# minjiyoon/MMGL

Hardware: AMD Instinct MI355X
Metric: train samples/sec (OPT-1.3B flamingo, 16 neighbors) (higher is better)
Workload: dtype bf16; 1 GPU; opt-1.3b context=all neighbor_mode=embedding peft=flamingo, 11+5 neighbors x 4 tokens, T=512+128, roberta-base + clip-vit-base-patch16 frozen encoders, full train step (fwd+bwd+exchange+AdamW); per_gpu_batch=64, global_batch=64, seq_len=640, neighbor_keys=64, trainable_params=216736520, parallelism=dp1

## Files before the change

### include/mmgl_hip.h

```cpp
#ifndef MMGL_HIP_H
#define MMGL_HIP_H

#include <stddef.h>
#include <stdint.h>

#ifdef __cplusplus
extern "C" {
#endif

enum { MMGL_F32 = 0, MMGL_BF16 = 1 };
enum { MMGL_OK = 0, MMGL_ERR_INVALID = 1, MMGL_ERR_UNSUPPORTED = 2, MMGL_ERR_HIP = 3 };
enum { MMGL_ACT_NONE = 0, MMGL_ACT_RELU = 1 };

const char* mmgl_last_error(void);
int mmgl_version(void);

int mmgl_xattn_fwd(const void* q, const void* k, const void* v, const uint8_t* key_valid,
                   void* out, float* lse, int B, int H, int T, int S, int D, int dtype, void* stream);

size_t mmgl_xattn_bwd_workspace(int B, int H, int T, int S, int D);
int mmgl_xattn_bwd(const void* dout, const void* q, const void* k, const void* v, const float* lse,
                   const uint8_t* key_valid, void* dq, void* dk, void* dv,
                   void* workspace, size_t workspace_bytes,
                   int B, int H, int T, int S, int D, int dtype, void* stream);
// ... 28 lines not shown
                          void* probs, float* lse, int B, int H, int T, int S, int D, int causal, float p_drop,
                          uint64_t seed, int dtype, void* stream);
size_t mmgl_attn_general_bwd_workspace(int B, int H, int T);
int mmgl_attn_general_bwd(const void* dout, const void* q, const void* k, const void* v, const float* lse, const uint8_t* key_valid,
                          const float* head_mask, void* dq, void* dk, void* dv, void* workspace, size_t workspace_bytes, int B, int H,
                          int T, int S, int D, int causal, float p_drop, uint64_t seed, int dtype, void* stream);
int mmgl_attn_dropout_mask(uint8_t* mask, int B, int H, int T, int S, float p_drop, uint64_t seed, void* stream);

int mmgl_layernorm_fwd(const void* x, const void* gamma, const void* beta, void* y, float* mean, float* rstd,
                       int rows, int cols, float eps, int dtype, void* stream);
size_t mmgl_norm_bwd_workspace(int rows, int cols);
int mmgl_layernorm_bwd(const void* dy, const void* x, const void* gamma, const float* mean, const float* rstd,
                       void* dx, float* dgamma, float* dbeta, void* workspace, size_t workspace_bytes,
                       int rows, int cols, int dtype, void* stream);

int mmgl_rmsnorm_fwd(const void* x, const void* gamma, void* y, float* rstd,
                     int rows, int cols, float eps, int dtype, void* stream);
int mmgl_rmsnorm_bwd(const void* dy, const void* x, const void* gamma, const float* rstd,
                     void* dx, float* dgamma, void* workspace, size_t workspace_bytes,
                     int rows, int cols, int dtype, void* stream);

int mmgl_add_rmsnorm_fwd(const void* x, const void* res, const void* gamma, void* sum_out, void* y, float* rstd,
                         int rows, int cols, float eps, int dtype, void* stream);
int mmgl_add_rmsnorm_bwd(const void* dy, const void* dsum, const void* sum, const void* gamma, const float* rstd,
                         void* dres, float* dgamma, void* workspace, size_t workspace_bytes,
                         int rows, int cols, int dtype, void* stream);

int mmgl_gated_residual_fwd(const void* residual, const void* x, const float* gate, void* y,
                            size_t n, float p_drop, uint64_t seed, int dtype, void* stream);
size_t mmgl_gated_residual_bwd_workspace(size_t n);
int mmgl_gated_residual_bwd(const void* dy, const void* x, const float* gate, void* dx, float* dgate,
                            void* workspace, size_t workspace_bytes,
                            size_t n, float p_drop, uint64_t seed, int dtype, void* stream);

int mmgl_linear_fwd(const void* x, const void* W, const void* bias, void* y,
                    int M, int N, int K, int act, float out_scale, int dtype, void* stream);
size_t mmgl_linear_bwd_workspace(int M, int N, int K, int act, int dtype);
int mmgl_linear_bwd(const void* dy, const void* y, const void* x, const void* W, void* dx, void* dW, void* dbias,
                    void* workspace, size_t workspace_bytes, int M, int N, int K, int act, float out_scale,
                    int accumulate, int mask_dx, int dtype, void* stream);

int mmgl_lora_linear_fwd(const void* x, const void* W, const void* bias, const void* A, const void* Bm,
                         void* y, void* xa, int M, int N, int K, int r, float scale, int dtype, void* stream);
size_t mmgl_lora_linear_bwd_workspace(int M, int N, int K, int r, int dtype);
int mmgl_lora_linear_bwd(const void* dy, const void* x, const void* xa, const void* W, const void* A,
                         const void* Bm, void* dx, void* dA, void* dB, void* dyb, void* workspace,
                         size_t workspace_bytes, int M, int N, int K, int r, float scale, int accumulate,
                         int dtype, void* stream);

int mmgl_neighbor_interleave_fwd(const void* text_emb, const void* vis_emb, const int64_t* text_loc,
                                 const int64_t* img_loc, const int64_t* text_pos, const int64_t* img_pos,
                                 void* out_emb, uint8_t* out_valid, int B, int Nt, int Ni, int n_tok, int d,
                                 int dtype, void* stream);
int mmgl_neighbor_interleave_bwd(const void* d_out_emb, const int64_t* text_loc, const int64_t* img_loc,
                                 void* d_text_emb, void* d_vis_emb, int B, int Nt, int Ni, int n_tok, int d,
                                 int dtype, void* stream);

int mmgl_cross_entropy_fwd(const void* logits, const int64_t* labels, float* row_lse, float* row_loss,
                           float* loss_sum, float* count, int rows, int V, int64_t ignore_index, int dtype,
                           void* stream);
int mmgl_cross_entropy_bwd(const void* logits, const int64_t* labels, const float* row_lse,
                           const float* count, const float* dloss, void* dlogits,
                           int rows, int V, int64_t ignore_index, int dtype, void* stream);

int mmgl_position_ids(const int64_t* attention_mask, int64_t* pos, int B, int T, void* stream);

int mmgl_adamw_step(void* param, float* master, const void* grad, float* exp_avg, float* exp_avg_sq, size_t n,
                    float lr, float beta1, float beta2, float eps, float weight_decay, int step,
                    float grad_scale, int dtype, void* stream);

int mmgl_gemm_nt_fast(int M, int N, int K, int ldx, int ldw, int ldy, int dtype);
size_t mmgl_gemm_nt_workspace(int M, int N, int K, int ldx, int ldw, int ldy, int dtype);
int mmgl_gemm_nt(const void* x, int ldx, const void* W, int ldw, const void* bias, const void* residual, const void* zmask,
                 void* y, int ldy, int M, int N, int K, int act, float out_scale, void* workspace, size_t workspace_bytes,
                 int dtype, void* stream);
int mmgl_relu_bwd(const void* dy, const void* y, void* out, size_t n, int dtype, void* stream);
int mmgl_gemm_set_tile_counter(void* counter);
void* mmgl_gemm_get_tile_counter(void);
size_t mmgl_gemm_nt_relu_bits_bytes(int M, int N, int K, int ldx, int ldw, int ldy, int dtype);
int mmgl_gemm_nt_relu_bits(const void* x, int ldx, const void* W, int ldw, const void* bias, void* y, int ldy, void* bits_out,
                           int M, int N, int K, float out_scale, int dtype, void* stream);
int mmgl_gemm_nt_masked(const void* x, int ldx, const void* W, int ldw, const void* bits_in, void* y, int ldy, int M, int N, int K,
                        float out_scale, int dtype, void* stream);

int mmgl_rope_inplace(void* buf, const float* cos_sin, size_t rows, int T, int H, int D, int ld, int nblk, int backward,
                      int dtype, void* stream);
int mmgl_rope(const void* src, void* dst, const float* cos_sin, size_t rows, int T, int H, int D, int ld, int nblk, int nall,
              int backward, int dtype, void* stream);
int mmgl_swiglu_fwd(const void* gate_up, void* y, size_t M, int F, int dtype, void* stream);
int mmgl_swiglu_bwd(const void* dy, const void* gate_up, void* dgate_up, size_t M, int F, int dtype, void* stream);

int mmgl_encattn_fwd(const void* q, const void* k, const void* v, const int32_t* cu_seqlens, void* out, int nseq,
                     int H, int D, int ld_in, int ld_out, int max_len, int q_rows, int dtype, void* stream);
int mmgl_add_layernorm_fwd(const void* x, const void* res, const void* gamma, const void* beta, void* sum_out,
                           void* y, float* mean, float* rstd, int rows, int cols, float eps, float p_drop, uint64_t seed,
                           int dtype, void* stream);
int mmgl_add_layernorm_bwd(const void* dy, const void* dsum, const void* sum, const void* gamma, const float* mean,
                           const float* rstd, void* dres, void* dx, float* dgamma, float* dbeta, void* workspace,
                           size_t workspace_bytes, int rows, int cols, float p_drop, uint64_t seed, int dtype,
                           void* stream);
int mmgl_layernorm_tiles_fwd(const void* x, const void* gamma, const void* beta, void* y, void* yc, const int32_t* rowmap,
                             float* mean, float* rstd, int rows, int cols, int crows, float eps, int dtype, void* stream);
int mmgl_add_layernorm_tiles_fwd(const void* x, const void* res, const void* gamma, const void* beta, void* sum_out, void* y,
                                 void* yc, const int32_t* rowmap, float* mean, float* rstd, int rows, int cols, int crows,
                                 float eps, float p_drop, uint64_t seed, int dtype, void* stream);
int mmgl_activation_fwd(const void* x, void* y, size_t n, int act, int dtype, void* stream);
int mmgl_scale(const void* x, const float* scale, void* y, size_t n, int dtype, void* stream);

enum { MMGL_COMM_I64 = 2 };
int mmgl_comm_unique_id(void* out128);
int mmgl_comm_init(int rank, int world, const void* unique_id, void** comm);
int mmgl_allreduce_sum(void* comm, void* buf, size_t count, int dtype, void* stream);
int mmgl_allgather(void* comm, const void* in, void* out, size_t count_per_rank, int dtype, void* stream);
int mmgl_broadcast(void* comm, void* buf, size_t count, int dtype, int root, void* stream);
int mmgl_comm_destroy(void* comm);

int mmgl_gemm_skinny_lora(const void* x, int ldx, const void* W, int ldw, const void* bias, const void* residual, void* y, int ldy,
                          const void* lora_A, int lda, const void* lora_B, int ldb, int r, float lora_scale, void* workspace,
                          int M, int N, int K, int act, float scale, int dtype, void* stream);
int mmgl_gemm_skinny(const void* x, int ldx, const void* W, int ldw, const void* bias, const void* residual, void* y, int ldy,
                     int M, int N, int K, int act, float scale, int dtype, void* stream);
int mmgl_attn_decode_fwd(const void* q, int ldq, const void* k, const void* v, int ldkv, size_t batch_stride_kv,
                         const uint8_t* key_valid, int ld_valid, void* out, int B, int H, int S, int D, int dtype, void* stream);

int mmgl_attn_decode_gqa_fwd(const void* q, int ldq, const void* k, const void* v, int ldkv, size_t batch_stride_kv,
                             const uint8_t* key_valid, int ld_valid, void* out, int B, int H, int Hkv, int S, int D, int dtype,
                             void* stream);
int mmgl_rope_kv_append(void* qkv, int ldqkv, const float* cos_sin_row, void* kv_col, size_t batch_stride_kv, int B, int H, int Hkv,
                        int D, int dtype, void* stream);

size_t mmgl_beam_topk_workspace(int rows, int V, int W);
int mmgl_attn_decode_beam_fwd(const void* q, int ldq, const void* k_pre, const void* v_pre, int ld_pre, size_t batch_stride_pre,
                              const uint8_t* key_valid, int ld_valid, const void* k_tail, const void* v_tail, int ld_tail,
                              size_t row_stride_tail, const int* src, int ld_src, void* out, int B, int W, int H, int S_pre, int n_tail,
                              int D, int dtype, void* stream);
int mmgl_beam_topk(const void* logits, size_t ld_logits, const float* beam_score, float* cand_score, int* cand_index, void* workspace,
                   size_t workspace_bytes, int B, int rows_in, int W, int V, int dtype, void* stream);
int mmgl_beam_advance(const float* cand_score, const int* cand_index, int64_t* tokens, int* parents, float* beam_score,
                      const int* src_old, int* src_new, int ld_src, const float* pool_score_old, float* pool_score_new,
                      const int* pool_len_old, int* pool_len_new, const int* pool_anc_old, int* pool_anc_new,
                      const int64_t* pool_tok_old, int64_t* pool_tok_new, int* done, int B, int W, int V, int n_cols, int eos_token_id,
                      int last_step, int early_stopping, float length_divisor, void* stream);

int mmgl_sample_tokens(const void* logits, size_t ld_logits, const float* u, int64_t* tokens, int64_t token_stride, uint8_t* finished,
                       int* kept, int rows, int n_draws, int V, float temperature, int top_k, float top_p, int eos_token_id,
                       int64_t pad_token_id, int dtype, void* stream);

int mmgl_logits_process(void* logits, size_t ld_logits, const int64_t* history, size_t ld_history, const uint8_t* hist_valid,
                        size_t ld_valid, int n_masked, int hist_len, const int* ban, int n_ban, int rows, int V,
                        float repetition_penalty, int no_repeat_ngram_size, int dtype, void* stream);

int mmgl_guidance_logits(void* logits, size_t ld_logits, int batch, int V, float guidance_scale, int dtype, void* stream);

int mmgl_attn_decode_block_fwd(const void* q, int ldq, const void* k_new, const void* v_new, int ld_new, void* k, void* v, int ldkv,
                               size_t batch_stride_kv, int capacity, const uint8_t* key_valid, int ld_valid, const int* len, void* out,
                               int B, int m, int H, int D, int dtype, void* stream);
int mmgl_lookup_accept(const void* logits, size_t ld_logits, int m_in, int64_t* block, int* n_draft, int64_t* positions, int64_t* ids,
                       size_t ld_ids, const uint8_t* prompt_mask, size_t ld_mask, int* gen, int* len, uint8_t* finished, int* emitted,
                       int B, int T, int n_new, int V, int K, int N, int64_t eos_token_id, int64_t pad_token_id, int pos_offset,
                       int pos_max, int dtype, void* stream);

int mmgl_rope_kv_append_block(void* qkv, int ldqkv, const float* cos_sin, int n_pos, void* kv, int ldkv, size_t batch_stride_kv, int capacity,
                              const int* len, int B, int m, int H, int Hkv, int D, int dtype, void* stream);
int mmgl_attn_decode_gqa_block_fwd(const void* q, int ldq, const void* k, const void* v, int ldkv, size_t batch_stride_kv, int capacity,
                                   const uint8_t* key_valid, int ld_valid, const int* len, void* out, int B, int m, int H, int Hkv, int D,
                                   int dtype, void* stream);

int mmgl_contrastive_chunk(void);
size_t mmgl_contrastive_workspace(int B, int k, int n_cap);
int mmgl_contrastive_select(const void* cand_hidden, size_t ld_cand, void* ctx, size_t ld_ctx, size_t batch_stride_ctx, uint8_t* ctx_valid,
                            size_t ld_valid, int n_cap, const float* cand_score, const int* cand_index, size_t ld_pair, float alpha, int n_ctx,
                            int step, int* src, size_t ld_src, int64_t* ids, size_t ld_ids, uint8_t* finished, int64_t eos_token_id,
                            int64_t pad_token_id, void* hidden_out, int* selected, float* trace_p, float* trace_pen, float* trace_score,
                            void* workspace, size_t workspace_bytes, int B, int k, int d, int V, int dtype, void* stream);

int mmgl_kv_quantize(const void* k, const void* v, int ld_src, size_t batch_stride_src, void* codes, int ld_code, size_t batch_stride_code,
                     void* scale, int ld_scale, size_t batch_stride_scale, int B, int n, int H, int D, int dtype, void* stream);
int mmgl_attn_decode_q8_fwd(const void* q, int ldq, const void* k_new, const void* v_new, int ld_new, void* k_codes, void* v_codes,
                            int ld_code, size_t batch_stride_code, void* k_scale, void* v_scale, int ld_scale, size_t batch_stride_scale,
                            int capacity, const uint8_t* key_valid, int ld_valid, void* out, int B, int H, int S, int D, int dtype,
                            void* stream);

int mmgl_attn_decode_gqa_q8_fwd(const void* q, int ldq, const void* k_new, const void* v_new, int ld_new, void* k_codes, void* v_codes,
                                int ld_code, size_t batch_stride_code, void* k_scale, void* v_scale, int ld_scale,
                                size_t batch_stride_scale, int capacity, const uint8_t* key_valid, int ld_valid, void* out, int B, int H,
                                int Hkv, int S, int D, int dtype, void* stream);

int mmgl_weight_quantize(const void* w, int ldw, void* codes, int ld_codes, void* exps, int N, int K, int dtype, void* stream);
// ... 8 lines not shown
```

### mmgl_amd/_lib.py

```python
import ctypes
import os

import torch

_HERE = os.path.dirname(os.path.abspath(__file__))
LIB_PATH = os.environ.get("MMGL_LIB_PATH") or os.path.join(_HERE, "libmmgl_hip.so")

ABI_VERSION = 110
F32, BF16 = 0, 1
ACT_NONE, ACT_RELU = 0, 1
_ERR_INVALID, _ERR_UNSUPPORTED, _ERR_HIP = 1, 2, 3

c_void_p, c_int, c_float, c_size_t, c_u64, c_i64 = (ctypes.c_void_p, ctypes.c_int, ctypes.c_float, ctypes.c_size_t,
                                                    ctypes.c_uint64, ctypes.c_int64)
P, I, F, Z, U, L = c_void_p, c_int, c_float, c_size_t, c_u64, c_i64

SIGNATURES = {
    "mmgl_last_error": (ctypes.c_char_p, []),
    "mmgl_version": (I, []),
    "mmgl_xattn_fwd": (I, [P, P, P, P, P, P, I, I, I, I, I, I, P]),
    "mmgl_xattn_bwd_workspace": (Z, [I, I, I, I, I]),
    "mmgl_xattn_bwd": (I, [P, P, P, P, P, P, P, P, P, P, Z, I, I, I, I, I, I, P]),
    "mmgl_selfattn_fwd": (I, [P, P, P, P, P, P, I, I, I, I, I, I, P]),
    "mmgl_selfattn_bwd_workspace": (Z, [I, I, I]),
    "mmgl_selfattn_bwd": (I, [P, P, P, P, P, P, P, P, P, P, P, Z, I, I, I, I, I, I, I, P]),
    "mmgl_selfattn_prefix_fwd": (I, [P, P, P, P, P, P, I, I, I, I, I, I, I, I, P]),
    "mmgl_selfattn_prefix_bwd": (I, [P, P, P, P, P, P, P, P, P, P, P, Z, I, I, I, I, I, I, I, I, I, I, P]),
    "mmgl_selfattn_tiles_fwd": (I, [P, P, P, P, P, P, P, I, I, I, I, I, I, I, I, P]),
    "mmgl_selfattn_tiles_bwd": (I, [P, P, P, P, P, P, P, P, P, P, P, P, Z, I, I, I, I, I, I, I, I, I, I, P]),
    "mmgl_selfattn_gqa_fwd": (I, [P, P, P, P, P, P, I, I, I, I, I, I, I, I, P]),
    "mmgl_selfattn_gqa_bwd_workspace": (Z, [I, I, I, I, I, I]),
    "mmgl_selfattn_gqa_bwd": (I, [P, P, P, P, P, P, P, P, P, P, P, Z, I, I, I, I, I, I, I, I, I, I, P]),
    "mmgl_attn_general_fwd": (I, [P, P, P, P, P, P, P, P, I, I, I, I, I, I, F, U, I, P]),
    "mmgl_attn_general_bwd_workspace": (Z, [I, I, I]),
    "mmgl_attn_general_bwd": (I, [P, P, P, P, P, P, P, P, P, P, P, Z, I, I, I, I, I, I, F, U, I, P]),
    "mmgl_attn_dropout_mask": (I, [P, I, I, I, I, F, U, P]),
    "mmgl_layernorm_fwd": (I, [P, P, P, P, P, P, I, I, F, I, P]),
    "mmgl_norm_bwd_workspace": (Z, [I, I]),
    "mmgl_layernorm_bwd": (I, [P, P, P, P, P, P, P, P, P, Z, I, I, I, P]),
    "mmgl_rmsnorm_fwd": (I, [P, P, P, P, I, I, F, I, P]),
    "mmgl_rmsnorm_bwd": (I, [P, P, P, P, P, P, P, Z, I, I, I, P]),
    "mmgl_add_rmsnorm_fwd": (I, [P, P, P, P, P, P, I, I, F, I, P]),
    "mmgl_add_rmsnorm_bwd": (I, [P, P, P, P, P, P, P, P, Z, I, I, I, P]),
    "mmgl_gated_residual_fwd": (I, [P, P, P, P, Z, F, U, I, P]),
    "mmgl_gated_residual_bwd_workspace": (Z, [Z]),
    "mmgl_gated_residual_bwd": (I, [P, P, P, P, P, P, Z, Z, F, U, I, P]),
    "mmgl_linear_fwd": (I, [P, P, P, P, I, I, I, I, F, I, P]),
    "mmgl_linear_bwd_workspace": (Z, [I, I, I, I, I]),
    "mmgl_linear_bwd": (I, [P, P, P, P, P, P, P, P, Z, I, I, I, I, F, I, I, I, P]),
    "mmgl_lora_linear_fwd": (I, [P, P, P, P, P, P, P, I, I, I, I, F, I, P]),
    "mmgl_lora_linear_bwd_workspace": (Z, [I, I, I, I, I]),
    "mmgl_lora_linear_bwd": (I, [P, P, P, P, P, P, P, P, P, P, P, Z, I, I, I, I, F, I, I, P]),
    "mmgl_neighbor_interleave_fwd": (I, [P, P, P, P, P, P, P, P, I, I, I, I, I, I, P]),
    "mmgl_neighbor_interleave_bwd": (I, [P, P, P, P, P, I, I, I, I, I, I, P]),
    "mmgl_cross_entropy_fwd": (I, [P, P, P, P, P, P, I, I, L, I, P]),
    "mmgl_cross_entropy_bwd": (I, [P, P, P, P, P, P, I, I, L, I, P]),
    "mmgl_position_ids": (I, [P, P, I, I, P]),
    "mmgl_adamw_step": (I, [P, P, P, P, P, Z, F, F, F, F, F, I, F, I, P]),
    "mmgl_encattn_fwd": (I, [P, P, P, P, P, I, I, I, I, I, I, I, I, P]),
    "mmgl_add_layernorm_fwd": (I, [P, P, P, P, P, P, P, P, I, I, F, F, U, I, P]),
    "mmgl_add_layernorm_bwd": (I, [P, P, P, P, P, P, P, P, P, P, P, Z, I, I, F, U, I, P]),
    "mmgl_layernorm_tiles_fwd": (I, [P, P, P, P, P, P, P, P, I, I, I, F, I, P]),
    "mmgl_add_layernorm_tiles_fwd": (I, [P, P, P, P, P, P, P, P, P, P, I, I, I, F, F, U, I, P]),
    "mmgl_activation_fwd": (I, [P, P, Z, I, I, P]),
    "mmgl_scale": (I, [P, P, P, Z, I, P]),
    "mmgl_gemm_nt_fast": (I, [I, I, I, I, I, I, I]),
    "mmgl_gemm_nt_workspace": (Z, [I, I, I, I, I, I, I]),
    "mmgl_gemm_nt_relu_bits_bytes": (Z, [I, I, I, I, I, I, I]),
    "mmgl_gemm_nt_relu_bits": (I, [P, I, P, I, P, P, I, P, I, I, I, F, I, P]),
    "mmgl_gemm_nt_masked": (I, [P, I, P, I, P, P, I, I, I, I, F, I, P]),
    "mmgl_gemm_nt": (I, [P, I, P, I, P, P, P, P, I, I, I, I, I, F, P, Z, I, P]),
    "mmgl_relu_bwd": (I, [P, P, P, Z, I, P]),
    "mmgl_gemm_set_tile_counter": (I, [P]),
    "mmgl_gemm_get_tile_counter": (P, []),
    "mmgl_rope_inplace": (I, [P, P, Z, I, I, I, I, I, I, I, P]),
    "mmgl_rope": (I, [P, P, P, Z, I, I, I, I, I, I, I, I, P]),
    "mmgl_swiglu_fwd": (I, [P, P, Z, I, I, P]),
    "mmgl_swiglu_bwd": (I, [P, P, P, Z, I, I, P]),
    "mmgl_comm_unique_id": (I, [P]),
    "mmgl_comm_init": (I, [I, I, P, ctypes.POINTER(ctypes.c_void_p)]),
    "mmgl_allreduce_sum": (I, [P, P, Z, I, P]),
    "mmgl_allgather": (I, [P, P, P, Z, I, P]),
    "mmgl_broadcast": (I, [P, P, Z, I, I, P]),
    "mmgl_comm_destroy": (I, [P]),
    "mmgl_gemm_skinny": (I, [P, I, P, I, P, P, P, I, I, I, I, I, F, I, P]),
    "mmgl_attn_decode_fwd": (I, [P, I, P, P, I, Z, P, I, P, I, I, I, I, I, P]),
    "mmgl_gemm_skinny_lora": (I, [P, I, P, I, P, P, P, I, P, I, P, I, I, F, P, I, I, I, I, F, I, P]),
    "mmgl_attn_decode_gqa_fwd": (I, [P, I, P, P, I, Z, P, I, P, I, I, I, I, I, I, P]),
    "mmgl_rope_kv_append": (I, [P, I, P, P, Z, I, I, I, I, I, P]),
    "mmgl_attn_decode_beam_fwd": (I, [P, I, P, P, I, Z, P, I, P, P, I, Z, P, I, P, I, I, I, I, I, I, I, P]),
    "mmgl_beam_topk_workspace": (Z, [I, I, I]),
    "mmgl_beam_topk": (I, [P, Z, P, P, P, P, Z, I, I, I, I, I, P]),
    "mmgl_beam_advance": (I, [P, P, P, P, P, P, P, I, P, P, P, P, P, P, P, P, P, I, I, I, I, I, I, I, F, P]),
    "mmgl_sample_tokens": (I, [P, Z, P, P, L, P, P, I, I, I, F, I, F, I, L, I, P]),
    "mmgl_logits_process": (I, [P, Z, P, Z, P, Z, I, I, P, I, I, I, F, I, I, P]),
    "mmgl_guidance_logits": (I, [P, Z, I, I, F, I, P]),
    "mmgl_attn_decode_block_fwd": (I, [P, I, P, P, I, P, P, I, Z, I, P, I, P, P, I, I, I, I, I, P]),
    "mmgl_lookup_accept": (I, [P, Z, I, P, P, P, P, Z, P, Z, P, P, P, P, I, I, I, I, I, I, L, L, I, I, I, P]),
    "mmgl_rope_kv_append_block": (I, [P, I, P, I, P, I, Z, I, P, I, I, I, I, I, I, P]),
    "mmgl_attn_decode_gqa_block_fwd": (I, [P, I, P, P, I, Z, I, P, I, P, P, I, I, I, I, I, I, P]),
    "mmgl_contrastive_chunk": (I, []),
    "mmgl_contrastive_workspace": (Z, [I, I, I]),
    "mmgl_contrastive_select": (I, [P, Z, P, Z, Z, P, Z, I, P, P, Z, F, I, I, P, Z, P, Z, P, L, L, P, P, P, P, P, P, Z, I, I, I, I, I, P]),
    "mmgl_kv_quantize": (I, [P, P, I, Z, P, I, Z, P, I, Z, I, I, I, I, I, P]),
    "mmgl_attn_decode_q8_fwd": (I, [P, I, P, P, I, P, P, I, Z, P, P, I, Z, I, P, I, P, I, I, I, I, I, P]),
    "mmgl_attn_decode_gqa_q8_fwd": (I, [P, I, P, P, I, P, P, I, Z, P, P, I, Z, I, P, I, P, I, I, I, I, I, I, P]),
    "mmgl_weight_quantize": (I, [P, I, P, I, P, I, I, I, P]),
    "mmgl_gemm_skinny_w8": (I, [P, I, P, I, P, P, P, P, I, I, I, I, I, F, I, P]),
}

_lib = None


def lib():
    global _lib
    if _lib is None:
        if not os.path.exists(LIB_PATH):
            raise RuntimeError(
                f"{LIB_PATH} not found: the HIP extension is not built. Run `python -m mmgl_amd._build` "
                "(or __graft_entry__.build()). mmgl_amd has no CPU fallback.")
        h = ctypes.CDLL(LIB_PATH)
        h.mmgl_version.restype = ctypes.c_int
        if h.mmgl_version() != ABI_VERSION:
            raise RuntimeError(f"{LIB_PATH} reports ABI version {h.mmgl_version()}, this binding expects {ABI_VERSION}: a stale build -- "
                               "run `python -m mmgl_amd._build --force`")
        for name, (res, args) in SIGNATURES.items():
            fn = getattr(h, name)
            fn.restype = res
            fn.argtypes = args
        _lib = h
    return _lib


def check(rc: int, what: str = ""):
    if rc == 0:
        return
    msg = lib().mmgl_last_error().decode("utf-8", "replace")
    if rc in (_ERR_INVALID, _ERR_UNSUPPORTED):
        raise ValueError(msg or what)
    raise RuntimeError(msg or what)


def dtype_code(t: torch.Tensor) -> int:
    if t.dtype == torch.float32:
        return F32
    if t.dtype == torch.bfloat16:
        return BF16
    raise ValueError(f"mmgl_amd kernels take float32 or bfloat16 activations, got {t.dtype}")


def ptr(t):
    return None if t is None else ctypes.c_void_p(t.data_ptr())


# ... 60 lines not shown
```

### mmgl_amd/csrc/gemm.hip

```cpp
#include "common.h"
#include "gemm8p.h"
#include <stdlib.h>

namespace {

constexpr int BM = 128, BN = 128, ROWB = 128;
constexpr int TILE_BYTES = BM * ROWB;

template <typename T> struct GT {
    static constexpr int VN = 16 / sizeof(T);
    static constexpr int BK = ROWB / sizeof(T);
    static constexpr int KSTEPS = BK / 32;
    typedef T chunk_t __attribute__((ext_vector_type(16 / sizeof(T))));
};

__device__ __forceinline__ int swz(int row, int c) { return row * ROWB + ((c ^ ((row >> 1) & 7)) << 4); }

template <typename T> __device__ __forceinline__ typename Elem<T>::v8 lds_frag(const char* tile, int row, int ks, int g);
template <> __device__ __forceinline__ bf16x8 lds_frag<bf16>(const char* tile, int row, int ks, int g) {
    return *(const bf16x8*)(tile + swz(row, ks * 4 + g));
}
template <> __device__ __forceinline__ f32x8 lds_frag<float>(const char* tile, int row, int ks, int g) {
    const f32x4 a = *(const f32x4*)(tile + swz(row, 2 * g));
    const f32x4 b = *(const f32x4*)(tile + swz(row, 2 * g + 1));
// ... 796 lines not shown
    MMGL_CHECK_ARG(dy && x && W && workspace && (act == MMGL_ACT_NONE || y), "mmgl_linear_bwd: null pointer");
    MMGL_CHECK_ARG(workspace_bytes >= mmgl_linear_bwd_workspace(M, N, K, act, dtype), "mmgl_linear_bwd: workspace too small");
    hipStream_t st = (hipStream_t)stream;
    char* ws = (char*)workspace;
    DT_SWITCH("mmgl_linear_bwd",
              linear_bwd<bf16>((const bf16*)dy, (const bf16*)y, (const bf16*)x, (const bf16*)W, (bf16*)dx, (bf16*)dW, (bf16*)dbias, ws, M, N, K, act, out_scale, accumulate, st, mask_dx != 0),
              linear_bwd<float>((const float*)dy, (const float*)y, (const float*)x, (const float*)W, (float*)dx, (float*)dW, (float*)dbias, ws, M, N, K, act, out_scale, accumulate, st, mask_dx != 0));
}

extern "C" int mmgl_lora_linear_fwd(const void* x, const void* W, const void* bias, const void* A, const void* Bm, void* y,
                                    void* xa, int M, int N, int K, int r, float scale, int dtype, void* stream) {
    MMGL_CHECK_ARG(x && W && A && Bm && y && xa && r > 0, "mmgl_lora_linear_fwd: bad arguments");
    hipStream_t st = (hipStream_t)stream;
    DT_SWITCH("mmgl_lora_linear_fwd",
              lora_fwd<bf16>((const bf16*)x, (const bf16*)W, (const bf16*)bias, (const bf16*)A, (const bf16*)Bm, (bf16*)y, (bf16*)xa, M, N, K, r, scale, st),
              lora_fwd<float>((const float*)x, (const float*)W, (const float*)bias, (const float*)A, (const float*)Bm, (float*)y, (float*)xa, M, N, K, r, scale, st));
}

extern "C" size_t mmgl_lora_linear_bwd_workspace(int M, int N, int K, int r, int dtype) {
    return lora_ws(M, N, K, r, dtype == MMGL_BF16 ? 2 : 4);
}

extern "C" int mmgl_lora_linear_bwd(const void* dy, const void* x, const void* xa, const void* W, const void* A,
                                    const void* Bm, void* dx, void* dA, void* dB, void* dyb, void* workspace,
                                    size_t workspace_bytes, int M, int N, int K, int r, float scale, int accumulate,
                                    int dtype, void* stream) {
    MMGL_CHECK_ARG(dy && x && xa && W && A && Bm && dx && dA && dB && dyb && workspace && r > 0, "mmgl_lora_linear_bwd: bad arguments");
    MMGL_CHECK_ARG(workspace_bytes >= mmgl_lora_linear_bwd_workspace(M, N, K, r, dtype), "mmgl_lora_linear_bwd: workspace too small");
    hipStream_t st = (hipStream_t)stream;
    char* ws = (char*)workspace;
    DT_SWITCH("mmgl_lora_linear_bwd",
              lora_bwd<bf16>((const bf16*)dy, (const bf16*)x, (const bf16*)xa, (const bf16*)W, (const bf16*)A, (const bf16*)Bm, (bf16*)dx, (bf16*)dA, (bf16*)dB, (bf16*)dyb, ws, M, N, K, r, scale, accumulate, st),
              lora_bwd<float>((const float*)dy, (const float*)x, (const float*)xa, (const float*)W, (const float*)A, (const float*)Bm, (float*)dx, (float*)dA, (float*)dB, (float*)dyb, ws, M, N, K, r, scale, accumulate, st));
}

extern "C" int mmgl_gemm_nt_fast(int M, int N, int K, int ldx, int ldw, int ldy, int dtype) {
    const NtRoute r = nt_route(M, N, K, ldx, ldw, ldy, dtype, true);
    return r == NtRoute::P8 ? 1 : r == NtRoute::MID ? 2 : 0;
}

extern "C" size_t mmgl_gemm_nt_workspace(int M, int N, int K, int ldx, int ldw, int ldy, int dtype) {
    if (nt_route(M, N, K, ldx, ldw, ldy, dtype, true) != NtRoute::P8 || !gemm8p_use_splits(M, N, K)) return 0;
    return align_up(gemm8p_split_bytes(M, N, K), 256);
}

extern "C" int mmgl_gemm_nt(const void* x, int ldx, const void* W, int ldw, const void* bias, const void* residual, const void* zmask,
                            void* y, int ldy, int M, int N, int K, int act, float out_scale, void* workspace, size_t workspace_bytes,
                            int dtype, void* stream) {
    MMGL_CHECK_ARG(x && W && y, "mmgl_gemm_nt: null pointer");
    MMGL_CHECK_ARG(act >= 0 && act <= 4, "mmgl_gemm_nt: unknown activation %d", act);
    MMGL_CHECK_ARG(ldx + 127 >= K && ldw >= K && ldy >= N, "mmgl_gemm_nt: leading dimensions (%d, %d, %d) smaller than the rows (K=%d, N=%d)", ldx, ldw, ldy, K, N);
    hipStream_t st = (hipStream_t)stream;
    const NtRoute r = nt_route(M, N, K, ldx, ldw, ldy, dtype, true);
    DT_SWITCH("mmgl_gemm_nt",
              launch_nt<bf16>(r, (const bf16*)x, ldx, (const bf16*)W, ldw, (bf16*)y, ldy, (const bf16*)bias, (const bf16*)residual,
                              (const bf16*)zmask, M, N, K, act, out_scale, (float*)workspace, workspace_bytes, st),
              launch_nt<float>(r, (const float*)x, ldx, (const float*)W, ldw, (float*)y, ldy, (const float*)bias, (const float*)residual,
                               (const float*)zmask, M, N, K, act, out_scale, (float*)workspace, workspace_bytes, st));
}

extern "C" size_t mmgl_gemm_nt_relu_bits_bytes(int M, int N, int K, int ldx, int ldw, int ldy, int dtype) {
    return nt_route(M, N, K, ldx, ldw, ldy, dtype, false) == NtRoute::P8 ? gemm8p_bits_bytes(M, N) : 0;
}

extern "C" int mmgl_gemm_nt_relu_bits(const void* x, int ldx, const void* W, int ldw, const void* bias, void* y, int ldy, void* bits_out,
                                      int M, int N, int K, float out_scale, int dtype, void* stream) {
    MMGL_CHECK_ARG(x && W && y && bits_out, "mmgl_gemm_nt_relu_bits: null pointer");
    MMGL_CHECK_ARG(mmgl_gemm_nt_relu_bits_bytes(M, N, K, ldx, ldw, ldy, dtype) > 0,
                   "mmgl_gemm_nt_relu_bits: shape M=%d N=%d K=%d (ld %d %d %d, dtype %d) does not run as whole tiles of the persistent kernel", M, N, K, ldx, ldw, ldy, dtype);
    return launch_gemm8p((const bf16*)x, ldx, (const bf16*)W, ldw, (bf16*)y, ldy, (const bf16*)bias, nullptr, nullptr, M, N, K, MMGL_ACT_RELU,
                         out_scale, (hipStream_t)stream, nullptr, 0, (unsigned*)bits_out, nullptr);
}

extern "C" int mmgl_gemm_nt_masked(const void* x, int ldx, const void* W, int ldw, const void* bits_in, void* y, int ldy, int M, int N, int K,
                                   float out_scale, int dtype, void* stream) {
    MMGL_CHECK_ARG(x && W && y && bits_in, "mmgl_gemm_nt_masked: null pointer");
    MMGL_CHECK_ARG(ldx + 127 >= K && ldw >= K && ldy >= N, "mmgl_gemm_nt_masked: leading dimensions (%d, %d, %d) smaller than the rows (K=%d, N=%d)", ldx, ldw, ldy, K, N);
    MMGL_CHECK_ARG(mmgl_gemm_nt_relu_bits_bytes(M, N, K, ldx, ldw, ldy, dtype) > 0,
                   "mmgl_gemm_nt_masked: shape M=%d N=%d K=%d (ld %d %d %d, dtype %d) does not run as whole tiles of the persistent kernel", M, N, K, ldx, ldw, ldy, dtype);
    return launch_gemm8p((const bf16*)x, ldx, (const bf16*)W, ldw, (bf16*)y, ldy, nullptr, nullptr, nullptr, M, N, K, MMGL_ACT_NONE, out_scale,
                         (hipStream_t)stream, nullptr, 0, nullptr, (const unsigned*)bits_in);
}

extern "C" int mmgl_relu_bwd(const void* dy, const void* y, void* out, size_t n, int dtype, void* stream) {
    MMGL_CHECK_ARG(dy && y && out, "mmgl_relu_bwd: null pointer");
    hipStream_t st = (hipStream_t)stream;
    DT_SWITCH("mmgl_relu_bwd", launch_relu_mask<bf16>((const bf16*)dy, (const bf16*)y, (bf16*)out, n, 1.f, st),
              launch_relu_mask<float>((const float*)dy, (const float*)y, (float*)out, n, 1.f, st));
}
```

### mmgl_amd/csrc/gemm8p.h

```cpp
#pragma once
#include "common.h"

bool gemm8p_supported(int M, int N, int K, int ldx, int ldw, int ldy);
constexpr int GEMM8P_MIN_TILES = 160;
int gemm8p_splits(int M, int N, int K);
size_t gemm8p_split_bytes(int M, int N, int K);
int launch_gemm8p(const bf16* X, int ldx, const bf16* W, int ldw, bf16* Y, int ldy, const bf16* bias, const bf16* resid,
                  const bf16* zmask, int M, int N, int K, int act, float scale, hipStream_t st, float* part = nullptr,
                  size_t part_bytes = 0, unsigned* bits_out = nullptr, const unsigned* bits_in = nullptr);
inline size_t gemm8p_bits_bytes(int M, int N) { return (size_t)cdiv(M, 256) * cdiv(N, 256) * 8192; }

int gemm8p_tt_splits(int RA, int RB, int M);
int launch_gemm8p_tt(const bf16* A, int lda, const bf16* B, int ldb, bf16* Out, float* part, int RA, int RB, int M, int nsplit, float scale,
                     int accumulate, hipStream_t st);

bool gemm_mid_supported(int M, int N, int K, int ldx, int ldw, int ldy);
int launch_gemm_mid(const bf16* X, int ldx, const bf16* W, int ldw, bf16* Y, int ldy, const bf16* bias, const bf16* resid, const bf16* zmask,
                    int M, int N, int K, int act, float scale, hipStream_t st);
```

### mmgl_amd/csrc/gemm8p.hip

```cpp
#include "common.h"
#include "gemm8p.h"
#include <atomic>
#include <stdlib.h>
#include <type_traits>

namespace {

typedef __attribute__((address_space(3))) void lds_void;
typedef unsigned p8_u32x4 __attribute__((ext_vector_type(4)));

constexpr int P8_UNIT = 16384;
constexpr int P8_LDS = 8 * P8_UNIT;
constexpr int P8_LDS_TOTAL = P8_LDS + 16 * 1024;
constexpr int P8_LDS_ALLOC = P8_LDS_TOTAL + 64;

struct P8Args {
    const bf16* X;
    const bf16* W;
    bf16* Y;
    const bf16* bias;
    const bf16* resid;
    const bf16* zmask;
    int M, N, K;
    int ldx, ldw, ldy;
    float scale;
    int act;
    int tiles_m, tiles_n, total;
    int nsplit;
    float* part;
    unsigned* bits_out;
    const unsigned* bits_in;
    int tile0;
    long long* trace;
    int trace_wg;
    unsigned* sched;
};

__device__ __forceinline__ int p8_fetch_item(unsigned* sched, int xcd, int nlists, int G, int Gx, int nitems) {
    for (int t = 0; t < nlists; ++t) {
        const int j = xcd + t < nlists ? xcd + t : xcd + t - nlists;
        const unsigned k = atomicAdd(&sched[j], 1u);
        const long long v = (long long)(k / (unsigned)Gx) * G + j * Gx + (int)(k % (unsigned)Gx);
        if (v < nitems) return (int)v;
    }
    return -1;
}

template <int ACT> __device__ __forceinline__ float p8_act(float v) {
    if constexpr (ACT == 2) {
        const float z = fabsf(v) * 0.70710678118654752f;
        const float t = __builtin_amdgcn_rcpf(1.f + 0.3275911f * z);
        const float poly = t * (0.254829592f + t * (-0.284496736f + t * (1.421413741f + t * (-1.453152027f + t * 1.061405429f))));
        const float er = 1.f - poly * __expf(-z * z);
        return 0.5f * v * (1.f + copysignf(er, v));
    }
    else if constexpr (ACT == 3) return v * __builtin_amdgcn_rcpf(1.f + __expf(-1.702f * v));
    else if constexpr (ACT == 4) {
        const float u = 0.7978845608028654f * (v + 0.044715f * v * v * v);
        return 0.5f * v * (1.f + tanhf(u));
    } else if constexpr (ACT == 1) return fmaxf(v, 0.f);
    else return v;
}

__device__ __forceinline__ int p8_lane() {
    int l;
    asm volatile("v_mbcnt_lo_u32_b32 %0, -1, 0\n\tv_mbcnt_hi_u32_b32 %0, -1, %0" : "=v"(l));
    return l;
}

#ifndef P8_STORE_AUX
#define P8_STORE_AUX 18
#endif
#ifndef P8_ZMASK_AUX
#define P8_ZMASK_AUX 2
#endif
#ifndef P8_PART_AUX
#define P8_PART_AUX 0
#endif
#ifndef P8_LOADX_AUX
#define P8_LOADX_AUX 0
#endif
#ifndef P8_LOADW_AUX
#define P8_LOADW_AUX 0
#endif
#ifndef P8_TRACE
#define P8_TRACE 0
#endif
#define P8_BARRIER() asm volatile("s_barrier" ::: "memory")
#define P8_VMCNT(n) asm volatile("s_waitcnt vmcnt(" #n ")" ::: "memory")
#define P8_LGKM0() asm volatile("s_waitcnt lgkmcnt(0)" ::: "memory")

template <int ACT, bool ZR> __global__ __launch_bounds__(512) void gemm8p_kernel(P8Args a) {
    extern __shared__ __attribute__((aligned(16))) char smem[];
    const int tid = threadIdx.x, lane = tid & 63;
    const int wave = __builtin_amdgcn_readfirstlane(tid >> 6);
    const int wr = wave >> 2, wc = wave & 3;
    const int x = lane & 15, g = lane >> 4;
    int nk = a.K >> 6;

    const int G = gridDim.x;
    const int wg = (G & 7) == 0 ? (int)(blockIdx.x & 7) * (G >> 3) + (int)(blockIdx.x >> 3) : (int)blockIdx.x;
    const bool dyn = a.sched != nullptr;
    const int nlists = (G & 7) == 0 ? 8 : 1, Gx = G / nlists, xcd = nlists == 8 ? (int)(blockIdx.x & 7) : 0;
    int* mailbox = (int*)(smem + P8_LDS_TOTAL);
    auto item_origin = [&](int v, int& m0, int& n0, int& k0, int& nki, int& sp) -> bool {
        if (v < 0 || v >= a.total * a.nsplit) return false;
        int tm, tn;
        sp = v % a.nsplit;
        grouped_tile(a.tile0 + v / a.nsplit, a.tiles_m, a.tiles_n, tm, tn);
        m0 = tm * 256;
        n0 = tn * 256;
        const int units = a.K >> 7, base = units / a.nsplit, rem = units % a.nsplit;
        k0 = (sp * base + (sp < rem ? sp : rem)) * 128;
        nki = (base + (sp < rem ? 1 : 0)) * 2;
        return true;
    };
    auto tile_origin = [&](int it, int& m0, int& n0, int& k0, int& nki, int& sp) -> bool { return item_origin(it * G + wg, m0, n0, k0, nki, sp); };
    auto mk_desc = [&](const bf16* base, int row0, int rows, int ld, int k0, bool valid) {
// ... 54 lines not shown
#if P8_TRACE
    int tr_n = 0;
    auto stamp = [&](int it_) __attribute__((always_inline)) {
        if (a.trace && (int)blockIdx.x == a.trace_wg && it_ >= 2 && tr_n < 64) {
            const long long t = __builtin_readcyclecounter();
            if (lane == 0) a.trace[wave * 64 + tr_n] = t;
            ++tr_n;
        }
    };
#define P8_STAMP(it_) stamp(it_)
#else
#define P8_STAMP(it_) (void)0
#endif

#define P8_MM(FX, FW, J0, T0, I0, I1)                                                          \
    do {                                                                                       \
        _Pragma("unroll") for (int i_ = (I0); i_ < (I1); ++i_) {                               \
            const int ks_ = i_ >> 3, j_ = (i_ >> 1) & 3, t_ = i_ & 1;                          \
            mma16(acc[(T0) + t_][(J0) + j_], FW[ks_][t_], FX[ks_][j_]);                        \
        }                                                                                      \
    } while (0)

    int m0 = 0, n0 = 0, m1 = 0, n1 = 0, k0 = 0, k1 = 0, nk1 = 0, sp0 = 0, sp1 = 0;
    int it = 0;
    int vcur = wg, vnext = G + wg;
    if (dyn) {
        if (tid == 0) mailbox[2] = p8_fetch_item(a.sched, xcd, nlists, G, Gx, a.total * a.nsplit);
        __syncthreads();
        vcur = mailbox[2];
        if (vcur < 0) {
            if (tid == 0 && atomicAdd(&a.sched[8], 1u) == (unsigned)G - 1u)
                for (int i = 0; i < 9; ++i) atomicExch(&a.sched[i], 0u);
            return;
        }
    }
    if (!item_origin(vcur, m0, n0, k0, nk, sp0)) return;
    bool have_next = dyn ? false : tile_origin(1, m1, n1, k1, nk1, sp1);
    __amdgpu_buffer_rsrc_t dXc = mk_desc(a.X, m0, a.M, a.ldx, k0, true), dWc = mk_desc(a.W, n0, a.N, a.ldw, k0, true);
    __amdgpu_buffer_rsrc_t dXn = mk_desc(a.X, m1, a.M, a.ldx, k1, have_next), dWn = mk_desc(a.W, n1, a.N, a.ldw, k1, have_next);

    const __amdgpu_buffer_rsrc_t dBias = __builtin_amdgcn_make_buffer_rsrc((void*)a.bias, 0, a.bias ? a.N * 2 : 0, 0x00020000);
    auto fetch_bias = [&](int nt0, int par) __attribute__((always_inline)) {
        const int ln = p8_lane();
        const unsigned off = ln < 8 ? (unsigned)((nt0 + wc * 64 + ln * 8) * 2) : 0xffffffffu;
        __builtin_amdgcn_raw_ptr_buffer_load_lds(dBias, (lds_void*)(smem + P8_LDS + (par & 1) * 8192 + wave * 1024), 16, off, 0, 0, 0);
    };
    auto y_desc = [&](const bf16* base, int mt0) {
        long long rem = (long long)(a.M - mt0) * a.ldy * 2;
        if (rem > 0xffffffffLL) rem = 0xffffffffLL;
        return __builtin_amdgcn_make_buffer_rsrc((void*)(base + (size_t)mt0 * a.ldy), 0, (int)(unsigned)rem, 0x00020000);
    };
    const bool has_bias = a.bias != nullptr, has_scale = a.scale != 1.f;
    auto epilogue_q = [&](int m0, int n0, int par, int q_lo, int q_hi) __attribute__((always_inline)) {
        if constexpr (ACT == 5) {
            const int ln = p8_lane();
            const int ncol_l = wc * 64 + 8 * (ln >> 4);
            const unsigned base = (unsigned)(((wr * 128 + (ln & 15)) * 256 + ncol_l) * 4);
            const unsigned rstep = (unsigned)(16 * 256 * 4);
            const int vitem = vcur;
            const __amdgpu_buffer_rsrc_t dP = __builtin_amdgcn_make_buffer_rsrc((void*)(a.part + ((size_t)vitem << 16)), 0, 256 * 256 * 4, 0x00020000);
#pragma unroll
            for (int T0 = 0; T0 < 4; T0 += 2)
#pragma unroll
                for (int J = 0; J < 8; ++J) {
                    const unsigned off = base + (unsigned)J * rstep + (unsigned)(64 * T0);
                    __builtin_amdgcn_raw_buffer_store_b128(__builtin_bit_cast(p8_u32x4, acc[T0][J]), dP, off, 0, P8_PART_AUX);
                    __builtin_amdgcn_raw_buffer_store_b128(__builtin_bit_cast(p8_u32x4, acc[T0 + 1][J]), dP, off + 16, 0, P8_PART_AUX);
                    acc[T0][J] = vzero<f32x4>();
                    acc[T0 + 1][J] = vzero<f32x4>();
                }
            return;
        }
        const int ln = p8_lane();
        const int ncol_l = wc * 64 + 8 * (ln >> 4);
        const bool col_ok0 = n0 + ncol_l < a.N, col_ok1 = n0 + ncol_l + 32 < a.N;
        const unsigned base = (unsigned)(((wr * 128 + (ln & 15)) * a.ldy + n0 + ncol_l) * 2);
        const unsigned rstep = (unsigned)(16 * a.ldy * 2);
        auto y_off = [&](int J, int T0) __attribute__((always_inline)) -> unsigned {
            return (T0 ? col_ok1 : col_ok0) ? base + (unsigned)J * rstep + (unsigned)(32 * T0) : 0xffffffffu;
        };
        const __amdgpu_buffer_rsrc_t dY = y_desc(a.Y, m0);
        bf16x8 pre[16];
        p8_u32x4 mbits = {0u, 0u, 0u, 0u};
        if constexpr (ZR) {
            const __amdgpu_buffer_rsrc_t dZ = y_desc(a.zmask ? a.zmask : a.resid, m0);
            if (a.bits_in) {
                mbits = *(const p8_u32x4*)(a.bits_in + ((size_t)((a.tile0 + vcur) * 8 + wave) * 64 + ln) * 4);
            } else if (a.zmask) {
#pragma unroll
                for (int q = 0; q < 4; ++q)
#pragma unroll
                    for (int j = 0; j < 4; ++j) {
                        const int J0 = (q == 0 || q == 1) ? 0 : 4, T0 = (q == 0 || q == 3) ? 0 : 2;
                        pre[q * 4 + j] = __builtin_bit_cast(bf16x8, __builtin_amdgcn_raw_buffer_load_b128(dZ, y_off(J0 + j, T0), 0, P8_ZMASK_AUX));
                    }
            } else {
#pragma unroll
                for (int q = 0; q < 4; ++q)
#pragma unroll
                    for (int j = 0; j < 4; ++j) {
                        const int J0 = (q == 0 || q == 1) ? 0 : 4, T0 = (q == 0 || q == 3) ? 0 : 2;
                        pre[q * 4 + j] = __builtin_bit_cast(bf16x8, __builtin_amdgcn_raw_buffer_load_b128(dZ, y_off(J0 + j, T0), 0, 0));
                    }
            }
        }
#pragma unroll
        for (int q = 0; q < 4; ++q) {
            if (q < q_lo || q >= q_hi) continue;
            const int J0 = (q == 0 || q == 1) ? 0 : 4, T0 = (q == 0 || q == 3) ? 0 : 2;
            if (has_bias) {
                const bf16x8 br = *(const bf16x8*)(smem + P8_LDS + (par & 1) * 8192 + wave * 1024 + ((ln >> 4) + 2 * T0) * 16);
                const f32x4 b0 = {(float)br[0], (float)br[1], (float)br[2], (float)br[3]}, b1 = {(float)br[4], (float)br[5], (float)br[6], (float)br[7]};
#pragma unroll
                for (int j = 0; j < 4; ++j) { acc[T0][J0 + j] += b0; acc[T0 + 1][J0 + j] += b1; }
            }
            if (has_scale) {
#pragma unroll
                for (int j = 0; j < 4; ++j) { acc[T0][J0 + j] *= a.scale; acc[T0 + 1][J0 + j] *= a.scale; }
            }
            unsigned qbits = 0;
            auto rows = [&](auto mode_tag) __attribute__((always_inline)) {
                constexpr int MODE = decltype(mode_tag)::value;
#pragma unroll
                for (int j = 0; j < 4; ++j) {
                    const unsigned off = y_off(J0 + j, T0);
                    const f32x4 lo = acc[T0][J0 + j], hi = acc[T0 + 1][J0 + j];
                    f32x8 v = {lo[0], lo[1], lo[2], lo[3], hi[0], hi[1], hi[2], hi[3]};
                    if constexpr (ACT >= 2 || (ACT == 1 && ZR)) {
#pragma unroll
                        for (int e = 0; e < 8; ++e) v[e] = p8_act<ACT>(v[e]);
                    }
                    if constexpr (MODE == 2) {
                        const bf16x8 z = pre[q * 4 + j];
#pragma unroll
                        for (int e = 0; e < 8; ++e) v[e] += (float)z[e];
                    }
                    if constexpr (MODE == 3) {
                        const bf16x8 z = pre[q * 4 + j];
                        const __amdgpu_buffer_rsrc_t dR = y_desc(a.resid, m0);
                        const bf16x8 rr = __builtin_bit_cast(bf16x8, __builtin_amdgcn_raw_buffer_load_b128(dR, off, 0, 0));
#pragma unroll
                        for (int e = 0; e < 8; ++e) v[e] = (((float)z[e] > 0.f) ? v[e] : 0.f) + (float)rr[e];
                    }
                    p8_u32x4 ob = __builtin_bit_cast(p8_u32x4, __builtin_convertvector(v, bf16x8));
                    if constexpr (ACT == 1 && !ZR) {
#pragma unroll
                        for (int e = 0; e < 4; ++e) {
                            unsigned w = ob[e];
                            asm("v_pk_max_i16 %0, %1, 0" : "=v"(w) : "v"(w));
                            ob[e] = w;
                        }
                        if (a.bits_out) {
                            unsigned by = 0;
#pragma unroll
                            for (int e = 0; e < 4; ++e) {
                                unsigned t = ob[e];
                                asm("v_pk_min_u16 %0, %1, 1 op_sel_hi:[1,0]" : "=v"(t) : "v"(t));
                                t |= t >> 15;
                                by |= t << (2 * e);
                            }
                            qbits |= (by & 0xffu) << (8 * j);
                        }
                    }
                    if constexpr (MODE == 1) {
                        const p8_u32x4 zz = __builtin_bit_cast(p8_u32x4, pre[q * 4 + j]);
#pragma unroll
                        for (int e = 0; e < 4; ++e) {
                            unsigned m = zz[e];
                            asm("v_pk_max_i16 %0, %1, 0\n\tv_pk_min_u16 %0, %0, 1 op_sel_hi:[1,0]\n\tv_pk_sub_u16 %0, 0, %0" : "=v"(m) : "v"(m));
                            ob[e] &= m;
                        }
                    }
                    if constexpr (MODE == 4) {
                        const unsigned by = mbits[q] >> (8 * j);
#pragma unroll
                        for (int e = 0; e < 4; ++e) {
                            unsigned t = (by >> (2 * e)) & 3u;
                            t = (t | (t << 15)) & 0x00010001u;
                            unsigned mk;
                            asm("v_mul_u32_u24 %0, %1, %2" : "=v"(mk) : "v"(t), "v"(0xffffu));
                            ob[e] &= mk;
                        }
                    }
                    __builtin_amdgcn_raw_buffer_store_b128(ob, dY, off, 0, P8_STORE_AUX);
                }
            };
            if constexpr (!ZR) rows(std::integral_constant<int, 0>());
            else if (a.bits_in) rows(std::integral_constant<int, 4>());
            else if (a.zmask && a.resid) rows(std::integral_constant<int, 3>());
            else if (a.zmask) rows(std::integral_constant<int, 1>());
            else rows(std::integral_constant<int, 2>());
            if constexpr (ACT == 1 && !ZR) {
                if (a.bits_out) a.bits_out[((size_t)((a.tile0 + vcur) * 8 + wave) * 64 + ln) * 4 + q] = qbits;
            }
#pragma unroll
            for (int j = 0; j < 4; ++j) { acc[T0][J0 + j] = vzero<f32x4>(); acc[T0 + 1][J0 + j] = vzero<f32x4>(); }
        }
    };
    auto epilogue = [&]() __attribute__((always_inline)) { epilogue_q(m0, n0, it, 0, 4); };


    stage(3, 7, dWc, 0);
    stage(0, 0, dXc, 0);
    stage(1, 1, dWc, 0);
    stage(2, 2, dXc, 0);
    stage(3, 3, dWc, 128);
    stage(0, 4, dXc, 128);
    stage(1, 5, dWc, 128);
#pragma unroll
    for (int t = 0; t < 4; ++t)
#pragma unroll
        for (int j = 0; j < 8; ++j) acc[t][j] = vzero<f32x4>();
    bf16x8 fx[2][4], fwA[2][2], fwB[2][2];
    fetch_bias(n0, 0);
    if (dyn && tid == 0) {
        const int nit = a.total * a.nsplit, cap = (nit + G - 1) / G;
        const int i1 = cap >= 2 ? p8_fetch_item(a.sched, xcd, nlists, G, Gx, nit) : -1;
        mailbox[0] = i1;
        mailbox[1] = (cap >= 3 && i1 >= 0) ? p8_fetch_item(a.sched, xcd, nlists, G, Gx, nit) : -1;
        asm volatile("s_waitcnt lgkmcnt(0)" ::: "memory");
    }
    P8_VMCNT(11);
    P8_BARRIER();
    rdW(fwA, 7);
    P8_LGKM0();
    if (wr) P8_BARRIER();
    if (dyn) {
        vnext = mailbox[0];
        have_next = item_origin(vnext, m1, n1, k1, nk1, sp1);
        dXn = mk_desc(a.X, m1, a.M, a.ldx, k1, have_next);
        dWn = mk_desc(a.W, n1, a.N, a.ldw, k1, have_next);
    }

#define P8_PHASE_M(READ, TY, SLOT, DK, FX, FW, J0, T0, MM, WAITN)                                \
    do {                                                                                         \
        READ;                                                                                    \
        {                                                                                        \
            const int kk_ = kt + (DK);                                                           \
            const bool nx_ = kk_ >= nk;                                                          \
            const int kb_ = (nx_ ? kk_ - nk : kk_) * 128;                                        \
            if ((TY) & 1) stage((TY), (SLOT), nx_ ? dWn : dWc, kb_);                             \
            else stage((TY), (SLOT), nx_ ? dXn : dXc, kb_);                                      \
        }                                                                                        \
        P8_VMCNT(WAITN);                                                                         \
        P8_BARRIER();                                                                            \
        __builtin_amdgcn_sched_barrier(0);                                                       \
        __builtin_amdgcn_s_setprio(1);                                                           \
         \
         \
        MM(FX, FW, J0, T0, 0, 15);                                                               \
        P8_LGKM0();                                                                              \
        __builtin_amdgcn_sched_barrier(0);                                                       \
        P8_BARRIER();                                                                            \
        MM(FX, FW, J0, T0, 15, 16);                                                              \
        __builtin_amdgcn_s_setprio(0);                                                           \
        __builtin_amdgcn_sched_barrier(0);                                                       \
    } while (0)

#define P8_PHASE(READ, TY, SLOT, DK, FX, FW, J0, T0) P8_PHASE_M(READ, TY, SLOT, DK, FX, FW, J0, T0, P8_MM, 10)
    for (;;) {
        P8_STAMP(it);
        for (int kt = 0; kt < nk; kt += 2) {
            P8_PHASE(rdX(fx, 0), 2, 6, 1, fx, fwA, 0, 0);
            if (kt < 4) P8_STAMP(it);
            P8_PHASE(rdW(fwB, 1), 3, 7, 2, fx, fwB, 0, 2);
            if (kt < 4) P8_STAMP(it);
            P8_PHASE(rdX(fx, 2), 0, 0, 2, fx, fwB, 4, 2);
            if (kt < 4) P8_STAMP(it);
            P8_PHASE(rdW(fwB, 3), 1, 1, 2, fx, fwA, 4, 0);
            if (kt < 4) P8_STAMP(it);
// ... 78 lines not shown
        }
        const size_t yo = m * (size_t)ldy + n;
        if (zmask) {
            const bf16x8 z = *(const bf16x8*)(zmask + yo);
#pragma unroll
            for (int e = 0; e < 8; ++e) v[e] = ((float)z[e] > 0.f) ? v[e] : 0.f;
        }
        if (resid) {
            const bf16x8 r = *(const bf16x8*)(resid + yo);
#pragma unroll
            for (int e = 0; e < 8; ++e) v[e] += (float)r[e];
        }
        f32x8 o8 = {v[0], v[1], v[2], v[3], v[4], v[5], v[6], v[7]};
        *(bf16x8*)(Y + yo) = __builtin_convertvector(o8, bf16x8);
    }
}

}

void gemm8p_plan(int M, int N, int K, int* direct, int* nsplit) {
    const int tiles = cdiv(M, 256) * cdiv(N, 256), units = K / 128;
    *direct = tiles;
    *nsplit = 0;
    if (tiles < GEMM8P_MIN_TILES) {
        constexpr int min_units = 24;
        if (units < min_units) return;
        if (units < 32 && tiles >= 64) return;
        int s = (224 + tiles - 1) / tiles;
        if (s > 8) s = 8;
        if (s > units / 2) s = units / 2;
        if (s >= 2) { *direct = 0; *nsplit = s; }
        return;
    }
    constexpr int hybrid = 3;
    const int G = mmgl_num_cu(), rounds = tiles / G, r = tiles % G;
    if (!hybrid || rounds < 1 || rounds > 12 || r == 0) return;
    int s = G / r;
    if (s > 8) s = 8;
    if (s > units / 4) s = units / 4;
    if (s >= hybrid && s >= 2) { *direct = tiles - r; *nsplit = s; }
}
int gemm8p_splits(int M, int N, int K) {
    int d, s;
    gemm8p_plan(M, N, K, &d, &s);
    return s;
}

bool gemm8p_supported(int M, int N, int K, int ldx, int ldw, int ldy) {
    return M > 0 && N > 0 && K >= 256 && K % 128 == 0 && N % 16 == 0 && ldx % 8 == 0 && ldw % 8 == 0 && ldy % 8 == 0 &&
           (long long)M * ldx * 2 < 0xffffffffLL && (long long)N * ldw * 2 < 0xffffffffLL;
}

size_t gemm8p_split_bytes(int M, int N, int K) {
    int d, sp;
    gemm8p_plan(M, N, K, &d, &sp);
    return sp ? (size_t)(cdiv(M, 256) * cdiv(N, 256) - d) * sp * (256 * 256 * sizeof(float)) : 0;
}

static std::atomic<unsigned*> g_tile_counter[64];
static std::atomic<int> g_tile_counters_set{0};
static hipStream_t const P8_STREAM_UNBOUND = (hipStream_t)(intptr_t)-1;
static std::atomic<hipStream_t> g_tile_stream[64];
static unsigned* p8_tile_counter() {
    if (!g_tile_counters_set.load(std::memory_order_relaxed)) return nullptr;
    int dev = 0;
    if (hipGetDevice(&dev) != hipSuccess) return nullptr;
    return g_tile_counter[dev & 63].load(std::memory_order_acquire);
}
static bool p8_tile_counter_for(hipStream_t st, unsigned** out) {
    *out = nullptr;
    if (!g_tile_counters_set.load(std::memory_order_relaxed)) return true;
    int dev = 0;
    if (hipGetDevice(&dev) != hipSuccess) return true;
    unsigned* c = g_tile_counter[dev & 63].load(std::memory_order_acquire);
    if (!c) return true;
    hipStream_t bound = P8_STREAM_UNBOUND;
    if (!g_tile_stream[dev & 63].compare_exchange_strong(bound, st, std::memory_order_acq_rel) && bound != st) return false;
    *out = c;
    return true;
}

int launch_gemm8p(const bf16* X, int ldx, const bf16* W, int ldw, bf16* Y, int ldy, const bf16* bias, const bf16* resid,
                  const bf16* zmask, int M, int N, int K, int act, float scale, hipStream_t st, float* part, size_t part_bytes,
                  unsigned* bits_out, const unsigned* bits_in) {
    if (!gemm8p_supported(M, N, K, ldx, ldw, ldy))
        MMGL_FAIL(MMGL_ERR_UNSUPPORTED, "gemm8p: shape M=%d N=%d K=%d (ld %d %d %d) not supported", M, N, K, ldx, ldw, ldy);
    P8Args a;
    a.X = X; a.W = W; a.Y = Y; a.bias = bias; a.resid = resid; a.zmask = zmask;
    a.M = M; a.N = N; a.K = K; a.ldx = ldx; a.ldw = ldw; a.ldy = ldy; a.scale = scale; a.act = act;
    a.tiles_m = cdiv(M, 256); a.tiles_n = cdiv(N, 256); a.total = a.tiles_m * a.tiles_n;
    a.nsplit = 1;
    a.part = nullptr;
    a.bits_out = bits_out;
    a.bits_in = bits_in;
    if (bits_out && (act != 1 || resid || zmask)) MMGL_FAIL(MMGL_ERR_INVALID, "gemm8p: mask bits are written by the plain ReLU epilogue only");
    if (bits_in && (zmask || resid || act != 0)) MMGL_FAIL(MMGL_ERR_INVALID, "gemm8p: mask bits are applied by the plain epilogue only");
    if (bits_out || bits_in) part = nullptr;
    const int n_cu = mmgl_num_cu();
    const int tiles = a.total;
    int direct = tiles, nsplit = 0;
    if (part && part_bytes >= gemm8p_split_bytes(M, N, K)) gemm8p_plan(M, N, K, &direct, &nsplit);
    a.trace = nullptr;
    a.trace_wg = 0;
    a.tile0 = 0;
    if (!p8_tile_counter_for(st, &a.sched)) {
        static const bool strict = getenv("MMGL_GEMM_STRICT_STREAM") && atoi(getenv("MMGL_GEMM_STRICT_STREAM"));
        if (strict)
            MMGL_FAIL(MMGL_ERR_INVALID, "gemm8p: the dynamic tile schedule of this device is bound to another stream (one stream per device "
                                        "while mmgl_gemm_set_tile_counter is in effect)");
        a.sched = nullptr;
    }
    if (direct > 0) {
        a.total = direct;
        const int grid = direct < n_cu ? direct : n_cu;
#if P8_TRACE
        if (const char* e = getenv("MMGL_P8_TRACE")) a.trace = (long long*)strtoull(e, nullptr, 0);
        if (const char* e = getenv("MMGL_P8_TRACE_WG")) a.trace_wg = atoi(e);
#endif
        const bool zr = resid || zmask || bits_in;
#define P8_LAUNCH(A, Z)                                                                                     \
    do {                                                                                                    \
        if (int rc = mmgl_set_lds(gemm8p_kernel<A, Z>, P8_LDS_ALLOC, "gemm8p")) return rc;                  \
        hipLaunchKernelGGL((gemm8p_kernel<A, Z>), dim3(grid), dim3(512), P8_LDS_ALLOC, st, a);              \
    } while (0)
        switch (act) {
            case 0: if (zr) P8_LAUNCH(0, true); else P8_LAUNCH(0, false); break;
            case 1: if (zr) P8_LAUNCH(1, true); else P8_LAUNCH(1, false); break;
            case 2: if (zr) MMGL_FAIL(MMGL_ERR_UNSUPPORTED, "gemm8p: gelu(erf) with residual / zmask is not instantiated"); P8_LAUNCH(2, false); break;
            case 3: if (zr) P8_LAUNCH(3, true); else P8_LAUNCH(3, false); break;
            case 4: if (zr) P8_LAUNCH(4, true); else P8_LAUNCH(4, false); break;
            default: MMGL_FAIL(MMGL_ERR_INVALID, "gemm8p: unknown activation %d", act);
        }
#undef P8_LAUNCH
        MMGL_CHECK_LAUNCH("gemm8p");
    }
    if (nsplit) {
        MMGL_CHECK_ARG(act >= 0 && act <= 4, "gemm8p: unknown activation %d", act);
        const int rest = tiles - direct;
        a.tile0 = direct;
        a.total = rest;
        a.nsplit = nsplit;
        a.part = part;
        a.trace = nullptr;
        const int items = rest * nsplit, g = items < n_cu ? items : n_cu;
        if (int rc = mmgl_set_lds(gemm8p_kernel<5, false>, P8_LDS_ALLOC, "gemm8p (K split)")) return rc;
        hipLaunchKernelGGL((gemm8p_kernel<5, false>), dim3(g), dim3(512), P8_LDS_ALLOC, st, a);
        MMGL_CHECK_LAUNCH("gemm8p (K split)");
        int blocks = rest * 32;
        if (blocks > 2048) blocks = 2048;
        hipLaunchKernelGGL(p8_splitk_finish_kernel, dim3(blocks), dim3(256), 0, st, part, Y, bias, resid, zmask, M, N, ldy, nsplit, act, scale,
                           direct, rest, a.tiles_m, a.tiles_n);
        MMGL_CHECK_LAUNCH("gemm8p split-K finish");
    }
    return MMGL_OK;
}

extern "C" int mmgl_gemm_set_tile_counter(void* counter) {
    int dev = 0;
    hipError_t e = hipGetDevice(&dev);
    if (e != hipSuccess) MMGL_FAIL(MMGL_ERR_HIP, "mmgl_gemm_set_tile_counter: hipGetDevice: %s", hipGetErrorString(e));
    g_tile_stream[dev & 63].store(P8_STREAM_UNBOUND, std::memory_order_release);
    unsigned* old = g_tile_counter[dev & 63].exchange((unsigned*)counter, std::memory_order_acq_rel);
    g_tile_counters_set.fetch_add((counter != nullptr) - (old != nullptr), std::memory_order_relaxed);
    return MMGL_OK;
}

extern "C" void* mmgl_gemm_get_tile_counter(void) { return p8_tile_counter(); }
```

### mmgl_amd/csrc/rownorm.hip

```cpp
#include "common.h"

namespace {

constexpr int NVMAX = 4;
constexpr int MAXBLK = 512;

template <typename T> struct Vec {
    static constexpr int N = 16 / sizeof(T);
    typedef T type __attribute__((ext_vector_type(16 / sizeof(T))));
};

template <int TPR> __device__ __forceinline__ float row_sum(float v, float* red, int row_in_blk) {
    v = wave_sum(v);
    if constexpr (TPR == 64) return v;
    else {
        const int w = threadIdx.x >> 6;
        __syncthreads();
        if ((threadIdx.x & 63) == 0) red[w] = v;
        __syncthreads();
        return red[0] + red[1] + red[2] + red[3];
    }
}

template <typename T, int TPR, int NV, int MODE>
__global__ __launch_bounds__(256) void norm_fwd_kernel(const T* __restrict__ x, const T* __restrict__ res,
                                                       const T* __restrict__ gamma, const T* __restrict__ beta,
                                                       T* __restrict__ sum_out, T* __restrict__ y,
                                                       float* __restrict__ mean, float* __restrict__ rstd, int rows,
                                                       int cols, float eps, float p, uint64_t seed,
                                                       const int* __restrict__ rowmap, T* __restrict__ yc, int crows) {
    constexpr bool RMS = (MODE & 1) != 0, COMPACT = (MODE & 4) != 0;
    typedef typename Vec<T>::type V;
    constexpr int VN = Vec<T>::N;
    __shared__ float red[4];
    const int rpb = 256 / TPR;
    const int tr = threadIdx.x % TPR, rib = threadIdx.x / TPR;
    const int nchunks = cols / VN;
    const float keep_scale = p > 0.f ? 1.f / (1.f - p) : 1.f;
    const uint32_t thr = (uint32_t)fminf(p * 4294967296.f, 4294967295.f);
    for (int row0 = blockIdx.x * rpb; row0 < rows; row0 += gridDim.x * rpb) {
        const int row = row0 + rib;
        const bool live = row < rows;
        int crow = -1;
        if constexpr (COMPACT) crow = live ? rowmap[row] : -1;
        float xv[NV][VN];
        float s = 0.f;
#pragma unroll
        for (int i = 0; i < NV; ++i) {
            const int c = tr + i * TPR;
            if (live && c < nchunks) {
                V v = *(const V*)(x + (size_t)row * cols + c * VN);
                if (res) {
                    const V r = *(const V*)(res + (size_t)row * cols + c * VN);
                    if (p > 0.f) {
                        const uint64_t e0 = (uint64_t)row * cols + (uint64_t)c * VN;
#pragma unroll
                        for (int j = 0; j < VN; ++j) {
                            const float a = (mmgl_hash32(seed, e0 + j) < thr) ? 0.f : (float)v[j];
                            v[j] = (T)fmaf(keep_scale, a, (float)r[j]);
                        }
                    } else {
#pragma unroll
                        for (int j = 0; j < VN; ++j) v[j] = (T)((float)v[j] + (float)r[j]);
                    }
                    if (sum_out) *(V*)(sum_out + (size_t)row * cols + c * VN) = v;
                }
#pragma unroll
                for (int j = 0; j < VN; ++j) { xv[i][j] = (float)v[j]; s += xv[i][j]; }
            } else {
#pragma unroll
                for (int j = 0; j < VN; ++j) xv[i][j] = 0.f;
            }
        }
        float mu = 0.f;
        if constexpr (!RMS) mu = row_sum<TPR>(s, red, rib) / cols;
        float ss = 0.f;
#pragma unroll
        for (int i = 0; i < NV; ++i) {
            const int c = tr + i * TPR;
            if (c < nchunks) {
#pragma unroll
                for (int j = 0; j < VN; ++j) { const float d = xv[i][j] - mu; ss += d * d; }
            }
        }
        const float var = row_sum<TPR>(ss, red, rib) / cols;
        const float rs = rsqrtf(var + eps);
        if (live && tr == 0) {
            if (mean) mean[row] = mu;
            if (rstd) rstd[row] = rs;
        }
#pragma unroll
        for (int i = 0; i < NV; ++i) {
            const int c = tr + i * TPR;
            if (live && c < nchunks) {
                V o;
                V gv, bv;
                if (gamma) gv = *(const V*)(gamma + c * VN);
                if (beta) bv = *(const V*)(beta + c * VN);
#pragma unroll
                for (int j = 0; j < VN; ++j) {
                    float t = (xv[i][j] - mu) * rs;
                    if (gamma) t *= (float)gv[j];
                    if (beta) t += (float)bv[j];
                    o[j] = (T)t;
                }
                *(V*)(y + (size_t)row * cols + c * VN) = o;
                if constexpr (COMPACT) {
                    if ((unsigned)crow < (unsigned)crows) *(V*)(yc + (size_t)crow * cols + c * VN) = o;
                }
            }
        }
    }
}

template <typename T, int TPR, int NV, int MODE>
__global__ __launch_bounds__(256) void norm_bwd_kernel(const T* __restrict__ dy, const T* __restrict__ x,
                                                       const T* __restrict__ gamma, const float* __restrict__ mean,
                                                       const float* __restrict__ rstd, const T* __restrict__ dres,
                                                       T* __restrict__ dx, T* __restrict__ dx_drop, float* __restrict__ part,
                                                       int rows, int cols, float p, uint64_t seed) {
    constexpr bool RMS = (MODE & 1) != 0, PARAMS = (MODE & 2) != 0;
    typedef typename Vec<T>::type V;
    constexpr int VN = Vec<T>::N;
    __shared__ float red[4];
    const int rpb = 256 / TPR;
    const int tr = threadIdx.x % TPR, rib = threadIdx.x / TPR;
    const int nchunks = cols / VN;
    float dg[NV][VN], dbt[NV][VN], gm[NV][VN];
#pragma unroll
    for (int i = 0; i < NV; ++i) {
        const int c = tr + i * TPR;
        V gv;
        const bool hg = gamma && c < nchunks;
        if (hg) gv = *(const V*)(gamma + c * VN);
// ... 54 lines not shown
                    for (int j = 0; j < VN; ++j) od[j] = (mmgl_hash32(seed, e0 + j) < thr) ? (T)0.f : (T)((float)o[j] * ks);
                    *(V*)(dx_drop + (size_t)row * cols + c * VN) = od;
                }
            }
        }
    }
    if (PARAMS && part) {
        float* pg = part + ((size_t)(blockIdx.x * rpb + rib)) * cols * 2;
#pragma unroll
        for (int i = 0; i < NV; ++i) {
            const int c = tr + i * TPR;
            if (c < nchunks) {
#pragma unroll
                for (int j = 0; j < VN; ++j) {
                    pg[c * VN + j] = dg[i][j];
                    pg[cols + c * VN + j] = dbt[i][j];
                }
            }
        }
    }
}

__global__ __launch_bounds__(256) void norm_param_reduce_kernel(const float* __restrict__ part, float* __restrict__ dgamma,
                                                                float* __restrict__ dbeta, int nparts, int cols) {
    __shared__ float red[8][33];
    const int cx = threadIdx.x & 31, py = threadIdx.x >> 5;
    const int c = blockIdx.x * 32 + cx;
    float a = 0.f;
    if (c < 2 * cols) {
        int p = py;
        for (; p + 24 < nparts; p += 32) {
            const float v0 = part[(size_t)p * cols * 2 + c], v1 = part[(size_t)(p + 8) * cols * 2 + c];
            const float v2 = part[(size_t)(p + 16) * cols * 2 + c], v3 = part[(size_t)(p + 24) * cols * 2 + c];
            a += (v0 + v1) + (v2 + v3);
        }
        for (; p < nparts; p += 8) a += part[(size_t)p * cols * 2 + c];
    }
    red[py][cx] = a;
    __syncthreads();
    if (py == 0 && c < 2 * cols) {
        float s = 0.f;
#pragma unroll
        for (int i = 0; i < 8; ++i) s += red[i][cx];
        if (c < cols) { if (dgamma) dgamma[c] = s; }
        else if (dbeta) dbeta[c - cols] = s;
    }
}

struct Geo { int tpr, nv, rpb; };
template <typename T> int geometry(const char* who, int rows, int cols, Geo& g) {
    constexpr int VN = Vec<T>::N;
    MMGL_CHECK_ARG(rows > 0 && cols > 0, "%s: rows/cols must be positive", who);
    if (cols % VN) MMGL_FAIL(MMGL_ERR_UNSUPPORTED, "%s: cols=%d must be a multiple of %d", who, cols, VN);
    const int nchunks = cols / VN;
    g.tpr = (nchunks <= 64 * 4) ? 64 : 256;
    g.nv = (nchunks + g.tpr - 1) / g.tpr;
    if (g.nv > NVMAX) MMGL_FAIL(MMGL_ERR_UNSUPPORTED, "%s: cols=%d exceeds the register-resident row limit %d", who, cols,
                                256 * NVMAX * VN);
    g.rpb = 256 / g.tpr;
    return MMGL_OK;
}

int bwd_blocks(int rows, int rpb) {
    int b = (rows + rpb - 1) / rpb;
    return b > MAXBLK ? MAXBLK : b;
}

#define NORM_DISPATCH(KERN, T, RMS, g, ...)                                                        \
    do {                                                                                           \
        if (g.tpr == 64) {                                                                         \
            if (g.nv == 1) hipLaunchKernelGGL((KERN<T, 64, 1, RMS>), __VA_ARGS__);                 \
            else if (g.nv == 2) hipLaunchKernelGGL((KERN<T, 64, 2, RMS>), __VA_ARGS__);            \
            else hipLaunchKernelGGL((KERN<T, 64, 4, RMS>), __VA_ARGS__);                           \
        } else {                                                                                   \
            if (g.nv == 1) hipLaunchKernelGGL((KERN<T, 256, 1, RMS>), __VA_ARGS__);                \
            else if (g.nv == 2) hipLaunchKernelGGL((KERN<T, 256, 2, RMS>), __VA_ARGS__);           \
            else hipLaunchKernelGGL((KERN<T, 256, 4, RMS>), __VA_ARGS__);                          \
        }                                                                                          \
    } while (0)

template <typename T, bool RMS>
int norm_fwd(const char* who, const void* x, const void* res, const void* gamma, const void* beta, void* sum_out, void* y,
             float* mean, float* rstd, int rows, int cols, float eps, hipStream_t st, float p = 0.f, uint64_t seed = 0,
             const int* rowmap = nullptr, void* yc = nullptr, int crows = 0) {
    Geo g;
    int rc = geometry<T>(who, rows, cols, g);
    if (rc) return rc;
    int blocks = (rows + g.rpb - 1) / g.rpb;
    if (blocks > 8192) blocks = 8192;
    if (!RMS && rowmap)
        NORM_DISPATCH(norm_fwd_kernel, T, (RMS ? 1 : 4), g, dim3(blocks), dim3(256), 0, st, (const T*)x, (const T*)res, (const T*)gamma,
                      (const T*)beta, (T*)sum_out, (T*)y, mean, rstd, rows, cols, eps, p, seed, rowmap, (T*)yc, crows);
    else
        NORM_DISPATCH(norm_fwd_kernel, T, (RMS ? 1 : 0), g, dim3(blocks), dim3(256), 0, st, (const T*)x, (const T*)res, (const T*)gamma,
                      (const T*)beta, (T*)sum_out, (T*)y, mean, rstd, rows, cols, eps, p, seed, (const int*)nullptr, (T*)nullptr, 0);
    MMGL_CHECK_LAUNCH(who);
    return MMGL_OK;
}

template <typename T, bool RMS>
int norm_bwd(const char* who, const void* dy, const void* x, const void* gamma, const float* mean, const float* rstd,
             const void* dres, void* dx, float* dgamma, float* dbeta, void* ws, size_t ws_bytes, int rows, int cols, hipStream_t st,
             void* dx_drop = nullptr, float p = 0.f, uint64_t seed = 0) {
    Geo g;
    int rc = geometry<T>(who, rows, cols, g);
    if (rc) return rc;
    const bool want = dgamma || dbeta;
    int blocks = bwd_blocks(rows, g.rpb);
    if (!want) { blocks = (rows + g.rpb - 1) / g.rpb; if (blocks > 8192) blocks = 8192; }
    float* part = nullptr;
    if (want) {
        MMGL_CHECK_ARG(ws && ws_bytes >= (size_t)blocks * g.rpb * cols * 2 * sizeof(float),
                       "%s: workspace too small (%zu B)", who, ws_bytes);
        part = (float*)ws;
    }
    if (want)
        NORM_DISPATCH(norm_bwd_kernel, T, (RMS ? 3 : 2), g, dim3(blocks), dim3(256), 0, st, (const T*)dy, (const T*)x,
                      (const T*)gamma, mean, rstd, (const T*)dres, (T*)dx, (T*)dx_drop, part, rows, cols, p, seed);
    else
        NORM_DISPATCH(norm_bwd_kernel, T, (RMS ? 1 : 0), g, dim3(blocks), dim3(256), 0, st, (const T*)dy, (const T*)x,
                      (const T*)gamma, mean, rstd, (const T*)dres, (T*)dx, (T*)dx_drop, part, rows, cols, p, seed);
    MMGL_CHECK_LAUNCH(who);
    if (want) {
        hipLaunchKernelGGL(norm_param_reduce_kernel, dim3((2 * cols + 31) / 32), dim3(256), 0, st, part, dgamma, dbeta,
                           blocks * g.rpb, cols);
        MMGL_CHECK_LAUNCH(who);
    }
    return MMGL_OK;
}

}

extern "C" size_t mmgl_norm_bwd_workspace(int rows, int cols) {
    if (rows <= 0 || cols <= 0) return 0;
    size_t parts = (size_t)((rows + 3) / 4) * 4;
    if (parts > (size_t)MAXBLK * 4) parts = (size_t)MAXBLK * 4;
    return parts * cols * 2 * sizeof(float);
}

#define NORM_BY_DTYPE(FN, RMS, ...)                                                    \
    do {                                                                               \
        if (dtype == MMGL_BF16) return FN<bf16, RMS>(__func__, __VA_ARGS__);           \
        if (dtype == MMGL_F32) return FN<float, RMS>(__func__, __VA_ARGS__);           \
        MMGL_FAIL(MMGL_ERR_INVALID, "%s: bad dtype %d", __func__, dtype);              \
    } while (0)

extern "C" int mmgl_layernorm_fwd(const void* x, const void* gamma, const void* beta, void* y, float* mean, float* rstd,
                                  int rows, int cols, float eps, int dtype, void* stream) {
    MMGL_CHECK_ARG(x && y && mean && rstd, "mmgl_layernorm_fwd: null pointer");
    NORM_BY_DTYPE(norm_fwd, false, x, nullptr, gamma, beta, nullptr, y, mean, rstd, rows, cols, eps, (hipStream_t)stream);
}

extern "C" int mmgl_add_layernorm_fwd(const void* x, const void* res, const void* gamma, const void* beta, void* sum_out,
                                      void* y, float* mean, float* rstd, int rows, int cols, float eps, float p_drop,
                                      uint64_t seed, int dtype, void* stream) {
    MMGL_CHECK_ARG(x && res && y, "mmgl_add_layernorm_fwd: null pointer");
    MMGL_CHECK_ARG(p_drop >= 0.f && p_drop < 1.f, "mmgl_add_layernorm_fwd: dropout p=%g outside [0,1)", p_drop);
    NORM_BY_DTYPE(norm_fwd, false, x, res, gamma, beta, sum_out, y, mean, rstd, rows, cols, eps, (hipStream_t)stream, p_drop, seed);
}

static int compact_check(const char* who, const int32_t* rowmap, const void* yc, int rows, int crows) {
    MMGL_CHECK_ARG(rowmap && yc && crows > 0 && crows <= rows, "%s: rowmap / compact buffer missing or crows = %d outside (0, rows]", who, crows);
    return MMGL_OK;
}

extern "C" int mmgl_layernorm_tiles_fwd(const void* x, const void* gamma, const void* beta, void* y, void* yc, const int32_t* rowmap,
                                        float* mean, float* rstd, int rows, int cols, int crows, float eps, int dtype, void* stream) {
    MMGL_CHECK_ARG(x && y && mean && rstd, "mmgl_layernorm_tiles_fwd: null pointer");
    if (int rc = compact_check("mmgl_layernorm_tiles_fwd", rowmap, yc, rows, crows)) return rc;
    NORM_BY_DTYPE(norm_fwd, false, x, nullptr, gamma, beta, nullptr, y, mean, rstd, rows, cols, eps, (hipStream_t)stream, 0.f, 0, rowmap, yc,
                  crows);
}

extern "C" int mmgl_add_layernorm_tiles_fwd(const void* x, const void* res, const void* gamma, const void* beta, void* sum_out, void* y,
                                            void* yc, const int32_t* rowmap, float* mean, float* rstd, int rows, int cols, int crows,
                                            float eps, float p_drop, uint64_t seed, int dtype, void* stream) {
    MMGL_CHECK_ARG(x && res && y, "mmgl_add_layernorm_tiles_fwd: null pointer");
    MMGL_CHECK_ARG(p_drop >= 0.f && p_drop < 1.f, "mmgl_add_layernorm_tiles_fwd: dropout p=%g outside [0,1)", p_drop);
    if (int rc = compact_check("mmgl_add_layernorm_tiles_fwd", rowmap, yc, rows, crows)) return rc;
    NORM_BY_DTYPE(norm_fwd, false, x, res, gamma, beta, sum_out, y, mean, rstd, rows, cols, eps, (hipStream_t)stream, p_drop, seed, rowmap,
                  yc, crows);
}

extern "C" int mmgl_add_layernorm_bwd(const void* dy, const void* dsum, const void* sum, const void* gamma, const float* mean,
                                      const float* rstd, void* dres, void* dx, float* dgamma, float* dbeta, void* workspace,
                                      size_t workspace_bytes, int rows, int cols, float p_drop, uint64_t seed, int dtype,
                                      void* stream) {
    MMGL_CHECK_ARG(dy && sum && mean && rstd && dres, "mmgl_add_layernorm_bwd: null pointer");
    MMGL_CHECK_ARG(p_drop >= 0.f && p_drop < 1.f, "mmgl_add_layernorm_bwd: dropout p=%g outside [0,1)", p_drop);
    MMGL_CHECK_ARG(p_drop == 0.f || dx, "mmgl_add_layernorm_bwd: dx is required when p_drop > 0");
    NORM_BY_DTYPE(norm_bwd, false, dy, sum, gamma, mean, rstd, dsum, dres, dgamma, dbeta, workspace, workspace_bytes, rows, cols,
                  (hipStream_t)stream, p_drop > 0.f ? dx : nullptr, p_drop, seed);
}

extern "C" int mmgl_layernorm_bwd(const void* dy, const void* x, const void* gamma, const float* mean, const float* rstd,
                                  void* dx, float* dgamma, float* dbeta, void* workspace, size_t workspace_bytes, int rows,
                                  int cols, int dtype, void* stream) {
    MMGL_CHECK_ARG(dy && x && mean && rstd && dx, "mmgl_layernorm_bwd: null pointer");
    NORM_BY_DTYPE(norm_bwd, false, dy, x, gamma, mean, rstd, nullptr, dx, dgamma, dbeta, workspace, workspace_bytes, rows, cols,
                  (hipStream_t)stream);
}

extern "C" int mmgl_rmsnorm_fwd(const void* x, const void* gamma, void* y, float* rstd, int rows, int cols, float eps,
                                int dtype, void* stream) {
    MMGL_CHECK_ARG(x && y && rstd, "mmgl_rmsnorm_fwd: null pointer");
    NORM_BY_DTYPE(norm_fwd, true, x, nullptr, gamma, nullptr, nullptr, y, nullptr, rstd, rows, cols, eps, (hipStream_t)stream);
}

extern "C" int mmgl_add_rmsnorm_fwd(const void* x, const void* res, const void* gamma, void* sum_out, void* y, float* rstd, int rows,
                                    int cols, float eps, int dtype, void* stream) {
    MMGL_CHECK_ARG(x && res && sum_out && y && rstd, "mmgl_add_rmsnorm_fwd: null pointer");
    NORM_BY_DTYPE(norm_fwd, true, x, res, gamma, nullptr, sum_out, y, nullptr, rstd, rows, cols, eps, (hipStream_t)stream);
}

extern "C" int mmgl_add_rmsnorm_bwd(const void* dy, const void* dsum, const void* sum, const void* gamma, const float* rstd, void* dres,
                                    float* dgamma, void* workspace, size_t workspace_bytes, int rows, int cols, int dtype, void* stream) {
    MMGL_CHECK_ARG(dy && sum && rstd && dres, "mmgl_add_rmsnorm_bwd: null pointer");
    NORM_BY_DTYPE(norm_bwd, true, dy, sum, gamma, nullptr, rstd, dsum, dres, dgamma, nullptr, workspace, workspace_bytes, rows, cols,
                  (hipStream_t)stream);
}

extern "C" int mmgl_rmsnorm_bwd(const void* dy, const void* x, const void* gamma, const float* rstd, void* dx,
                                float* dgamma, void* workspace, size_t workspace_bytes, int rows, int cols, int dtype,
                                void* stream) {
    MMGL_CHECK_ARG(dy && x && rstd && dx, "mmgl_rmsnorm_bwd: null pointer");
    NORM_BY_DTYPE(norm_bwd, true, dy, x, gamma, nullptr, rstd, nullptr, dx, dgamma, nullptr, workspace, workspace_bytes, rows, cols,
                  (hipStream_t)stream);
}
```

### mmgl_amd/model/modelling_cross_attention.py

```python
import math
import os
from typing import List, Optional, Tuple, Union

import torch
import torch.nn as nn
import torch.nn.functional as F
from transformers import (AutoConfig, AutoModelForCausalLM, CLIPTextModel, CLIPVisionModel, PretrainedConfig,
                          RobertaModel)
from transformers.activations import ACT2FN
from transformers.modeling_outputs import BaseModelOutputWithPast, CausalLMOutputWithPast

from .. import ops
from .decode_cache import BeamState, DecodeCache, LookupState, StepCodes
from .encoders import ClipTextEncoder, PackedTextEncoder, PackedVisionEncoder
from .generation import beam_loop, check_prompt, contrastive_loop, decode_loop, lookup_loop, make_select
from .sampling import (check_contrastive, check_guidance, check_kv_cache, check_lookup, check_processors, check_sampling,
                       check_weight_dtype)

CROSS_MODES = ("cross_attention", "embedding")


def uses_cross_attention(neighbor_mode: str, peft_type: str = "flamingo") -> bool:
    return neighbor_mode == "cross_attention" or (neighbor_mode == "embedding" and peft_type == "flamingo")

# ... 84 lines not shown
class MPTAttention(nn.Module):

    def __init__(self, config, cross_attention):
        super().__init__()
        self.embed_dim = config.hidden_size
        self.num_heads = config.num_attention_heads
        self.dropout = config.attention_dropout
        self.head_dim = self.embed_dim // self.num_heads
        bias = config.enable_bias
        if self.head_dim * self.num_heads != self.embed_dim:
            raise ValueError(f"embed_dim must be divisible by num_heads (got `embed_dim`: {self.embed_dim}"
                             f" and `num_heads`: {self.num_heads}).")
        self.scaling = self.head_dim ** -0.5
        self.is_decoder = False
        self.k_proj = nn.Linear(self.embed_dim, self.embed_dim, bias=bias)
        self.q_proj = nn.Linear(self.embed_dim, self.embed_dim, bias=bias)
        self.out_proj = nn.Linear(self.embed_dim, self.embed_dim, bias=bias)
        self.cross_attention = cross_attention
        self.peft_type = config.peft_type
        self.v_proj = nn.Linear(self.embed_dim, self.embed_dim, bias=bias)

    def _forward_cross(self, hidden_states, neighbor_embeds, neighbor_attention_mask, layer_head_mask, output_attentions, kv_out=None):
        if neighbor_embeds is None:
            raise ValueError("cross-attention layer called without neighbor_embeds")
        general = layer_head_mask is not None or output_attentions or (self.training and self.dropout > 0)
        bsz, tgt_len, _ = hidden_states.shape
        src_len = neighbor_embeds.shape[1]
        if neighbor_attention_mask is None:
            key_valid = torch.ones(bsz, src_len, dtype=torch.uint8, device=hidden_states.device)
        else:
            key_valid = _key_valid_from(neighbor_attention_mask)
            if key_valid.shape != (bsz, src_len):
                raise ValueError(f"Attention mask should be of size {(bsz, 1, tgt_len, src_len)}, but is"
                                 f" {tuple(neighbor_attention_mask.shape)}")
        q = ops.linear(hidden_states, self.q_proj.weight, self.q_proj.bias, out_scale=self.scaling)
        k = ops.linear(neighbor_embeds, self.k_proj.weight, self.k_proj.bias)
        v = ops.linear(neighbor_embeds, self.v_proj.weight, self.v_proj.bias)
        if kv_out is not None:
            kv_out.append((k, v))
        attn_w = None
        if general:
            o, attn_w = ops.attn_general(q, k, v, key_valid, self.num_heads, causal=False, head_mask=layer_head_mask, p_drop=self.dropout,
                                         training=self.training, output_attentions=output_attentions)
        else:
            o = ops.xattn_core(q, k, v, key_valid, self.num_heads)
        return ops.linear(o, self.out_proj.weight, self.out_proj.bias), attn_w, None

    def _fused_qkv(self, ps, slot):
        if any(p is None or p.requires_grad for p in ps):
            return None
        key = tuple((p.data_ptr(), p._version, p.dtype) for p in ps)
        cache = self.__dict__.get(slot)
        if cache is None or cache[0] != key:
            with torch.no_grad():
                w = torch.cat([ps[0].float() * self.scaling, ps[1].float(), ps[2].float()], 0).to(ps[0].dtype).contiguous()
                b = torch.cat([ps[3].float() * self.scaling, ps[4].float(), ps[5].float()], 0).to(ps[0].dtype).contiguous()
            cache = (key, (w, b))
            self.__dict__[slot] = cache
        return cache[1]

    def key_tiles_route(self, x, key_tiles, layer_head_mask, output_attentions, past_key_value, kv_out):
        if key_tiles is None or self.cross_attention or past_key_value is not None or kv_out is not None:
            return False
        if layer_head_mask is not None or output_attentions or (self.training and self.dropout > 0):
            return False
        return ops.selfattn_tiles_supported(x, self.num_heads, key_tiles) and self._frozen_qkv() is not None

    def _frozen_qkv(self):
        q, k, v = self.q_proj, self.k_proj, self.v_proj
        if any(type(m) is not nn.Linear for m in (q, k, v)):
            return None
        return self._fused_qkv((q.weight, k.weight, v.weight, q.bias, k.bias, v.bias), "_qkv_cache")

    def _lora_qkv(self):
        q, k, v = self.q_proj, self.k_proj, self.v_proj
        if not (hasattr(q, "lora_A") and hasattr(v, "lora_A") and type(k) is nn.Linear) or q.r != v.r or q.scaling != v.scaling:
            return None
        if self.training and (getattr(q, "lora_dropout", 0.0) > 0.0 or getattr(v, "lora_dropout", 0.0) > 0.0):
            return None
        return self._fused_qkv((q.base_layer.weight, k.weight, v.base_layer.weight, q.base_layer.bias, k.bias, v.base_layer.bias),
                               "_lora_qkv_cache")

    def _forward_self(self, hidden_states, attention_mask, layer_head_mask, output_attentions, past_key_value=None, kv_out=None,
                      live=None):
        H, d = self.num_heads, self.embed_dim
        if attention_mask is None or attention_mask.dim() != 2:
            raise ValueError("self-attention takes the [bsz, seq_len] key mask (causality is implied); additive 4-D masks are "
                             f"not materialised on this path (got {None if attention_mask is None else tuple(attention_mask.shape)})")
        general = layer_head_mask is not None or output_attentions or (self.training and self.dropout > 0)
        if general and past_key_value is not None:
            raise ValueError("layer_head_mask / output_attentions / attention dropout together with a key / value prefix (prefix tuning) "
                             "are not implemented")
        fused = self._frozen_qkv()
        if live is not None:
            yc, key_tiles = live
            o = ops.frozen_selfattn_tiles(hidden_states, yc, *fused, attention_mask, key_tiles, H)
            return _lin(self.out_proj, o), None, None
        if general:
            if fused is not None:
                qkv = ops.frozen_linear(hidden_states, *fused)
                q, k, v = qkv[..., :d], qkv[..., d:2 * d], qkv[..., 2 * d:]
            else:
                q = _lin(self.q_proj, hidden_states) * self.scaling
                k, v = _lin(self.k_proj, hidden_states), _lin(self.v_proj, hidden_states)
            o, attn_w = ops.attn_general(q, k, v, attention_mask, H, causal=True, head_mask=layer_head_mask, p_drop=self.dropout,
                                         training=self.training, output_attentions=output_attentions)
            return _lin(self.out_proj, o), attn_w, None
        if past_key_value is not None:
            kp, vp = past_key_value
            B, T, _ = hidden_states.shape
            P = kp.shape[-2]
            if fused is not None:
                qkv = ops.frozen_linear(hidden_states, *fused)
                q, k, v = qkv[..., :d], qkv[..., d:2 * d], qkv[..., 2 * d:]
            else:
                q = _lin(self.q_proj, hidden_states) * self.scaling
                k, v = _lin(self.k_proj, hidden_states), _lin(self.v_proj, hidden_states)
            k = torch.cat([kp.to(k.dtype).expand(B, P, d), k], dim=1)
            v = torch.cat([vp.to(v.dtype).expand(B, P, d), v], dim=1)
            o = ops.selfattn_core_prefix(q, k, v, attention_mask, H, P)
        elif fused is not None:
            qkv = ops.frozen_linear(hidden_states, *fused)
            if kv_out is not None:
                self._file_kv(kv_out, qkv[..., d:2 * d], qkv[..., 2 * d:], qkv[..., d:])
            o = ops.selfattn_core_fused(qkv, attention_mask, H)
        elif (lq := self._lora_qkv()) is not None and ops.lora_qkv_supported(hidden_states, lq[0], self.q_proj.r):
            qkv = ops.lora_qkv(hidden_states, lq[0], lq[1], self.q_proj.lora_A, self.q_proj.lora_B, self.v_proj.lora_A, self.v_proj.lora_B,
                               self.q_proj.scaling, self.scaling)
            if kv_out is not None:
                self._file_kv(kv_out, qkv[..., d:2 * d], qkv[..., 2 * d:], qkv[..., d:])
            o = ops.selfattn_core_fused(qkv, attention_mask, H)
        else:
            if type(self.q_proj) is nn.Linear and self.q_proj.weight.requires_grad:
                q = ops.linear(hidden_states, self.q_proj.weight, self.q_proj.bias, out_scale=self.scaling)
            elif type(self.q_proj) is not nn.Linear and hasattr(self.q_proj, "lora_A"):
                q = self.q_proj(hidden_states, out_scale=self.scaling)
            else:
                q = _lin(self.q_proj, hidden_states) * self.scaling
            k, v = _lin(self.k_proj, hidden_states), _lin(self.v_proj, hidden_states)
            if kv_out is not None:
                self._file_kv(kv_out, k, v)
            o = ops.selfattn_core(q, k, v, attention_mask, H)
        return _lin(self.out_proj, o), None, None

    def _file_kv(self, kv_out, k, v, kv=None):
        if isinstance(kv_out, tuple):
            ops.kv_quantize(k, v, kv_out[0], kv_out[1], self.num_heads)
        elif kv is not None:
            kv_out[:, :kv.shape[1]].copy_(kv)
        else:
            kv_out[:, :k.shape[1], :k.shape[2]].copy_(k)
            kv_out[:, :k.shape[1], k.shape[2]:].copy_(v)

    def forward(self, hidden_states, attention_mask=None, neighbor_embeds=None, neighbor_attention_mask=None,
                past_key_value=None, layer_head_mask=None, output_attentions=False, kv_out=None, live=None):
        if self.cross_attention:
            return self._forward_cross(hidden_states, neighbor_embeds, neighbor_attention_mask, layer_head_mask, output_attentions, kv_out)
        return self._forward_self(hidden_states, attention_mask, layer_head_mask, output_attentions, past_key_value, kv_out, live)

    @staticmethod
    def _decode_proj(mod, x, out_scale=1.0, out=None):
        if type(mod) is not nn.Linear and hasattr(mod, "lora_A") and hasattr(mod, "decode"):
            return mod.decode(x, out_scale=out_scale, out=out)
        _plain(mod)
        return ops.decode_linear(x, mod.weight, mod.bias, out_scale=out_scale, out=out)

    def _decode_qkv(self, x, dst, w8=None):
        d = self.embed_dim
        fused = self._frozen_qkv()
        if w8 is not None:
            if fused is not None:
                w, b = fused
                key = self.__dict__["_qkv_cache"][0]
                q = ops.decode_linear_w8(x, *w8.get(self, "q", w[:d], key), b[:d])
                ops.decode_linear_w8(x, *w8.get(self, "kv", w[d:], key), b[d:], out=dst)
            else:
                q = ops.decode_linear_w8(x, *w8.get(self, "q", self.q_proj.weight), self.q_proj.bias, out_scale=self.scaling)
                ops.decode_linear_w8(x, *w8.get(self, "k", self.k_proj.weight), self.k_proj.bias, out=dst[:, :d])
                ops.decode_linear_w8(x, *w8.get(self, "v", self.v_proj.weight), self.v_proj.bias, out=dst[:, d:])
            return q
        if fused is not None:
            w, b = fused
            q = ops.decode_linear(x, w[:d], b[:d])
            ops.decode_linear(x, w[d:], b[d:], out=dst)
        else:
            q = self._decode_proj(self.q_proj, x, out_scale=self.scaling)
            ops.decode_linear(x, self.k_proj.weight, self.k_proj.bias, out=dst[:, :d])
            self._decode_proj(self.v_proj, x, out=dst[:, d:])
        return q

    def decode_self(self, x, cache, idx):
        _plain(self.k_proj, self.out_proj)
        dst = cache.new_kv(idx)
        if not cache.plain or cache.w8 is not None:
            _plain(self.q_proj, self.v_proj)
        return cache.attend_self(idx, self._decode_qkv(x, dst, cache.w8), dst, self.num_heads)

    def decode_cross(self, x, cache, idx):
        _plain(self.q_proj, self.out_proj)
        q = ops.decode_linear(x, self.q_proj.weight, self.q_proj.bias, out_scale=self.scaling)
        return cache.attend_cross(idx, q, self.num_heads)


class _Deferred:
    __slots__ = ("residual", "branch", "p_drop", "training")

    def __init__(self, residual, branch, p_drop=0.0, training=False):
        self.residual, self.branch, self.p_drop, self.training = residual, branch, p_drop, training


def _materialize(h, *_):
    return ops.gated_residual(h.residual, h.branch, None, h.p_drop, h.training) if isinstance(h, _Deferred) else h


class MPTDecoderLayer(nn.Module):

    def __init__(self, config, cross_attention=False):
        super().__init__()
        self.embed_dim = config.hidden_size
        self.self_attn = MPTAttention(config, cross_attention)
        self.do_layer_norm_before = config.do_layer_norm_before
        self.dropout = config.dropout
        self.activation_name = config.activation_function
        self.activation_fn = ACT2FN[config.activation_function]
        affine = config.layer_norm_elementwise_affine
        self.self_attn_layer_norm = nn.LayerNorm(self.embed_dim, elementwise_affine=affine)
        self.fc1 = nn.Linear(self.embed_dim, config.ffn_dim, bias=config.enable_bias)
        self.fc2 = nn.Linear(config.ffn_dim, self.embed_dim, bias=config.enable_bias)
        self.final_layer_norm = nn.LayerNorm(self.embed_dim, elementwise_affine=affine)
        self.cross_attention = cross_attention
        self.peft_type = config.peft_type
        if self.cross_attention and self.peft_type == "flamingo":
            self.tanh_layer1 = nn.Tanh()
            self.tanh_layer2 = nn.Tanh()
            self.gating1 = nn.Parameter(torch.tensor(0.0))
            self.gating2 = nn.Parameter(torch.tensor(0.0))

    def _ln(self, ln, x):
        return ops.layer_norm(x, ln.weight, ln.bias, ln.eps)

    def _ln_fanout(self, ln, x):
        if torch.is_grad_enabled() and x.requires_grad:
            return ops.layer_norm_fanout(x, ln.weight, ln.bias, ln.eps)
        return x, ops.layer_norm(x, ln.weight, ln.bias, ln.eps)

    def _ffn(self, x, frozen):
        if self.activation_name == "relu":
            return ops.relu_ffn(x, self.fc1.weight, self.fc1.bias, self.fc2.weight, self.fc2.bias, frozen=frozen)
        lin = _lin if frozen is None else lambda m, t: ops.linear(t, m.weight, m.bias)
        return lin(self.fc2, self.activation_fn(lin(self.fc1, x)))

    def _forward_cross(self, h, neighbor_embeds, neighbor_attention_mask, layer_head_mask, output_attentions, kv_out=None):
        gated = self.peft_type == "flamingo"
        residual, x = self._ln_fanout(self.self_attn_layer_norm, h) if self.do_layer_norm_before else (h, h)
        a, attn_w, _ = self.self_attn(x, neighbor_embeds=neighbor_embeds, neighbor_attention_mask=neighbor_attention_mask,
                                      layer_head_mask=layer_head_mask, output_attentions=output_attentions, kv_out=kv_out)
        h = ops.gated_residual(residual, a, self.gating1 if gated else None, self.dropout, self.training)
        if not self.do_layer_norm_before:
            h = self._ln(self.self_attn_layer_norm, h)
        residual, x = self._ln_fanout(self.final_layer_norm, h) if self.do_layer_norm_before else (h, h)
        x = self._ffn(x, frozen=False)
        h = ops.gated_residual(residual, x, self.gating2 if gated else None, self.dropout, self.training)
        if not self.do_layer_norm_before:
            h = self._ln(self.final_layer_norm, h)
        return h, attn_w

    def _forward_self(self, h, attention_mask, layer_head_mask, output_attentions, defer_residual=False, past_key_value=None, kv_out=None,
                      key_tiles=None):
        pre = self.do_layer_norm_before
        ln1, ln2 = self.self_attn_layer_norm, self.final_layer_norm
        pair = lambda x, r, ln: ops.add_layer_norm_pair(x, r, ln.weight, ln.bias, ln.eps, self.dropout, self.training)
        like = h.residual if isinstance(h, _Deferred) else h
        live = None
        if pre and self.self_attn.key_tiles_route(like, key_tiles, layer_head_mask, output_attentions, past_key_value, kv_out):
            if isinstance(h, _Deferred):
                h, x, yc = ops.add_layer_norm_tiles(h.branch, h.residual, ln1.weight, ln1.bias, ln1.eps, key_tiles, h.p_drop, h.training)
            else:
                h, x, yc = ops.layer_norm_tiles(h, ln1.weight, ln1.bias, ln1.eps, key_tiles)
            live = (yc, key_tiles)
        elif isinstance(h, _Deferred):
            if pre:
                h, x = ops.add_layer_norm_pair(h.branch, h.residual, ln1.weight, ln1.bias, ln1.eps, h.p_drop, h.training)
            else:
                h = x = _materialize(h)
        elif pre:
            h, x = self._ln_fanout(ln1, h)
        else:
            x = h
        residual = h
        a, attn_w, _ = self.self_attn(x, attention_mask=attention_mask, layer_head_mask=layer_head_mask,
                                      output_attentions=output_attentions, past_key_value=past_key_value, kv_out=kv_out, live=live)
        if pre:
            h, x = pair(a, residual, ln2)
        else:
            _, h = pair(a, residual, ln1)
            x = h
        residual = h
        x = self._ffn(x, frozen=None)
        if pre and defer_residual:
            return _Deferred(residual, x, self.dropout, self.training), attn_w
        if not pre:
            _, h = pair(x, residual, ln2)
            return h, attn_w
        return ops.gated_residual(residual, x, None, self.dropout, self.training), attn_w

    def forward(self, hidden_states, attention_mask=None, neighbor_embeds=None, neighbor_attention_mask=None,
                layer_head_mask=None, past_key_value=None, output_attentions=False, use_cache=False, defer_residual=False, kv_out=None,
                key_tiles=None):
        if self.cross_attention:
            h, attn_w = self._forward_cross(_materialize(hidden_states), neighbor_embeds, neighbor_attention_mask, layer_head_mask,
                                            output_attentions, kv_out)
        else:
            h, attn_w = self._forward_self(hidden_states, attention_mask, layer_head_mask, output_attentions, defer_residual, past_key_value,
                                           kv_out, key_tiles)
        outputs = (h,)
        if output_attentions:
            outputs += (attn_w,)
        if use_cache:
            outputs += (None,)
        return outputs


    def _decode_ffn(self, x, w8=None):
        if self.activation_name == "relu":
            return _decode_linear(self, "fc1", x, w8, act="relu")
        return ops.activation_(_decode_linear(self, "fc1", x, w8), self.activation_name)

    def decode_step(self, h, cache, idx):
        pre = self.do_layer_norm_before
        attn = self.self_attn
        ln1, ln2 = self.self_attn_layer_norm, self.final_layer_norm
        _plain(self.fc1, self.fc2, attn.out_proj)
        x = self._ln(ln1, h) if pre else h
        gated = self.cross_attention
        w8 = None if gated else cache.w8
        if gated:
            g1, g2 = (self.gating1, self.gating2) if self.peft_type == "flamingo" else (None, None)
            a = attn.decode_cross(x, cache, idx)
            h = ops.gated_residual(h, ops.decode_linear(a, attn.out_proj.weight, attn.out_proj.bias), g1, 0.0, False)
        else:
            h = _decode_linear(self, "out_proj", attn.decode_self(x, cache, idx), w8, residual=h)
        if not pre:
            h = self._ln(ln1, h)
        x = self._decode_ffn(self._ln(ln2, h) if pre else h, w8)
        if gated:
            h = ops.gated_residual(h, ops.decode_linear(x, self.fc2.weight, self.fc2.bias), g2, 0.0, False)
        else:
            h = _decode_linear(self, "fc2", x, w8, residual=h)
        return h if pre else self._ln(ln2, h)


class MPTPreTrainedModel(nn.Module):
    config_class = MPTConfig
    base_model_prefix = "model"

    def __init__(self, config):
        super().__init__()
        self.config = config

    def _init_weights(self, module):
        std = self.config.init_std
        if isinstance(module, nn.Linear):
            module.weight.data.normal_(mean=0.0, std=std)
            if module.bias is not None:
                module.bias.data.zero_()
        elif isinstance(module, nn.Embedding):
            module.weight.data.normal_(mean=0.0, std=std)
            if module.padding_idx is not None:
                module.weight.data[module.padding_idx].zero_()

    def post_init(self):
        self.apply(self._init_weights)


class MPTDecoder(MPTPreTrainedModel):

    def __init__(self, config: MPTConfig):
        super().__init__(config)
        self.dropout = config.dropout
        self.layerdrop = config.layerdrop
# ... 76 lines not shown
            prefix_len = past_key_values[0][0].shape[-2]
            if self.cross_attention:
                raise ValueError("a key/value prefix is only defined for the plain (self-attention) decoder")
        if input_ids is not None and inputs_embeds is not None:
            raise ValueError("You cannot specify both decoder_input_ids and decoder_inputs_embeds at the same time")
        elif input_ids is not None:
            input_shape = input_ids.size()
            input_ids = input_ids.view(-1, input_shape[-1])
        elif inputs_embeds is not None:
            input_shape = inputs_embeds.size()[:-1]
        else:
            raise ValueError("You have to specify either decoder_input_ids or decoder_inputs_embeds")
        if inputs_embeds is None:
            inputs_embeds = self.embed_tokens(input_ids)
        batch_size, seq_length = input_shape
        rows = slice(None)
        if use_cache and cache_rows is not None:
            cache, r0 = cache_rows
            rows = slice(r0, r0 + batch_size)
            if kv_dtype is not None or cache.kv_scale is not None or seq_length > cache.capacity or rows.stop > cache.mask.shape[0]:
                raise ValueError(f"decode cache: rows [{r0}, {rows.stop}) x {seq_length} columns do not fit a cache of "
                                 f"{cache.mask.shape[0]} rows x {cache.capacity} columns in the model's dtype")
        elif use_cache:
            capacity = self.max_target_positions if cache_capacity is None else int(cache_capacity)
            if seq_length > capacity or capacity > self.max_target_positions:
                raise ValueError(f"decode cache: a prompt of {seq_length} columns, capacity {capacity}, max_position_embeddings "
                                 f"{self.max_target_positions}")
            cache = DecodeCache(len(self.layers), batch_size, capacity, self.config.hidden_size, inputs_embeds.dtype, inputs_embeds.device,
                                kv_dtype, self.config.num_attention_heads)
        if attention_mask is None:
            attention_mask = torch.ones(batch_size, seq_length + prefix_len, device=inputs_embeds.device)
        elif attention_mask.shape[1] == seq_length and prefix_len:
            attention_mask = torch.cat([attention_mask.new_ones(batch_size, prefix_len), attention_mask], dim=1)
        elif attention_mask.shape[1] != seq_length + prefix_len:
            raise ValueError(f"The provided attention mask has length {attention_mask.shape[1]}, but its length should be "
                             f"{seq_length + prefix_len} (sum of the lengths of current and past inputs)")
        if not first_key_valid:
            torch._assert_async((attention_mask[:, 0] != 0).all(),
                                "MPTDecoder: attention_mask[:, 0] must be 1 for every sample (right-padded sequences)")
        causal_attention_mask = (attention_mask != 0).to(torch.uint8).contiguous()
        key_valid = None
        if neighbor_attention_mask is not None:
            key_valid = _key_valid_from(neighbor_attention_mask).to(torch.uint8).contiguous()
        if neighbor_embeds is not None and neighbor_embeds.dtype != inputs_embeds.dtype:
            neighbor_embeds = neighbor_embeds.to(inputs_embeds.dtype)

        pos_embeds = self.embed_positions(attention_mask, prefix_len)
        if self.project_in is not None:
            inputs_embeds = _lin(self.project_in, inputs_embeds)
        hidden_states = inputs_embeds + pos_embeds

        all_hidden_states = () if output_hidden_states else None
        all_self_attns = () if output_attentions else None
        if head_mask is not None and head_mask.size()[0] != len(self.layers):
            raise ValueError(f"The `head_mask` should be specified for {len(self.layers)} layers, but it is for"
                             f" {head_mask.size()[0]}.")

        defer = not output_hidden_states
        for idx, decoder_layer in enumerate(self.layers):
            if output_hidden_states:
                all_hidden_states += (hidden_states,)
            if self.training and self.layerdrop > 0:
                if torch.rand([]) < self.layerdrop:
                    continue
            lhm = head_mask[idx] if head_mask is not None else None
            layer_outputs = decoder_layer(hidden_states, attention_mask=causal_attention_mask, layer_head_mask=lhm,
                                          output_attentions=output_attentions, defer_residual=defer,
                                          past_key_value=None if past_key_values is None else past_key_values[idx],
                                          kv_out=None if cache is None else cache.kv_out(idx) if cache_rows is None else cache.kv[idx][rows],
                                          key_tiles=key_tiles)
            if self.cross_attention and neighbor_embeds is not None and (idx + 1) % self.neighbor_layer_wise == 0:
                hidden_states = _materialize(layer_outputs[0])
                neighbor_idx = (idx + 1) // self.neighbor_layer_wise - 1
                layer_outputs = self.neighbor_layers[neighbor_idx](
                    hidden_states, attention_mask=causal_attention_mask, neighbor_embeds=neighbor_embeds,
                    neighbor_attention_mask=key_valid, layer_head_mask=lhm, output_attentions=output_attentions,
                    kv_out=None if cache is None else cache.cross)
            hidden_states = layer_outputs[0]
            if output_attentions:
                all_self_attns += (layer_outputs[1],)

        if self.final_layer_norm is not None:
            fln = self.final_layer_norm
            if isinstance(hidden_states, _Deferred):
                _, hidden_states = ops.add_layer_norm_pair(hidden_states.branch, hidden_states.residual, fln.weight, fln.bias, fln.eps,
                                                           hidden_states.p_drop, hidden_states.training)
            else:
                hidden_states = ops.layer_norm(hidden_states, fln.weight, fln.bias, fln.eps)
        hidden_states = _materialize(hidden_states)
        if self.project_out is not None:
            hidden_states = _lin(self.project_out, hidden_states)
        if output_hidden_states:
            all_hidden_states += (hidden_states,)
        if cache is not None:
            cache.mask[rows, :seq_length] = causal_attention_mask
            cache.col = seq_length
            next_pos = causal_attention_mask.sum(dim=1, dtype=torch.int64) + self.embed_positions.offset
            if cache_rows is None:
                cache.next_pos = next_pos
            else:
                cache.next_pos[rows] = next_pos
            if cache.cross and (cache_rows is None or neighbor_embeds is not None):
                cache.cross_valid = key_valid if key_valid is not None else torch.ones(cache.cross[0][0].shape[:2], dtype=torch.uint8,
                                                                                       device=hidden_states.device)
        if not return_dict:
            return tuple(v for v in [hidden_states, cache, all_hidden_states, all_self_attns] if v is not None)
        return BaseModelOutputWithPast(last_hidden_state=hidden_states, past_key_values=cache,
                                       hidden_states=all_hidden_states, attentions=all_self_attns)

    def prefill_guided(self, input_ids, attention_mask, neighbor_embeds, neighbor_attention_mask, first_key_valid=False,
                       cache_capacity=None):
        B, T = input_ids.shape
        capacity = self.max_target_positions if cache_capacity is None else int(cache_capacity)
        if T > capacity or capacity > self.max_target_positions:
            raise ValueError(f"decode cache: a prompt of {T} columns, capacity {capacity}, max_position_embeddings {self.max_target_positions}")
        w = self.embed_tokens.weight
        cache = DecodeCache(len(self.layers), 2 * B, capacity, self.config.hidden_size, w.dtype, w.device)
        cache.pairs = B
        cache.next_pos = torch.empty(2 * B, dtype=torch.int64, device=w.device)
        last = []
        for r0, ne, nm in ((0, neighbor_embeds, neighbor_attention_mask), (B, None, None)):
            out = self(input_ids=input_ids, attention_mask=attention_mask, neighbor_embeds=ne, neighbor_attention_mask=nm, use_cache=True,
                       first_key_valid=first_key_valid, cache_rows=(cache, r0))
            last.append(out.last_hidden_state[:, -1])
        if len(cache.cross) != len(self.neighbor_layers) or not cache.cross:
            raise ValueError("guidance_scale: the decoder ran no gated layer on the neighbors: there is nothing to contrast")
        return torch.cat(last, dim=0), cache

    def _decode_step(self, input_ids, inputs_embeds, cache, output_hidden_states, return_dict):
        if (input_ids is None) == (inputs_embeds is None):
            raise ValueError("You have to specify either decoder_input_ids or decoder_inputs_embeds")
        shape = input_ids.shape if input_ids is not None else inputs_embeds.shape[:2]
        beam = cache.beam
        rows = cache.mask.shape[0] * (1 if beam is None else beam.W)
        if len(shape) != 2 or shape[1] != 1 or shape[0] != rows:
            raise ValueError(f"a decode step takes one new token per cached " + ("sample" if beam is None else "beam")
                             + f" ([{rows}, 1]), got {tuple(shape)}")
        if cache.next_pos is None:
            raise ValueError("the DecodeCache has not been filled: run the prompt with use_cache=True first")
        if beam is not None:
            if beam.n_tail >= beam.n_cap or cache.col + beam.n_tail >= self.max_target_positions:
                raise ValueError(f"beam tail is full: column {beam.n_tail} of capacity {beam.n_cap} behind {cache.col} prompt columns "
                                 f"(max_position_embeddings {self.max_target_positions})")
        elif cache.col >= cache.capacity or cache.col >= self.max_target_positions:
            raise ValueError(f"decode cache is full: column {cache.col} of capacity {cache.capacity} "
                             f"(max_position_embeddings {self.max_target_positions})")
        ops.require_cuda(cache.mask, input_ids, inputs_embeds)
        with torch.no_grad():
            emb = self.embed_tokens(input_ids[:, 0]) if inputs_embeds is None else inputs_embeds[:, 0]
            pos = cache.next_pos if beam is None else cache.next_pos.repeat_interleave(beam.W)
            if beam is None:
                cache.mask[:, cache.col] = 1
            layer_inputs = [] if output_hidden_states else None
            h = self._decode_rows(emb, pos, cache, layer_inputs)
            if beam is None:
                cache.col += 1
            else:
                beam.n_tail += 1
            cache.next_pos = cache.next_pos + 1
        h = h[:, None]
        all_hidden_states = tuple(x[:, None] for x in layer_inputs) + (h,) if output_hidden_states else None
        if not return_dict:
            return tuple(v for v in [h, cache, all_hidden_states] if v is not None)
        return BaseModelOutputWithPast(last_hidden_state=h, past_key_values=cache, hidden_states=all_hidden_states, attentions=None)

    def _decode_rows(self, emb, positions, cache, layer_inputs=None):
        if self.project_in is not None:
# ... 583 lines not shown
```

### mmgl_amd/ops.py

```python
import math
import os
import weakref

import torch
import torch.nn.functional as F

from . import _lib
from ._lib import dtype_code, lib, ptr, ptr_off, require_cuda, stream_ptr


def _dropout(p_drop, training, seed):
    p = float(p_drop) if training else 0.0
    if p > 0.0 and seed is None:
        seed = int(torch.randint(0, 2 ** 62, (1,)).item())
    return p, int(seed or 0)


def _check_mask(key_valid, shape):
    if key_valid.shape != shape:
        raise ValueError(f"Attention mask should be of size {tuple(shape)}, but is {tuple(key_valid.shape)}")


def _key_valid(key_valid):
    if key_valid.dtype != torch.uint8:
# ... 233 lines not shown
        qkv, key_valid, out, lse = ctx.saved_tensors
        H, Hkv = ctx.heads
        B, T, ld = qkv.shape
        D = ld // (H + 2 * Hkv)
        es = qkv.element_size()
        dqkv = torch.empty_like(qkv)
        _gqa_bwd(qkv, dout, ptr(qkv), ptr_off(qkv, H * D * es), ptr_off(qkv, (H + Hkv) * D * es), out, lse, key_valid,
                 ptr(dqkv), ptr_off(dqkv, H * D * es), ptr_off(dqkv, (H + Hkv) * D * es), B, T, H, Hkv, D, ld, ld, ld, ld)
        return dqkv, None, None, None


def _kv_heads(op, num_heads, num_kv_heads):
    if num_kv_heads is None or num_kv_heads == num_heads:
        return None
    if num_kv_heads < 1 or num_heads % num_kv_heads:
        raise ValueError(f"{op}: num_heads = {num_heads} must be a multiple of num_kv_heads = {num_kv_heads}")
    return int(num_kv_heads)


def selfattn_core_fused(qkv, key_valid, num_heads, num_kv_heads=None):
    Hkv = _kv_heads("selfattn_core_fused", num_heads, num_kv_heads)
    if Hkv is not None:
        if qkv.dim() != 3 or qkv.shape[2] % (num_heads + 2 * Hkv):
            raise ValueError(f"selfattn_core_fused: qkv{tuple(qkv.shape)} is not [B, T, (H+2*Hkv)*D] for H={num_heads}, Hkv={Hkv}")
        _check_mask(key_valid, qkv.shape[:2])
        return _SelfAttnFusedGQA.apply(qkv, _key_valid(key_valid), num_heads, Hkv)
    if qkv.dim() != 3 or qkv.shape[2] % (3 * num_heads):
        raise ValueError(f"selfattn_core_fused: qkv{tuple(qkv.shape)} is not [B, T, 3*H*D] for H={num_heads}")
    _check_mask(key_valid, qkv.shape[:2])
    return _SelfAttnFusedQKV.apply(qkv, _key_valid(key_valid), num_heads)


def selfattn_core(q, k, v, key_valid, num_heads, num_kv_heads=None):
    Hkv = _kv_heads("selfattn_core", num_heads, num_kv_heads)
    if Hkv is not None:
        if (q.dim() != 3 or k.dim() != 3 or k.shape != v.shape or q.shape[:2] != k.shape[:2] or q.shape[2] % num_heads
                or k.shape[2] != q.shape[2] // num_heads * Hkv):
            raise ValueError(f"selfattn_core: incompatible shapes q{tuple(q.shape)} k{tuple(k.shape)} v{tuple(v.shape)} for H={num_heads}, Hkv={Hkv}")
        _check_mask(key_valid, k.shape[:2])
        return _SelfAttnGQA.apply(q, k, v, _key_valid(key_valid), num_heads, Hkv)
    _attn_args("selfattn_core", q, k, v, key_valid, num_heads, 0)
    return _SelfAttn.apply(q, k, v, _key_valid(key_valid), num_heads, None)


def selfattn_core_prefix(q, k, v, key_valid, num_heads, prefix_len):
    _attn_args("selfattn_core_prefix", q, k, v, key_valid, num_heads, prefix_len, f" for a prefix of {prefix_len}")
    return _SelfAttn.apply(q, k, v, _key_valid(key_valid), num_heads, int(prefix_len))


KEY_TILE = 64


def key_tile_table(attention_mask):
    am = attention_mask.cpu() != 0
    B, T = am.shape
    if T == 0 or T % KEY_TILE:
        return None, 0
    live = am.view(B, T // KEY_TILE, KEY_TILE).any(dim=-1).reshape(-1)
    index = torch.cumsum(live.to(torch.int32), 0, dtype=torch.int32) - 1
    table = torch.where(live, index, torch.full_like(index, -1)).view(B, T // KEY_TILE).contiguous()
    return table, KEY_TILE * int(live.sum())


class KeyTiles:
    __slots__ = ("table", "rowmap", "m_live")

    def __init__(self, table, m_live, device):
        self.table = table.to(device=device, dtype=torch.int32, non_blocking=True).contiguous()
        self.m_live = int(m_live)
        t = self.table.view(-1, 1)
        rows = t * KEY_TILE + torch.arange(KEY_TILE, dtype=torch.int32, device=self.table.device)
        self.rowmap = torch.where(t >= 0, rows, torch.full_like(rows, -1)).reshape(-1).contiguous()

    def fits(self, B, T):
        return self.m_live > 0 and tuple(self.table.shape) == (B, T // KEY_TILE) and T % KEY_TILE == 0


def selfattn_tiles_supported(like, num_heads, tiles):
    B, T, d = like.shape
    return (tiles is not None and like.is_cuda and like.dtype == torch.bfloat16 and d == 64 * num_heads and T <= 4096
            and tiles.fits(B, T))


def layer_norm_tiles(x, gamma, beta, eps, tiles):
    if torch.is_grad_enabled() and x.requires_grad:
        return _NormPair.apply(x, None, gamma, beta, float(eps), False, 0.0, 0, tiles)
    yc = x.new_empty(tiles.m_live, x.shape[-1])
    with torch.no_grad():
        _, y, _, _, _ = _norm_fwd(False, x, None, gamma, beta, float(eps), compact=(tiles.rowmap, yc))
    return x, y.view(x.shape), yc


def add_layer_norm_tiles(x, res, gamma, beta, eps, tiles, p_drop=0.0, training=False, seed=None):
    if x.shape != res.shape:
        raise ValueError(f"add_layer_norm_tiles: shapes differ {tuple(x.shape)} vs {tuple(res.shape)}")
    return _NormPair.apply(x, res, gamma, beta, float(eps), False, *_dropout(p_drop, training, seed), tiles)


class _FrozenSelfAttnTiles(torch.autograd.Function):

    @staticmethod
    def forward(ctx, y, yc, w, b, key_valid, tiles, num_heads):
        require_cuda(y, yc, key_valid)
        B, T, d = y.shape
        m = tiles.m_live
        y2 = y.contiguous().view(-1, d)
        q = gemm_nt(y2, w[:d], None if b is None else b[:d], k_splits=False)
        kv = gemm_nt(yc, w[d:], None if b is None else b[d:], k_splits=False)
        out = torch.empty(B, T, d, dtype=y.dtype, device=y.device)
        lse = torch.empty(B, num_heads, T, dtype=torch.float32, device=y.device)
        es = y.element_size()
        work = dict(flops=2.0 * B * T * T * d, bytes=(2.0 * B * T * d + 2.0 * m * d) * es)
        _lib.call("mmgl_selfattn_tiles_fwd", work, ptr(q), ptr(kv), ptr_off(kv, d * es), ptr(key_valid), ptr(tiles.table), ptr(out), ptr(lse),
                  B, num_heads, T, d // num_heads, m, d, 2 * d, dtype_code(y), stream_ptr())
        ctx.save_for_backward(q, kv, key_valid, out, lse, w)
        ctx.tiles, ctx.num_heads = tiles, num_heads
        return out

    @staticmethod
    def backward(ctx, dout):
        q, kv, key_valid, out, lse, w = ctx.saved_tensors
        tiles, H = ctx.tiles, ctx.num_heads
        B, T, d = out.shape
        m, es = tiles.m_live, out.element_size()
        dout = dout.contiguous()
        dqkv = torch.empty(B, T, 3 * d, dtype=out.dtype, device=out.device)
        nbytes = lib().mmgl_selfattn_bwd_workspace(B, H, T)
        ws = torch.empty(nbytes, dtype=torch.uint8, device=out.device)
        work = dict(flops=5.0 * B * T * T * d, bytes=(6.0 * B * T * d + 2.0 * m * d) * es)
        _lib.call("mmgl_selfattn_tiles_bwd", work, ptr(dout), ptr(q), ptr(kv), ptr_off(kv, d * es), ptr(out), ptr(lse), ptr(key_valid),
                  ptr(tiles.table), ptr(dqkv), ptr_off(dqkv, d * es), ptr_off(dqkv, 2 * d * es), ptr(ws), nbytes, B, H, T, d // H, m, d, 2 * d,
                  3 * d, 3 * d, dtype_code(out), stream_ptr())
        return frozen_dgrad(dqkv.view(-1, 3 * d), w).view(B, T, d), None, None, None, None, None, None


def frozen_selfattn_tiles(y, yc, w, b, key_valid, tiles, num_heads):
    if not selfattn_tiles_supported(y, num_heads, tiles):
        raise ValueError(f"frozen_selfattn_tiles: y{tuple(y.shape)} {y.dtype} with {num_heads} heads is not a bf16 head_dim-64 batch "
                         f"whose [B, T // 64] table and m_live > 0 are given")
    if w.requires_grad or (b is not None and b.requires_grad) or w.shape != (3 * y.shape[2], y.shape[2]):
        raise ValueError("frozen_selfattn_tiles: w must be the frozen fused [3d, d] projection")
    if yc.shape != (tiles.m_live, y.shape[2]):
        raise ValueError(f"frozen_selfattn_tiles: yc{tuple(yc.shape)} is not [m_live = {tiles.m_live}, d]")
    _check_mask(key_valid, y.shape[:2])
    return _FrozenSelfAttnTiles.apply(y, yc, w, b, _key_valid(key_valid), tiles, num_heads)


def _ws(nbytes, device):
    return torch.empty(max(int(nbytes), 16), dtype=torch.uint8, device=device)


def _norm_fwd(rms, x, res, gamma, beta, eps, p=0.0, seed=0, keep_sum=True, keep_stats=True, compact=None):
    require_cuda(x, res)
    cols = x.shape[-1]
    x2 = x.contiguous().view(-1, cols)
    rows = x2.shape[0]
    y = torch.empty_like(x2)
    mean = torch.empty(rows, dtype=torch.float32, device=x.device) if keep_stats and not rms else None
    rstd = torch.empty(rows, dtype=torch.float32, device=x.device) if keep_stats else None
    g = None if gamma is None else gamma.to(x.dtype).contiguous()
    b = None if beta is None else beta.to(x.dtype).contiguous()
    if compact is not None:
        rowmap, yc = compact
        if rms or rowmap.numel() != rows:
            raise ValueError(f"_norm_fwd: the compact copy is LayerNorm's, with one map entry per row ({rowmap.numel()} for {rows} rows)")
        work = dict(bytes=((2.0 if res is None else 3.0 + keep_sum) * rows * cols + yc.numel()) * x.element_size())
        if res is None:
            s = x2
            _lib.call("mmgl_layernorm_tiles_fwd", work, ptr(x2), ptr(g), ptr(b), ptr(y), ptr(yc), ptr(rowmap), ptr(mean), ptr(rstd), rows,
                      cols, yc.shape[0], eps, dtype_code(x), stream_ptr())
        else:
            r2 = res.contiguous().view(-1, cols)
            s = torch.empty_like(x2) if keep_sum else None
            _lib.call("mmgl_add_layernorm_tiles_fwd", work, ptr(x2), ptr(r2), ptr(g), ptr(b), ptr(s), ptr(y), ptr(yc), ptr(rowmap), ptr(mean),
                      ptr(rstd), rows, cols, yc.shape[0], eps, p, seed, dtype_code(x), stream_ptr())
    elif res is None:
        s = x2
        work = dict(bytes=2.0 * rows * cols * x.element_size())
        if rms:
            _lib.call("mmgl_rmsnorm_fwd", work, ptr(x2), ptr(g), ptr(y), ptr(rstd), rows, cols, eps, dtype_code(x), stream_ptr())
        else:
            _lib.call("mmgl_layernorm_fwd", work, ptr(x2), ptr(g), ptr(b), ptr(y), ptr(mean), ptr(rstd), rows, cols, eps, dtype_code(x),
                      stream_ptr())
    else:
        r2 = res.contiguous().view(-1, cols)
        s = torch.empty_like(x2) if keep_sum else None
        work = dict(bytes=(3.0 + keep_sum) * rows * cols * x.element_size())
        if rms:
            _lib.call("mmgl_add_rmsnorm_fwd", work, ptr(x2), ptr(r2), ptr(g), ptr(s), ptr(y), ptr(rstd), rows, cols, eps, dtype_code(x),
                      stream_ptr())
        else:
            _lib.call("mmgl_add_layernorm_fwd", work, ptr(x2), ptr(r2), ptr(g), ptr(b), ptr(s), ptr(y), ptr(mean), ptr(rstd), rows, cols,
                      eps, p, seed, dtype_code(x), stream_ptr())
    return s, y, g, mean, rstd


def _norm_bwd(rms, fused, dy, dsum, s, g, mean, rstd, pgrad, pdtype, p=0.0, seed=0):
    rows, cols = s.shape
    dy = dy.contiguous().view(rows, cols)
    dsum = None if dsum is None else dsum.contiguous().view(rows, cols)
    ds = torch.empty_like(s)
    dx = torch.empty_like(s) if p > 0.0 else None
    want = any(pgrad)
    dgamma = torch.empty(cols, dtype=torch.float32, device=s.device) if want else None
    dbeta = torch.empty(cols, dtype=torch.float32, device=s.device) if want and not rms else None
    nbytes = lib().mmgl_norm_bwd_workspace(rows, cols) if want else 0
    ws = torch.empty(nbytes, dtype=torch.uint8, device=s.device) if want else None
    work = dict(bytes=(3.0 + (dsum is not None) + (dx is not None)) * rows * cols * s.element_size())
    if not fused:
        if rms:
            _lib.call("mmgl_rmsnorm_bwd", work, ptr(dy), ptr(s), ptr(g), ptr(rstd), ptr(ds), ptr(dgamma), ptr(ws), nbytes, rows, cols,
                      dtype_code(s), stream_ptr())
        else:
            _lib.call("mmgl_layernorm_bwd", work, ptr(dy), ptr(s), ptr(g), ptr(mean), ptr(rstd), ptr(ds), ptr(dgamma), ptr(dbeta), ptr(ws),
                      nbytes, rows, cols, dtype_code(s), stream_ptr())
    elif rms:
        _lib.call("mmgl_add_rmsnorm_bwd", work, ptr(dy), ptr(dsum), ptr(s), ptr(g), ptr(rstd), ptr(ds), ptr(dgamma), ptr(ws), nbytes, rows,
                  cols, dtype_code(s), stream_ptr())
    else:
        _lib.call("mmgl_add_layernorm_bwd", work, ptr(dy), ptr(dsum), ptr(s), ptr(g), ptr(mean), ptr(rstd), ptr(ds), ptr(dx), ptr(dgamma),
                  ptr(dbeta), ptr(ws), nbytes, rows, cols, p, seed, dtype_code(s), stream_ptr())
    return ds, dx, (dgamma.to(pdtype) if pgrad[0] else None), (dbeta.to(pdtype) if pgrad[1] else None)


def _norm_ctx(ctx, rms, shape, gamma, beta, p=0.0, seed=0):
    pgrad = (gamma is not None and gamma.requires_grad, beta is not None and beta.requires_grad)
    ctx.cfg = (rms, shape, pgrad, None if gamma is None else gamma.dtype, p, seed)


class _Norm(torch.autograd.Function):

    @staticmethod
    def forward(ctx, x, gamma, beta, eps, rms):
        x2, y, g, mean, rstd = _norm_fwd(rms, x, None, gamma, beta, eps)
        ctx.save_for_backward(x2, g, mean, rstd)
        _norm_ctx(ctx, rms, x.shape, gamma, beta)
        return y.view(x.shape)

    @staticmethod
    def backward(ctx, dy):
        x2, g, mean, rstd = ctx.saved_tensors
        rms, shape, pgrad, pdtype, _, _ = ctx.cfg
        dx, _, dg, db = _norm_bwd(rms, False, dy, None, x2, g, mean, rstd, pgrad, pdtype)
        return dx.view(shape), dg, db, None, None


class _NormPair(torch.autograd.Function):

    @staticmethod
    def forward(ctx, x, res, gamma, beta, eps, rms, p, seed, tiles):
        yc = None if tiles is None else x.new_empty(tiles.m_live, x.shape[-1])
        s, y, g, mean, rstd = _norm_fwd(rms, x, res, gamma, beta, eps, p, seed, compact=None if tiles is None else (tiles.rowmap, yc))
        ctx.save_for_backward(s, g, mean, rstd)
        ctx.set_materialize_grads(False)
        _norm_ctx(ctx, rms, x.shape, gamma, beta, p, seed)
        ctx.fanout = res is None
        outs = (x if res is None else s.view(x.shape)), y.view(x.shape)
        if tiles is None:
            return outs
        ctx.mark_non_differentiable(yc)
        return outs + (yc,)

    @staticmethod
    def backward(ctx, ds, dy, _dyc=None):
        s, g, mean, rstd = ctx.saved_tensors
        rms, shape, pgrad, pdtype, p, seed = ctx.cfg
        if dy is None:
            if ds is None or p == 0.0:
                return ds, (None if ctx.fanout else ds), None, None, None, None, None, None, None
            dy = torch.zeros_like(ds)
        dres, dx, dg, db = _norm_bwd(rms, True, dy, ds, s, g, mean, rstd, pgrad, pdtype, p, seed)
        dres = dres.view(shape)
        if ctx.fanout:
            return dres, None, dg, db, None, None, None, None, None
        return (dres if dx is None else dx.view(shape)), dres, dg, db, None, None, None, None, None


def layer_norm(x, gamma, beta, eps=1e-5):
    return _Norm.apply(x, gamma, beta, float(eps), False)


def layer_norm_fanout(x, gamma, beta, eps=1e-5):
    return _NormPair.apply(x, None, gamma, beta, float(eps), False, 0.0, 0, None)


def add_layer_norm_pair(x, res, gamma, beta, eps=1e-5, p_drop=0.0, training=False, seed=None):
    if x.shape != res.shape:
        raise ValueError(f"add_layer_norm_pair: shapes differ {tuple(x.shape)} vs {tuple(res.shape)}")
    return _NormPair.apply(x, res, gamma, beta, float(eps), False, *_dropout(p_drop, training, seed), None)


def rms_norm(x, gamma, eps=1e-6):
    return _Norm.apply(x, gamma, None, float(eps), True)


def add_rms_norm_pair(x, res, gamma, eps=1e-6):
    if x.shape != res.shape:
        raise ValueError(f"add_rms_norm_pair: shapes differ {tuple(x.shape)} vs {tuple(res.shape)}")
    return _NormPair.apply(x, res, gamma, None, float(eps), True, 0.0, 0, None)


class _GatedResidual(torch.autograd.Function):
    @staticmethod
    def forward(ctx, residual, x, gate, p_drop, seed):
        require_cuda(residual, x)
        residual, x = residual.contiguous(), x.contiguous()
        y = torch.empty_like(x)
        g32 = None if gate is None else gate.detach().to(torch.float32).reshape(1).contiguous()
        _lib.call("mmgl_gated_residual_fwd", dict(bytes=3.0 * x.numel() * x.element_size()), ptr(residual), ptr(x), ptr(g32), ptr(y), x.numel(), p_drop, seed,
                                            dtype_code(x), stream_ptr())
        ctx.save_for_backward(x, g32)
        ctx.p, ctx.seed = p_drop, seed
        ctx.gate_meta = None if gate is None else (gate.dtype, gate.shape, gate.requires_grad)
        return y

    @staticmethod
    def backward(ctx, dy):
        x, g32 = ctx.saved_tensors
        dy = dy.contiguous()
        dx = torch.empty_like(x)
        dgate = torch.zeros(1, dtype=torch.float32, device=x.device) if g32 is not None else None
        ws = _ws(lib().mmgl_gated_residual_bwd_workspace(x.numel()), x.device)
        _lib.call("mmgl_gated_residual_bwd", dict(bytes=3.0 * x.numel() * x.element_size()), ptr(dy), ptr(x), ptr(g32), ptr(dx), ptr(dgate), ptr(ws), ws.numel(), x.numel(),
                                            ctx.p, ctx.seed, dtype_code(x), stream_ptr())
        dg = None
        if ctx.gate_meta is not None and ctx.gate_meta[2]:
            dg = dgate.to(ctx.gate_meta[0]).reshape(ctx.gate_meta[1])
        return dy, dx, dg, None, None


def gated_residual(residual, x, gate=None, p_drop=0.0, training=False, seed=None):
    return _GatedResidual.apply(residual, x, gate, *_dropout(p_drop, training, seed))


_ACTS = {"none": _lib.ACT_NONE, "relu": _lib.ACT_RELU}


def _act_code(op, act):
    code = _ACTS.get(act)
    if code is None:
        raise ValueError(f"{op}: activation {act!r} is not fused (supported: none, relu)")
    return code


def _mfma_aligned(gemm, x, w, bias=None, residual=None, zmask=None, act=0, out_scale=1.0, out=None):
    N, K = w.shape
    kq = 8 if x.dtype == torch.bfloat16 else 4
    if K % kq == 0 and N % 8 == 0:
        return gemm(x, w, bias, residual, zmask, act, out_scale, K, out)
    pk, pn = (-K) % kq, (-N) % 8
    x = F.pad(x, (0, pk)) if pk else x
    w = F.pad(w, (0, pk, 0, pn))
    bias, residual, zmask = (F.pad(c, (0, pn)) if (pn and c is not None) else c for c in (bias, residual, zmask))
    y = gemm(x, w, bias, residual, zmask, act, out_scale, K + pk, None)
    y = y[..., :N] if pn else y
    return y if out is None else out.copy_(y)


class _Linear(torch.autograd.Function):
    @staticmethod
    def forward(ctx, x, weight, bias, act, out_scale, mask_dx=False, premasked=False):
        require_cuda(x, weight)
        shape = x.shape
        K = shape[-1]
        N = weight.shape[0]
        x2 = x.contiguous().view(-1, K)
# ... 352 lines not shown
            return wt.contiguous()
        full = wt.new_zeros(wt.shape[0], npad)
        full[:, :n] = wt
        return full


def _transposed(weight, pad_to=1):
    key = (id(weight), pad_to)
    tag = (weight.data_ptr(), weight._version, weight.dtype, tuple(weight.shape))
    hit = _WT_CACHE.get(key)
    if hit is None or hit[0]() is not weight or hit[1] != tag:
        if len(_WT_CACHE) > 4096:
            for k in [k for k, h in _WT_CACHE.items() if h[0]() is None]:
                del _WT_CACHE[k]
        hit = (weakref.ref(weight), tag, _padded_t(weight, pad_to))
        _WT_CACHE[key] = hit
    return hit[2]


_tile_counters = {}


def gemm_dynamic_schedule(enable=True, device=None):
    device = torch.device("cuda", torch.cuda.current_device()) if device is None else torch.device(device)
    with torch.cuda.device(device):
        if not enable:
            lib().mmgl_gemm_set_tile_counter(None)
            return None
        c = _tile_counters.get(device)
        if c is None:
            c = _tile_counters[device] = torch.zeros(16, dtype=torch.int32, device=device)
        lib().mmgl_gemm_set_tile_counter(ptr(c))
    return c


def gemm_nt(x2, w, bias=None, residual=None, zmask=None, act=0, out_scale=1.0, K=None, out=None, k_splits=True):
    require_cuda(x2, w)
    M, N = x2.shape[0], w.shape[0]
    K = x2.shape[1] if K is None else K
    if x2.stride(1) != 1 or w.stride(1) != 1:
        raise ValueError("gemm_nt: operands need unit column stride")
    y = torch.empty(M, N, dtype=x2.dtype, device=x2.device) if out is None else out
    if M == 0:
        return y
    for name, t in (("zmask", zmask), ("residual", residual)):
        if t is not None and (t.stride(1) != 1 or t.stride(0) != y.stride(0)):
            raise ValueError(f"gemm_nt: {name} must share the output's row stride ({t.stride(0)} vs {y.stride(0)})")
    nws = lib().mmgl_gemm_nt_workspace(M, N, K, x2.stride(0), w.stride(0), y.stride(0), dtype_code(x2)) if k_splits else 0
    ws = torch.empty(nws, dtype=torch.uint8, device=x2.device) if nws else None
    _lib.call("mmgl_gemm_nt", dict(flops=2.0 * M * N * K, bytes=float(M * K + N * K + M * N) * x2.element_size(),
                                   tag=f"{M}x{N}x{K}" + ("+b" if bias is not None else "") + ("+z" if zmask is not None else "")
                                       + ("+r" if residual is not None else "") + (f"+a{act}" if act else "")),
              ptr(x2), x2.stride(0), ptr(w), w.stride(0), ptr(bias), ptr(residual), ptr(zmask), ptr(y), y.stride(0), M, N, K, act,
              float(out_scale), ptr(ws), nws, dtype_code(x2), stream_ptr())
    return y


def relu_bits_bytes(M, N, K, ldx, ldw, ldy, dtype):
    if dtype != torch.bfloat16:
        return 0
    return lib().mmgl_gemm_nt_relu_bits_bytes(M, N, K, ldx, ldw, ldy, _lib.BF16)


def gemm_nt_relu_bits(x2, w, bias, out, K=None):
    M, N = x2.shape[0], w.shape[0]
    K = x2.shape[1] if K is None else K
    nb = relu_bits_bytes(M, N, K, x2.stride(0), w.stride(0), out.stride(0), x2.dtype)
    if not nb:
        raise ValueError("gemm_nt_relu_bits: shape not eligible (relu_bits_bytes == 0)")
    bits = torch.empty(nb, dtype=torch.uint8, device=x2.device)
    _lib.call("mmgl_gemm_nt_relu_bits", dict(flops=2.0 * M * N * K, bytes=float(M * K + N * K + M * N) * x2.element_size(), tag=f"{M}x{N}x{K}+b+a1+bits"),
              ptr(x2), x2.stride(0), ptr(w), w.stride(0), ptr(bias), ptr(out), out.stride(0), ptr(bits), M, N, K, 1.0, dtype_code(x2), stream_ptr())
    return out, bits


def gemm_nt_masked(x2, w, bits, out, K=None):
    M, N = x2.shape[0], w.shape[0]
    K = x2.shape[1] if K is None else K
    _lib.call("mmgl_gemm_nt_masked", dict(flops=2.0 * M * N * K, bytes=float(M * K + N * K + M * N) * x2.element_size(), tag=f"{M}x{N}x{K}+bits"),
              ptr(x2), x2.stride(0), ptr(w), w.stride(0), ptr(bits), ptr(out), out.stride(0), M, N, K, 1.0, dtype_code(x2), stream_ptr())
    return out


def _dgrad_pad_to(g, weight):
    N, K = weight.shape
    if N % 128 == 0 or not (g.dtype == weight.dtype == torch.bfloat16):
        return 1
    npad = N + (-N) % 128
    return 128 if lib().mmgl_gemm_nt_fast(g.shape[0], K, npad, g.stride(0), npad, K, _lib.BF16) else 1


def frozen_dgrad(g, weight, zmask=None, out=None, bits=None, out_scale=1.0, residual=None, wt=None):
    if wt is None:
        if weight.dtype == g.dtype:
            wt = _transposed(weight, _dgrad_pad_to(g, weight))
        else:
            wt = weight.detach().to(g.dtype).t().contiguous()
    if out is None:
        K = wt.shape[0]
        ld = K if zmask is None else zmask.stride(0)
        out = g.new_empty(g.shape[0], ld)
        out = out[:, :K] if ld != K else out
    if bits is not None:
        return gemm_nt_masked(g, wt, bits, out, K=wt.shape[1])
    return _mfma_aligned(gemm_nt, g, wt, residual=residual, zmask=zmask, out_scale=out_scale, out=out)


def _ffn_pitch(M, N, K, dtype):
    if dtype != torch.bfloat16 or (N * 2) % 8192:
        return N
    P, L = N + 128, lib()
    if L.mmgl_gemm_nt_fast(M, N, K, K, K, P, _lib.BF16) == 1 and L.mmgl_gemm_nt_fast(M, K, N, P, N, K, _lib.BF16) == 1:
        return P
    return N


_CU_COUNT = {}


def _round_split_rows(M, N, device):
    G = _CU_COUNT.get(device.index)
    if G is None:
        G = _CU_COUNT[device.index] = torch.cuda.get_device_properties(device).multi_processor_count
    tm, tn = (M + 255) // 256, (N + 255) // 256
    rounds, rem = divmod(tm * tn, G)
    if not (1 <= rounds <= 3 and 0 < rem <= G // 4) or (rounds * G) % tn:
        return 0
    m1 = rounds * G // tn * 256
    return m1 if 0 < m1 < M else 0


def _row_strided(t2, cols, n_out):
    if t2.is_contiguous():
        return t2
    if (t2.stride(1) == 1 and t2.stride(0) >= cols and t2.stride(0) % 8 == 0 and t2.dtype == torch.bfloat16
            and lib().mmgl_gemm_nt_fast(t2.shape[0], n_out, cols, t2.stride(0), cols, n_out, _lib.BF16)):
        return t2
    return t2.contiguous()


class _FrozenLinear(torch.autograd.Function):
    @staticmethod
    def forward(ctx, x, weight, bias, act):
        N, K = weight.shape
        x2 = _row_strided(x.reshape(-1, K), K, N)
        out = torch.empty(*x.shape[:-1], N, dtype=x.dtype, device=x.device)
        _mfma_aligned(gemm_nt, x2, weight.to(x.dtype).contiguous(), None if bias is None else bias.to(x.dtype), act=act, out=out.view(-1, N))
        ctx.save_for_backward(weight, out if act == 1 else None)
        return out

    @staticmethod
    def backward(ctx, dy):
        weight, y = ctx.saved_tensors
        N, K = weight.shape
        g = dy.reshape(-1, N)
        g = _row_strided(g, N, K) if y is None else g.contiguous()
        if y is not None:
            gm = torch.empty_like(g)
            _lib.call("mmgl_relu_bwd", dict(bytes=3.0 * g.numel() * g.element_size()), ptr(g), ptr(y), ptr(gm), g.numel(), dtype_code(g), stream_ptr())
            g = gm
        return frozen_dgrad(g, weight).reshape(*dy.shape[:-1], K), None, None, None


def frozen_linear(x, weight, bias, act="none"):
    if weight.requires_grad or (bias is not None and bias.requires_grad):
        raise ValueError("frozen_linear: weight and bias must be frozen (requires_grad=False)")
    if x.shape[-1] != weight.shape[1]:
        raise ValueError(f"frozen_linear: x has {x.shape[-1]} features, weight expects {weight.shape[1]}")
    return _FrozenLinear.apply(x, weight, bias, _act_code("frozen_linear", act))


class _FrozenReluFFN(torch.autograd.Function):

    @staticmethod
    def forward(ctx, x, w1, b1, w2, b2):
        (F_, K), N = w1.shape, w2.shape[0]
        x2 = x.contiguous().reshape(-1, K)
        M = x2.shape[0]
        pitch = _ffn_pitch(M, F_, K, x.dtype)
        rows = nb = 0
        if pitch != F_:
            rows = _round_split_rows(M, F_, x.device)
            nb = relu_bits_bytes(rows, F_, K, K, K, pitch, x.dtype) if rows else 0
            if not nb:
                rows, nb = M, relu_bits_bytes(M, F_, K, K, K, pitch, x.dtype)
        w, b = w1.to(x.dtype).contiguous(), None if b1 is None else b1.to(x.dtype)
        h = x.new_empty(M, pitch)[:, :F_]
        if nb:
            _, bits = gemm_nt_relu_bits(x2[:rows], w, b, h[:rows])
            if rows < M:
                gemm_nt(x2[rows:], w, b, act=1, out=h[rows:])
        else:
            _mfma_aligned(gemm_nt, x2, w, b, act=1, out=h)
        hx = _row_strided(h, F_, N)
        y = x.new_empty(*x.shape[:-1], N)
        _mfma_aligned(gemm_nt, hx, w2.to(x.dtype).contiguous(), None if b2 is None else b2.to(x.dtype), out=y.view(-1, N))
        mask, ctx.mask_bits = hx, None
        if nb and hx.stride(0) == pitch and N % 128 == 0 and relu_bits_bytes(rows, F_, N, N, N, pitch, x.dtype) == nb:
            mask, ctx.mask_bits = None, (bits, pitch, rows)
            if rows < M:
                mask = x.new_empty(M - rows, pitch)[:, :F_].copy_(hx[rows:])
        ctx.save_for_backward(w1, w2, mask)
        h = h.view(*x.shape[:-1], F_)
        ctx.mark_non_differentiable(h)
        ctx.set_materialize_grads(False)
        return y, h

    @staticmethod
    def backward(ctx, dy, _dh=None):
        w1, w2, mask = ctx.saved_tensors
        (F_, K), N = w1.shape, w2.shape[0]
        g = _row_strided(dy.reshape(-1, N), N, F_)
        if ctx.mask_bits is None:
            dh = frozen_dgrad(g, w2, zmask=mask)
        else:
            bits, pitch, rows = ctx.mask_bits
            dh = g.new_empty(g.shape[0], pitch)[:, :F_]
            frozen_dgrad(g[:rows], w2, out=dh[:rows], bits=bits)
            if rows < g.shape[0]:
                frozen_dgrad(g[rows:], w2, zmask=mask, out=dh[rows:])
        return frozen_dgrad(_row_strided(dh, F_, K), w1).reshape(*dy.shape[:-1], K), None, None, None, None


def relu_ffn(x, w1, b1, w2, b2, frozen=None, return_hidden=False):
    if x.shape[-1] != w1.shape[1] or w1.shape[0] != w2.shape[1]:
        raise ValueError(f"relu_ffn: x has {x.shape[-1]} features, fc1 maps {w1.shape[1]} to {w1.shape[0]}, fc2 expects {w2.shape[1]}")
    trainable = any(p is not None and p.requires_grad for p in (w1, b1, w2, b2))
    if frozen and trainable:
        raise ValueError("relu_ffn: weight and bias must be frozen (requires_grad=False)")
    if trainable or frozen is False:
        h = _linear(x, w1, b1, _lib.ACT_RELU, premasked=True)
        y = _linear(h, w2, b2, _lib.ACT_NONE, mask_dx=True)
    else:
        y, h = _FrozenReluFFN.apply(x, w1, b1, w2, b2)
    return (y, h) if return_hidden else y


class _RopeQK(torch.autograd.Function):

    @staticmethod
    def forward(ctx, qkv, cos_sin, unit, nblk, nall):
        require_cuda(qkv, cos_sin)
        B, T, ld = qkv.shape
        D = ld // nall // unit
        if not qkv.is_contiguous():
            raise ValueError("rope_qk_: qkv must be contiguous")
        _lib.call("mmgl_rope_inplace", dict(bytes=2.0 * B * T * (nblk * ld // nall) * qkv.element_size()), ptr(qkv), ptr(cos_sin), B * T, T, unit, D, ld, nblk, 0,
                  dtype_code(qkv), stream_ptr())
        ctx.mark_dirty(qkv)
        ctx.save_for_backward(cos_sin)
        ctx.meta = (T, unit, D, nblk, nall)
        return qkv

    @staticmethod
    def backward(ctx, dqkv):
        (cos_sin,) = ctx.saved_tensors
        T, H, D, nblk, nall = ctx.meta
        dqkv = dqkv.contiguous()
        out = torch.empty_like(dqkv)
        rows = dqkv.numel() // dqkv.shape[-1]
        _lib.call("mmgl_rope", dict(bytes=2.0 * rows * dqkv.shape[-1] * dqkv.element_size()), ptr(dqkv), ptr(out), ptr(cos_sin), rows, T, H, D,
                  dqkv.shape[-1], nblk, nall, 1, dtype_code(dqkv), stream_ptr())
        return out, None, None, None, None


def rope_qk_(qkv, cos_sin, num_heads, num_kv_heads=None):
    Hkv = _kv_heads("rope_qk_", num_heads, num_kv_heads)
    if Hkv is not None:
        if qkv.dim() != 3 or qkv.shape[2] % (num_heads + 2 * Hkv):
            raise ValueError(f"rope_qk_: qkv{tuple(qkv.shape)} is not [B, T, (H+2*Hkv)*D] for H={num_heads}, Hkv={Hkv}")
        D, G = qkv.shape[2] // (num_heads + 2 * Hkv), num_heads // Hkv
        unit, nblk, nall = Hkv, G + 1, G + 2
    else:
        if qkv.dim() != 3 or qkv.shape[2] % (3 * num_heads):
            raise ValueError(f"rope_qk_: qkv{tuple(qkv.shape)} is not [B, T, 3*H*D] for H={num_heads}")
        D = qkv.shape[2] // 3 // num_heads
        unit, nblk, nall = num_heads, 2, 3
    if cos_sin.dtype != torch.float32 or tuple(cos_sin.shape) != (qkv.shape[1], D // 2, 2):
        raise ValueError(f"rope_qk_: cos_sin must be fp32 [T={qkv.shape[1]}, D/2={D // 2}, 2], got {cos_sin.dtype} {tuple(cos_sin.shape)}")
    return _RopeQK.apply(qkv, cos_sin.contiguous(), unit, nblk, nall)


class _SwiGLU(torch.autograd.Function):
    @staticmethod
    def forward(ctx, gu):
        require_cuda(gu)
        F2 = gu.shape[-1]
        g2 = gu.contiguous().view(-1, F2)
        y = torch.empty(g2.shape[0], F2 // 2, dtype=gu.dtype, device=gu.device)
        _lib.call("mmgl_swiglu_fwd", dict(bytes=1.5 * g2.numel() * g2.element_size()), ptr(g2), ptr(y), g2.shape[0], F2 // 2, dtype_code(g2), stream_ptr())
        ctx.save_for_backward(g2)
        ctx.shape = gu.shape
        return y.view(*gu.shape[:-1], F2 // 2)

    @staticmethod
    def backward(ctx, dy):
        (g2,) = ctx.saved_tensors
        M, F2 = g2.shape
        dy2 = dy.contiguous().view(M, F2 // 2)
        dgu = torch.empty_like(g2)
        _lib.call("mmgl_swiglu_bwd", dict(bytes=2.5 * g2.numel() * g2.element_size()), ptr(dy2), ptr(g2), ptr(dgu), M, F2 // 2, dtype_code(g2), stream_ptr())
        return dgu.view(ctx.shape)


def swiglu(gate_up):
    if gate_up.shape[-1] % 2:
        raise ValueError("swiglu: last dim must be 2*F")
    return _SwiGLU.apply(gate_up)


def encoder_attention(q, k, v, cu_seqlens, num_heads, max_len, q_rows=None, work=None):
    require_cuda(q, k, v, cu_seqlens)
    ntok, hd = q.shape
    if k.shape != q.shape or v.shape != q.shape or hd % num_heads:
        raise ValueError(f"encoder_attention: incompatible shapes q{tuple(q.shape)} k{tuple(k.shape)} v{tuple(v.shape)} H={num_heads}")
# ... 761 lines not shown
```

Baseline: 290.2 samples/s.

## Fuse residual add and dropout into frozen GEMM epilogue with precomputed keep masks

Adds a gemm8p epilogue mode (ACT=6) that adds the residual, optionally applying a dropout keep-mask and scale, right after bf16 rounding of the GEMM output. The keep bitmap for the next dropout is generated inside the preceding layernorm kernel, and a presummed layernorm path consumes the already-summed tensor. This targets the separate elementwise add/dropout pass and its extra memory traffic in the frozen decoder blocks. In exchange there are new kernel instantiations, restrictions on shape (whole tiles, no split-K), and extra keep-map storage and loads.

```diff
diff --git a/include/mmgl_hip.h b/include/mmgl_hip.h
--- a/include/mmgl_hip.h
+++ b/include/mmgl_hip.h
@@ -134,6 +134,9 @@
                            int M, int N, int K, float out_scale, int dtype, void* stream);
 int mmgl_gemm_nt_masked(const void* x, int ldx, const void* W, int ldw, const void* bits_in, void* y, int ldy, int M, int N, int K,
                         float out_scale, int dtype, void* stream);
+int mmgl_gemm_nt_add_fast(int M, int N, int K, int ldx, int ldw, int ldy, int dtype);
+int mmgl_gemm_nt_add(const void* x, int ldx, const void* W, int ldw, const void* bias, const void* residual, const void* keep,
+                     void* y, int ldy, int M, int N, int K, float p_drop, int dtype, void* stream);
 
 int mmgl_rope_inplace(void* buf, const float* cos_sin, size_t rows, int T, int H, int D, int ld, int nblk, int backward,
                       int dtype, void* stream);
@@ -156,6 +159,11 @@
 int mmgl_add_layernorm_tiles_fwd(const void* x, const void* res, const void* gamma, const void* beta, void* sum_out, void* y,
                                  void* yc, const int32_t* rowmap, float* mean, float* rstd, int rows, int cols, int crows,
                                  float eps, float p_drop, uint64_t seed, int dtype, void* stream);
+int mmgl_layernorm_keep_fwd(const void* x, const void* gamma, const void* beta, void* y, float* mean, float* rstd, void* keep_out,
+                            int rows, int cols, float eps, float p_next, uint64_t seed_next, int dtype, void* stream);
+int mmgl_layernorm_tiles_keep_fwd(const void* x, const void* gamma, const void* beta, void* y, void* yc, const int32_t* rowmap,
+                                  float* mean, float* rstd, void* keep_out, int rows, int cols, int crows, float eps, float p_next,
+                                  uint64_t seed_next, int dtype, void* stream);
 int mmgl_activation_fwd(const void* x, void* y, size_t n, int act, int dtype, void* stream);
 int mmgl_scale(const void* x, const float* scale, void* y, size_t n, int dtype, void* stream);
 
diff --git a/mmgl_amd/_lib.py b/mmgl_amd/_lib.py
--- a/mmgl_amd/_lib.py
+++ b/mmgl_amd/_lib.py
@@ -62,6 +62,8 @@
     "mmgl_add_layernorm_bwd": (I, [P, P, P, P, P, P, P, P, P, P, P, Z, I, I, F, U, I, P]),
     "mmgl_layernorm_tiles_fwd": (I, [P, P, P, P, P, P, P, P, I, I, I, F, I, P]),
     "mmgl_add_layernorm_tiles_fwd": (I, [P, P, P, P, P, P, P, P, P, P, I, I, I, F, F, U, I, P]),
+    "mmgl_layernorm_keep_fwd": (I, [P, P, P, P, P, P, P, I, I, F, F, U, I, P]),
+    "mmgl_layernorm_tiles_keep_fwd": (I, [P, P, P, P, P, P, P, P, P, I, I, I, F, F, U, I, P]),
     "mmgl_activation_fwd": (I, [P, P, Z, I, I, P]),
     "mmgl_scale": (I, [P, P, P, Z, I, P]),
     "mmgl_gemm_nt_fast": (I, [I, I, I, I, I, I, I]),
@@ -70,6 +72,8 @@
     "mmgl_gemm_nt_relu_bits": (I, [P, I, P, I, P, P, I, P, I, I, I, F, I, P]),
     "mmgl_gemm_nt_masked": (I, [P, I, P, I, P, P, I, I, I, I, F, I, P]),
     "mmgl_gemm_nt": (I, [P, I, P, I, P, P, P, P, I, I, I, I, I, F, P, Z, I, P]),
+    "mmgl_gemm_nt_add_fast": (I, [I, I, I, I, I, I, I]),
+    "mmgl_gemm_nt_add": (I, [P, I, P, I, P, P, P, P, I, I, I, I, F, I, P]),
     "mmgl_relu_bwd": (I, [P, P, P, Z, I, P]),
     "mmgl_gemm_set_tile_counter": (I, [P]),
     "mmgl_gemm_get_tile_counter": (P, []),
diff --git a/mmgl_amd/csrc/gemm.hip b/mmgl_amd/csrc/gemm.hip
--- a/mmgl_amd/csrc/gemm.hip
+++ b/mmgl_amd/csrc/gemm.hip
@@ -902,6 +902,24 @@
                          (hipStream_t)stream, nullptr, 0, nullptr, (const unsigned*)bits_in);
 }
 
+extern "C" int mmgl_gemm_nt_add_fast(int M, int N, int K, int ldx, int ldw, int ldy, int dtype) {
+    if (N % 64 || nt_route(M, N, K, ldx, ldw, ldy, dtype, false) != NtRoute::P8) return 0;
+    return gemm8p_row_split(M, N, K, ldx, ldw, ldy) == 0 && gemm8p_splits(M, N, K) == 0;
+}
+
+extern "C" int mmgl_gemm_nt_add(const void* x, int ldx, const void* W, int ldw, const void* bias, const void* residual, const void* keep,
+                                void* y, int ldy, int M, int N, int K, float p_drop, int dtype, void* stream) {
+    MMGL_CHECK_ARG(x && W && y && residual, "mmgl_gemm_nt_add: null pointer");
+    MMGL_CHECK_ARG(ldx + 127 >= K && ldw >= K && ldy >= N, "mmgl_gemm_nt_add: leading dimensions (%d, %d, %d) smaller than the rows (K=%d, N=%d)", ldx, ldw, ldy, K, N);
+    MMGL_CHECK_ARG(p_drop >= 0.f && p_drop < 1.f && (p_drop > 0.f) == (keep != nullptr),
+                   "mmgl_gemm_nt_add: dropout p=%g outside [0,1), or a keep map without dropout / dropout without a keep map", p_drop);
+    MMGL_CHECK_ARG(mmgl_gemm_nt_add_fast(M, N, K, ldx, ldw, ldy, dtype) == 1,
+                   "mmgl_gemm_nt_add: shape M=%d N=%d K=%d (ld %d %d %d, dtype %d) does not run as whole tiles of the persistent kernel", M, N, K, ldx, ldw, ldy, dtype);
+    const float keep_scale = p_drop > 0.f ? 1.f / (1.f - p_drop) : 1.f;
+    return launch_gemm8p((const bf16*)x, ldx, (const bf16*)W, ldw, (bf16*)y, ldy, (const bf16*)bias, (const bf16*)residual, nullptr, M, N, K,
+                         MMGL_ACT_NONE, 1.f, (hipStream_t)stream, nullptr, 0, nullptr, nullptr, 1, (const unsigned char*)keep, keep_scale);
+}
+
 extern "C" int mmgl_relu_bwd(const void* dy, const void* y, void* out, size_t n, int dtype, void* stream) {
     MMGL_CHECK_ARG(dy && y && out, "mmgl_relu_bwd: null pointer");
     hipStream_t st = (hipStream_t)stream;
diff --git a/mmgl_amd/csrc/gemm8p.h b/mmgl_amd/csrc/gemm8p.h
--- a/mmgl_amd/csrc/gemm8p.h
+++ b/mmgl_amd/csrc/gemm8p.h
@@ -7,7 +7,8 @@
 size_t gemm8p_split_bytes(int M, int N, int K);
 int launch_gemm8p(const bf16* X, int ldx, const bf16* W, int ldw, bf16* Y, int ldy, const bf16* bias, const bf16* resid,
                   const bf16* zmask, int M, int N, int K, int act, float scale, hipStream_t st, float* part = nullptr,
-                  size_t part_bytes = 0, unsigned* bits_out = nullptr, const unsigned* bits_in = nullptr);
+                  size_t part_bytes = 0, unsigned* bits_out = nullptr, const unsigned* bits_in = nullptr, int add_rounded = 0,
+                  const unsigned char* keep = nullptr, float keep_scale = 1.f);
 inline size_t gemm8p_bits_bytes(int M, int N) { return (size_t)cdiv(M, 256) * cdiv(N, 256) * 8192; }
 
 int gemm8p_tt_splits(int RA, int RB, int M);
diff --git a/mmgl_amd/csrc/gemm8p.hip b/mmgl_amd/csrc/gemm8p.hip
--- a/mmgl_amd/csrc/gemm8p.hip
+++ b/mmgl_amd/csrc/gemm8p.hip
@@ -8,6 +8,7 @@
 
 typedef __attribute__((address_space(3))) void lds_void;
 typedef unsigned p8_u32x4 __attribute__((ext_vector_type(4)));
+typedef unsigned p8_u32x2 __attribute__((ext_vector_type(2)));
 
 constexpr int P8_UNIT = 16384;
 constexpr int P8_LDS = 8 * P8_UNIT;
@@ -34,6 +35,8 @@
     long long* trace;
     int trace_wg;
     unsigned* sched;
+    const unsigned char* keep;
+    float keep_scale;
 };
 
 __device__ __forceinline__ int p8_fetch_item(unsigned* sched, int xcd, int nlists, int G, int Gx, int nitems) {
@@ -254,7 +257,28 @@
         const __amdgpu_buffer_rsrc_t dY = y_desc(a.Y, m0);
         bf16x8 pre[16];
         p8_u32x4 mbits = {0u, 0u, 0u, 0u};
-        if constexpr (ZR) {
+        p8_u32x2 kb[8];
+        auto fetch_resid = [&](int q) __attribute__((always_inline)) {
+            const __amdgpu_buffer_rsrc_t dR = y_desc(a.resid, m0);
+            const int J0 = (q == 0 || q == 1) ? 0 : 4, T0 = (q == 0 || q == 3) ? 0 : 2;
+#pragma unroll
+            for (int j = 0; j < 4; ++j)
+                pre[q * 4 + j] = __builtin_bit_cast(bf16x8, __builtin_amdgcn_raw_buffer_load_b128(dR, y_off(J0 + j, T0), 0, 0));
+        };
+        if constexpr (ACT == 6) {
+            if (a.keep) {
+                const int kld = a.N >> 3;
+                long long rem = (long long)(a.M - m0) * kld;
+                if (rem > 0xffffffffLL) rem = 0xffffffffLL;
+                const __amdgpu_buffer_rsrc_t dK = __builtin_amdgcn_make_buffer_rsrc((void*)(a.keep + (size_t)m0 * kld), 0, (int)(unsigned)rem, 0x00020000);
+                const unsigned kbase = (unsigned)((wr * 128 + (ln & 15)) * kld + ((n0 + wc * 64) >> 3));
+#pragma unroll
+                for (int J = 0; J < 8; ++J)
+                    kb[J] = __builtin_amdgcn_raw_buffer_load_b64(dK, n0 + wc * 64 < a.N ? kbase + (unsigned)(J * 16 * kld) : 0xffffffffu, 0, P8_ZMASK_AUX);
+            }
+            fetch_resid(0);
+            fetch_resid(1);
+        } else if constexpr (ZR) {
             const __amdgpu_buffer_rsrc_t dZ = y_desc(a.zmask ? a.zmask : a.resid, m0);
             if (a.bits_in) {
                 mbits = *(const p8_u32x4*)(a.bits_in + ((size_t)((a.tile0 + vcur) * 8 + wave) * 64 + ln) * 4);
@@ -293,12 +317,15 @@
             unsigned qbits = 0;
             auto rows = [&](auto mode_tag) __attribute__((always_inline)) {
                 constexpr int MODE = decltype(mode_tag)::value;
+                unsigned sbase = base;
+                if constexpr (ACT == 6) asm volatile("" : "+v"(sbase));
 #pragma unroll
                 for (int j = 0; j < 4; ++j) {
-                    const unsigned off = y_off(J0 + j, T0);
+                    const unsigned off = ACT == 6 ? ((T0 ? col_ok1 : col_ok0) ? sbase + (unsigned)(J0 + j) * rstep + (unsigned)(32 * T0) : 0xffffffffu)
+                                                  : y_off(J0 + j, T0);
                     const f32x4 lo = acc[T0][J0 + j], hi = acc[T0 + 1][J0 + j];
                     f32x8 v = {lo[0], lo[1], lo[2], lo[3], hi[0], hi[1], hi[2], hi[3]};
-                    if constexpr (ACT >= 2 || (ACT == 1 && ZR)) {
+                    if constexpr ((ACT >= 2 && ACT <= 4) || (ACT == 1 && ZR)) {
 #pragma unroll
                         for (int e = 0; e < 8; ++e) v[e] = p8_act<ACT>(v[e]);
                     }
@@ -315,6 +342,26 @@
                         for (int e = 0; e < 8; ++e) v[e] = (((float)z[e] > 0.f) ? v[e] : 0.f) + (float)rr[e];
                     }
                     p8_u32x4 ob = __builtin_bit_cast(p8_u32x4, __builtin_convertvector(v, bf16x8));
+                    if constexpr (MODE == 5 || MODE == 6) {
+                        if constexpr (MODE == 6) {
+                            const unsigned by = kb[J0 + j][T0 >> 1] >> (8 * (ln >> 4));
+#pragma unroll
+                            for (int e = 0; e < 4; ++e) {
+                                unsigned t = (by >> (2 * e)) & 3u;
+                                t = (t | (t << 15)) & 0x00010001u;
+                                unsigned mk;
+                                asm("v_pk_sub_u16 %0, 0, %1" : "=v"(mk) : "v"(t));
+                                ob[e] &= mk;
+                            }
+                        }
+                        const bf16x8 z = pre[q * 4 + j];
+#pragma unroll
+                        for (int e = 0; e < 4; ++e) {
+                            v[2 * e] = __builtin_fmaf(a.keep_scale, __builtin_bit_cast(float, ob[e] << 16), (float)z[2 * e]);
+                            v[2 * e + 1] = __builtin_fmaf(a.keep_scale, __builtin_bit_cast(float, ob[e] & 0xffff0000u), (float)z[2 * e + 1]);
+                        }
+                        ob = __builtin_bit_cast(p8_u32x4, __builtin_convertvector(v, bf16x8));
+                    }
                     if constexpr (ACT == 1 && !ZR) {
 #pragma unroll
                         for (int e = 0; e < 4; ++e) {
@@ -358,6 +405,11 @@
                 }
             };
             if constexpr (!ZR) rows(std::integral_constant<int, 0>());
+            else if constexpr (ACT == 6) {
+                if (a.keep) rows(std::integral_constant<int, 6>());
+                else rows(std::integral_constant<int, 5>());
+                if (q < 2) fetch_resid(q + 2);
+            }
             else if (a.bits_in) rows(std::integral_constant<int, 4>());
             else if (a.zmask && a.resid) rows(std::integral_constant<int, 3>());
             else if (a.zmask) rows(std::integral_constant<int, 1>());
@@ -602,7 +654,7 @@
 
 int launch_gemm8p(const bf16* X, int ldx, const bf16* W, int ldw, bf16* Y, int ldy, const bf16* bias, const bf16* resid,
                   const bf16* zmask, int M, int N, int K, int act, float scale, hipStream_t st, float* part, size_t part_bytes,
-                  unsigned* bits_out, const unsigned* bits_in) {
+                  unsigned* bits_out, const unsigned* bits_in, int add_rounded, const unsigned char* keep, float keep_scale) {
     if (!gemm8p_supported(M, N, K, ldx, ldw, ldy))
         MMGL_FAIL(MMGL_ERR_UNSUPPORTED, "gemm8p: shape M=%d N=%d K=%d (ld %d %d %d) not supported", M, N, K, ldx, ldw, ldy);
     P8Args a;
@@ -616,6 +668,13 @@
     if (bits_out && (act != 1 || resid || zmask)) MMGL_FAIL(MMGL_ERR_INVALID, "gemm8p: mask bits are written by the plain ReLU epilogue only");
     if (bits_in && (zmask || resid || act != 0)) MMGL_FAIL(MMGL_ERR_INVALID, "gemm8p: mask bits are applied by the plain epilogue only");
     if (bits_out || bits_in) part = nullptr;
+    a.keep = keep;
+    a.keep_scale = keep_scale;
+    if (add_rounded) {
+        if (!resid || zmask || bits_in || bits_out || act != 0 || scale != 1.f || N % 64)
+            MMGL_FAIL(MMGL_ERR_INVALID, "gemm8p: the rounded residual add takes a residual, no activation, no scale, no masks and N %% 64 == 0");
+        part = nullptr;
+    }
     const int n_cu = mmgl_num_cu();
     const int tiles = a.total;
     int direct = tiles, nsplit = 0;
@@ -638,6 +697,7 @@
         if (const char* e = getenv("MMGL_P8_TRACE_WG")) a.trace_wg = atoi(e);
 #endif
         const bool zr = resid || zmask || bits_in;
+        if (add_rounded) act = 6;
 #define P8_LAUNCH(A, Z)                                                                                     \
     do {                                                                                                    \
         if (int rc = mmgl_set_lds(gemm8p_kernel<A, Z>, P8_LDS_ALLOC, "gemm8p")) return rc;                  \
@@ -649,6 +709,7 @@
             case 2: if (zr) MMGL_FAIL(MMGL_ERR_UNSUPPORTED, "gemm8p: gelu(erf) with residual / zmask is not instantiated"); P8_LAUNCH(2, false); break;
             case 3: if (zr) P8_LAUNCH(3, true); else P8_LAUNCH(3, false); break;
             case 4: if (zr) P8_LAUNCH(4, true); else P8_LAUNCH(4, false); break;
+            case 6: P8_LAUNCH(6, true); break;
             default: MMGL_FAIL(MMGL_ERR_INVALID, "gemm8p: unknown activation %d", act);
         }
 #undef P8_LAUNCH
diff --git a/mmgl_amd/csrc/rownorm.hip b/mmgl_amd/csrc/rownorm.hip
--- a/mmgl_amd/csrc/rownorm.hip
+++ b/mmgl_amd/csrc/rownorm.hip
@@ -28,8 +28,9 @@
                                                        T* __restrict__ sum_out, T* __restrict__ y,
                                                        float* __restrict__ mean, float* __restrict__ rstd, int rows,
                                                        int cols, float eps, float p, uint64_t seed,
-                                                       const int* __restrict__ rowmap, T* __restrict__ yc, int crows) {
-    constexpr bool RMS = (MODE & 1) != 0, COMPACT = (MODE & 4) != 0;
+                                                       const int* __restrict__ rowmap, T* __restrict__ yc, int crows,
+                                                       uint8_t* __restrict__ keep_out, float p_next, uint64_t seed_next) {
+    constexpr bool RMS = (MODE & 1) != 0, COMPACT = (MODE & 4) != 0, KEEP = (MODE & 8) != 0;
     typedef typename Vec<T>::type V;
     constexpr int VN = Vec<T>::N;
     __shared__ float red[4];
@@ -50,6 +51,22 @@
             const int c = tr + i * TPR;
             if (live && c < nchunks) {
                 V v = *(const V*)(x + (size_t)row * cols + c * VN);
+                if constexpr (KEEP) {
+                    static_assert(!KEEP || VN == 8, "one keep byte per 8-element chunk");
+                    const uint32_t thr_next = (uint32_t)fminf(p_next * 4294967296.f, 4294967295.f);
+                    constexpr uint64_t G = 0x9E3779B97F4A7C15ull;
+                    const uint64_t z0 = seed_next + ((uint64_t)row * cols + (uint64_t)c * VN + 1) * G;
+                    unsigned kbyte = 0;
+#pragma unroll
+                    for (int j = 0; j < VN; ++j) {
+                        uint64_t z = z0 + (uint64_t)j * G;
+                        z = (z ^ (z >> 30)) * 0xBF58476D1CE4E5B9ull;
+                        z = (z ^ (z >> 27)) * 0x94D049BB133111EBull;
+                        z = z ^ (z >> 31);
+                        kbyte |= ((uint32_t)(z >> 32) < thr_next ? 0u : 1u) << j;
+                    }
+                    keep_out[(size_t)row * nchunks + c] = (uint8_t)kbyte;
+                }
                 if (res) {
                     const V r = *(const V*)(res + (size_t)row * cols + c * VN);
                     if (p > 0.f) {
@@ -270,18 +287,30 @@
 template <typename T, bool RMS>
 int norm_fwd(const char* who, const void* x, const void* res, const void* gamma, const void* beta, void* sum_out, void* y,
              float* mean, float* rstd, int rows, int cols, float eps, hipStream_t st, float p = 0.f, uint64_t seed = 0,
-             const int* rowmap = nullptr, void* yc = nullptr, int crows = 0) {
+             const int* rowmap = nullptr, void* yc = nullptr, int crows = 0, uint8_t* keep_out = nullptr, float p_next = 0.f,
+             uint64_t seed_next = 0) {
     Geo g;
     int rc = geometry<T>(who, rows, cols, g);
     if (rc) return rc;
     int blocks = (rows + g.rpb - 1) / g.rpb;
     if (blocks > 8192) blocks = 8192;
-    if (!RMS && rowmap)
+    if constexpr (!RMS && sizeof(T) == 2) {
+        if (keep_out && rowmap)
+            NORM_DISPATCH(norm_fwd_kernel, T, 12, g, dim3(blocks), dim3(256), 0, st, (const T*)x, (const T*)res, (const T*)gamma, (const T*)beta,
+                          (T*)sum_out, (T*)y, mean, rstd, rows, cols, eps, p, seed, rowmap, (T*)yc, crows, keep_out, p_next, seed_next);
+        else if (keep_out)
+            NORM_DISPATCH(norm_fwd_kernel, T, 8, g, dim3(blocks), dim3(256), 0, st, (const T*)x, (const T*)res, (const T*)gamma, (const T*)beta,
+                          (T*)sum_out, (T*)y, mean, rstd, rows, cols, eps, p, seed, (const int*)nullptr, (T*)nullptr, 0, keep_out, p_next, seed_next);
+    }
+    if (keep_out) {
+        if (RMS || sizeof(T) != 2) MMGL_FAIL(MMGL_ERR_UNSUPPORTED, "%s: the keep map is written by the bf16 LayerNorm kernels only", who);
+    } else if (!RMS && rowmap)
         NORM_DISPATCH(norm_fwd_kernel, T, (RMS ? 1 : 4), g, dim3(blocks), dim3(256), 0, st, (const T*)x, (const T*)res, (const T*)gamma,
-                      (const T*)beta, (T*)sum_out, (T*)y, mean, rstd, rows, cols, eps, p, seed, rowmap, (T*)yc, crows);
+                      (const T*)beta, (T*)sum_out, (T*)y, mean, rstd, rows, cols, eps, p, seed, rowmap, (T*)yc, crows, (uint8_t*)nullptr, 0.f, 0);
     else
         NORM_DISPATCH(norm_fwd_kernel, T, (RMS ? 1 : 0), g, dim3(blocks), dim3(256), 0, st, (const T*)x, (const T*)res, (const T*)gamma,
-                      (const T*)beta, (T*)sum_out, (T*)y, mean, rstd, rows, cols, eps, p, seed, (const int*)nullptr, (T*)nullptr, 0);
+                      (const T*)beta, (T*)sum_out, (T*)y, mean, rstd, rows, cols, eps, p, seed, (const int*)nullptr, (T*)nullptr, 0,
+                      (uint8_t*)nullptr, 0.f, 0);
     MMGL_CHECK_LAUNCH(who);
     return MMGL_OK;
 }
@@ -360,6 +389,30 @@
                   crows);
 }
 
+static int keep_check(const char* who, const void* keep_out, int cols, float p_next, int dtype) {
+    MMGL_CHECK_ARG(keep_out && dtype == MMGL_BF16 && cols % 8 == 0, "%s: the keep map needs bf16 rows of a multiple of 8 columns", who);
+    MMGL_CHECK_ARG(p_next > 0.f && p_next < 1.f, "%s: dropout p=%g outside (0,1)", who, p_next);
+    return MMGL_OK;
+}
+
+extern "C" int mmgl_layernorm_keep_fwd(const void* x, const void* gamma, const void* beta, void* y, float* mean, float* rstd, void* keep_out,
+                                       int rows, int cols, float eps, float p_next, uint64_t seed_next, int dtype, void* stream) {
+    MMGL_CHECK_ARG(x && y && mean && rstd, "mmgl_layernorm_keep_fwd: null pointer");
+    if (int rc = keep_check("mmgl_layernorm_keep_fwd", keep_out, cols, p_next, dtype)) return rc;
+    NORM_BY_DTYPE(norm_fwd, false, x, nullptr, gamma, beta, nullptr, y, mean, rstd, rows, cols, eps, (hipStream_t)stream, 0.f, 0, nullptr, nullptr, 0,
+                  (uint8_t*)keep_out, p_next, seed_next);
+}
+
+extern "C" int mmgl_layernorm_tiles_keep_fwd(const void* x, const void* gamma, const void* beta, void* y, void* yc, const int32_t* rowmap,
+                                             float* mean, float* rstd, void* keep_out, int rows, int cols, int crows, float eps, float p_next,
+                                             uint64_t seed_next, int dtype, void* stream) {
+    MMGL_CHECK_ARG(x && y && mean && rstd, "mmgl_layernorm_tiles_keep_fwd: null pointer");
+    if (int rc = compact_check("mmgl_layernorm_tiles_keep_fwd", rowmap, yc, rows, crows)) return rc;
+    if (int rc = keep_check("mmgl_layernorm_tiles_keep_fwd", keep_out, cols, p_next, dtype)) return rc;
+    NORM_BY_DTYPE(norm_fwd, false, x, nullptr, gamma, beta, nullptr, y, mean, rstd, rows, cols, eps, (hipStream_t)stream, 0.f, 0, rowmap, yc, crows,
+                  (uint8_t*)keep_out, p_next, seed_next);
+}
+
 extern "C" int mmgl_add_layernorm_tiles_fwd(const void* x, const void* res, const void* gamma, const void* beta, void* sum_out, void* y,
                                             void* yc, const int32_t* rowmap, float* mean, float* rstd, int rows, int cols, int crows,
                                             float eps, float p_drop, uint64_t seed, int dtype, void* stream) {
diff --git a/mmgl_amd/model/modelling_cross_attention.py b/mmgl_amd/model/modelling_cross_attention.py
--- a/mmgl_amd/model/modelling_cross_attention.py
+++ b/mmgl_amd/model/modelling_cross_attention.py
@@ -190,7 +190,7 @@
                                "_lora_qkv_cache")
 
     def _forward_self(self, hidden_states, attention_mask, layer_head_mask, output_attentions, past_key_value=None, kv_out=None,
-                      live=None):
+                      live=None, project=True):
         H, d = self.num_heads, self.embed_dim
         if attention_mask is None or attention_mask.dim() != 2:
             raise ValueError("self-attention takes the [bsz, seq_len] key mask (causality is implied); additive 4-D masks are "
@@ -203,7 +203,7 @@
         if live is not None:
             yc, key_tiles = live
             o = ops.frozen_selfattn_tiles(hidden_states, yc, *fused, attention_mask, key_tiles, H)
-            return _lin(self.out_proj, o), None, None
+            return (_lin(self.out_proj, o) if project else o), None, None
         if general:
             if fused is not None:
                 qkv = ops.frozen_linear(hidden_states, *fused)
@@ -249,7 +249,7 @@
             if kv_out is not None:
                 self._file_kv(kv_out, k, v)
             o = ops.selfattn_core(q, k, v, attention_mask, H)
-        return _lin(self.out_proj, o), None, None
+        return (_lin(self.out_proj, o) if project else o), None, None
 
     def _file_kv(self, kv_out, k, v, kv=None):
         if isinstance(kv_out, tuple):
@@ -261,10 +261,10 @@
             kv_out[:, :k.shape[1], k.shape[2]:].copy_(v)
 
     def forward(self, hidden_states, attention_mask=None, neighbor_embeds=None, neighbor_attention_mask=None,
-                past_key_value=None, layer_head_mask=None, output_attentions=False, kv_out=None, live=None):
+                past_key_value=None, layer_head_mask=None, output_attentions=False, kv_out=None, live=None, project=True):
         if self.cross_attention:
             return self._forward_cross(hidden_states, neighbor_embeds, neighbor_attention_mask, layer_head_mask, output_attentions, kv_out)
-        return self._forward_self(hidden_states, attention_mask, layer_head_mask, output_attentions, past_key_value, kv_out, live)
+        return self._forward_self(hidden_states, attention_mask, layer_head_mask, output_attentions, past_key_value, kv_out, live, project)
 
     @staticmethod
     def _decode_proj(mod, x, out_scale=1.0, out=None):
@@ -311,14 +311,18 @@
 
 
 class _Deferred:
-    __slots__ = ("residual", "branch", "p_drop", "training")
-
-    def __init__(self, residual, branch, p_drop=0.0, training=False):
-        self.residual, self.branch, self.p_drop, self.training = residual, branch, p_drop, training
+    __slots__ = ("residual", "branch", "p_drop", "training", "presummed", "seed")
+
+    def __init__(self, residual, branch, p_drop=0.0, training=False, presummed=False, seed=0):
+        self.residual, self.branch, self.p_drop, self.training, self.presummed, self.seed = residual, branch, p_drop, training, presummed, seed
 
 
 def _materialize(h, *_):
-    return ops.gated_residual(h.residual, h.branch, None, h.p_drop, h.training) if isinstance(h, _Deferred) else h
+    if not isinstance(h, _Deferred):
+        return h
+    if h.presummed:
+        return ops.presummed_residual(h.branch, h.residual, h.p_drop, h.seed)
+    return ops.gated_residual(h.residual, h.branch, None, h.p_drop, h.training)
 
 
 class MPTDecoderLayer(nn.Module):
@@ -373,37 +377,77 @@
             h = self._ln(self.final_layer_norm, h)
         return h, attn_w
 
+    def _fused_add_route(self, like, layer_head_mask, output_attentions, past_key_value, kv_out):
+        attn = self.self_attn
+        if not (ops.FUSED_ADD and self.do_layer_norm_before and like.is_cuda and like.dtype == torch.bfloat16):
+            return False, False
+        if layer_head_mask is not None or output_attentions or past_key_value is not None or kv_out is not None:
+            return False, False
+        if (attn.training and attn.dropout > 0) or type(attn.out_proj) is not nn.Linear or attn._frozen_qkv() is None:
+            return False, False
+        by_attn = ops.frozen_linear_add_supported(like, attn.out_proj.weight, attn.out_proj.bias)
+        by_ffn = (self.activation_name == "relu" and type(self.fc1) is nn.Linear and type(self.fc2) is nn.Linear
+                  and ops.relu_ffn_add_supported(like, self.fc1.weight, self.fc1.bias, self.fc2.weight, self.fc2.bias))
+        return by_attn, by_ffn
+
     def _forward_self(self, h, attention_mask, layer_head_mask, output_attentions, defer_residual=False, past_key_value=None, kv_out=None,
                       key_tiles=None):
         pre = self.do_layer_norm_before
         ln1, ln2 = self.self_attn_layer_norm, self.final_layer_norm
         pair = lambda x, r, ln: ops.add_layer_norm_pair(x, r, ln.weight, ln.bias, ln.eps, self.dropout, self.training)
+        summed = pre and isinstance(h, _Deferred) and h.presummed
         like = h.residual if isinstance(h, _Deferred) else h
-        live = None
+        fuse_attn, fuse_ffn = self._fused_add_route(like, layer_head_mask, output_attentions, past_key_value, kv_out)
+        if self.training and self.dropout > 0:
+            fuse_attn = fuse_attn and (summed or not isinstance(h, _Deferred))
+            fuse_ffn = fuse_ffn and fuse_attn
+        p1, seed1 = ops._dropout(self.dropout, self.training, None) if fuse_attn else (0.0, 0)
+        bits1 = (p1, seed1) if p1 > 0 else None
+        tiles = None
         if pre and self.self_attn.key_tiles_route(like, key_tiles, layer_head_mask, output_attentions, past_key_value, kv_out):
+            tiles = key_tiles
+        if summed:
+            outs = ops.presummed_layer_norm(h.branch, h.residual, ln1.weight, ln1.bias, ln1.eps, h.p_drop, h.seed, tiles, bits1)
+        elif tiles is not None:
             if isinstance(h, _Deferred):
-                h, x, yc = ops.add_layer_norm_tiles(h.branch, h.residual, ln1.weight, ln1.bias, ln1.eps, key_tiles, h.p_drop, h.training)
+                outs = ops.add_layer_norm_tiles(h.branch, h.residual, ln1.weight, ln1.bias, ln1.eps, key_tiles, h.p_drop, h.training)
             else:
-                h, x, yc = ops.layer_norm_tiles(h, ln1.weight, ln1.bias, ln1.eps, key_tiles)
-            live = (yc, key_tiles)
+                outs = ops.layer_norm_tiles(h, ln1.weight, ln1.bias, ln1.eps, key_tiles, keep_next=bits1)
         elif isinstance(h, _Deferred):
             if pre:
-                h, x = ops.add_layer_norm_pair(h.branch, h.residual, ln1.weight, ln1.bias, ln1.eps, h.p_drop, h.training)
+                outs = ops.add_layer_norm_pair(h.branch, h.residual, ln1.weight, ln1.bias, ln1.eps, h.p_drop, h.training)
             else:
-                h = x = _materialize(h)
+                outs = (_materialize(h),) * 2
         elif pre:
-            h, x = self._ln_fanout(ln1, h)
-        else:
-            x = h
+            outs = self._ln_fanout(ln1, h) if bits1 is None else ops.layer_norm_fanout(h, ln1.weight, ln1.bias, ln1.eps, keep_next=bits1)
+        else:
+            outs = (h, h)
+        (h, x), more = outs[:2], list(outs[2:])
+        live = (more.pop(0), key_tiles) if tiles is not None else None
+        keep1 = more.pop(0) if bits1 is not None else None
         residual = h
         a, attn_w, _ = self.self_attn(x, attention_mask=attention_mask, layer_head_mask=layer_head_mask,
-                                      output_attentions=output_attentions, past_key_value=past_key_value, kv_out=kv_out, live=live)
-        if pre:
+                                      output_attentions=output_attentions, past_key_value=past_key_value, kv_out=kv_out, live=live,
+                                      project=not fuse_attn)
+        p2, seed2, keep2 = 0.0, 0, None
+        if fuse_attn:
+            if fuse_ffn:
+                p2, seed2 = ops._dropout(self.dropout, self.training, None)
+            bits2 = (p2, seed2) if p2 > 0 else None
+            op = self.self_attn.out_proj
+            outs = ops.frozen_linear_add_norm(a, op.weight, op.bias, residual, ln2.weight, ln2.bias, ln2.eps, p1, seed1, keep1, bits2)
+            (h, x), keep2 = outs[:2], (outs[2] if bits2 is not None else None)
+        elif pre:
             h, x = pair(a, residual, ln2)
         else:
             _, h = pair(a, residual, ln1)
             x = h
         residual = h
+        if fuse_ffn:
+            s = ops.relu_ffn(x, self.fc1.weight, self.fc1.bias, self.fc2.weight, self.fc2.bias, add=(residual, keep2, p2))
+            if defer_residual:
+                return _Deferred(residual, s, p2, self.training, True, seed2), attn_w
+            return ops.presummed_residual(s, residual, p2, seed2), attn_w
         x = self._ffn(x, frozen=None)
         if pre and defer_residual:
             return _Deferred(residual, x, self.dropout, self.training), attn_w
@@ -646,7 +690,10 @@
 
         if self.final_layer_norm is not None:
             fln = self.final_layer_norm
-            if isinstance(hidden_states, _Deferred):
+            if isinstance(hidden_states, _Deferred) and hidden_states.presummed:
+                _, hidden_states = ops.presummed_layer_norm(hidden_states.branch, hidden_states.residual, fln.weight, fln.bias, fln.eps,
+                                                            hidden_states.p_drop, hidden_states.seed)
+            elif isinstance(hidden_states, _Deferred):
                 _, hidden_states = ops.add_layer_norm_pair(hidden_states.branch, hidden_states.residual, fln.weight, fln.bias, fln.eps,
                                                            hidden_states.p_drop, hidden_states.training)
             else:
diff --git a/mmgl_amd/ops.py b/mmgl_amd/ops.py
--- a/mmgl_amd/ops.py
+++ b/mmgl_amd/ops.py
@@ -339,7 +339,9 @@
             and tiles.fits(B, T))
 
 
-def layer_norm_tiles(x, gamma, beta, eps, tiles):
+def layer_norm_tiles(x, gamma, beta, eps, tiles, keep_next=None):
+    if keep_next is not None:
+        return _NormPair.apply(x, None, gamma, beta, float(eps), False, 0.0, 0, tiles, False, keep_next)
     if torch.is_grad_enabled() and x.requires_grad:
         return _NormPair.apply(x, None, gamma, beta, float(eps), False, 0.0, 0, tiles)
     yc = x.new_empty(tiles.m_live, x.shape[-1])
@@ -407,8 +409,10 @@
     return torch.empty(max(int(nbytes), 16), dtype=torch.uint8, device=device)
 
 
-def _norm_fwd(rms, x, res, gamma, beta, eps, p=0.0, seed=0, keep_sum=True, keep_stats=True, compact=None):
+def _norm_fwd(rms, x, res, gamma, beta, eps, p=0.0, seed=0, keep_sum=True, keep_stats=True, compact=None, keep=None):
     require_cuda(x, res)
+    if keep is not None and (rms or res is not None):
+        raise ValueError("_norm_fwd: the keep map is written by the one-input LayerNorm kernels")
     cols = x.shape[-1]
     x2 = x.contiguous().view(-1, cols)
     rows = x2.shape[0]
@@ -422,7 +426,11 @@
         if rms or rowmap.numel() != rows:
             raise ValueError(f"_norm_fwd: the compact copy is LayerNorm's, with one map entry per row ({rowmap.numel()} for {rows} rows)")
         work = dict(bytes=((2.0 if res is None else 3.0 + keep_sum) * rows * cols + yc.numel()) * x.element_size())
-        if res is None:
+        if res is None and keep is not None:
+            s = x2
+            _lib.call("mmgl_layernorm_tiles_keep_fwd", work, ptr(x2), ptr(g), ptr(b), ptr(y), ptr(yc), ptr(rowmap), ptr(mean), ptr(rstd),
+                      ptr(keep[0]), rows, cols, yc.shape[0], eps, keep[1], keep[2], dtype_code(x), stream_ptr())
+        elif res is None:
             s = x2
             _lib.call("mmgl_layernorm_tiles_fwd", work, ptr(x2), ptr(g), ptr(b), ptr(y), ptr(yc), ptr(rowmap), ptr(mean), ptr(rstd), rows,
                       cols, yc.shape[0], eps, dtype_code(x), stream_ptr())
@@ -436,6 +444,9 @@
         work = dict(bytes=2.0 * rows * cols * x.element_size())
         if rms:
             _lib.call("mmgl_rmsnorm_fwd", work, ptr(x2), ptr(g), ptr(y), ptr(rstd), rows, cols, eps, dtype_code(x), stream_ptr())
+        elif keep is not None:
+            _lib.call("mmgl_layernorm_keep_fwd", work, ptr(x2), ptr(g), ptr(b), ptr(y), ptr(mean), ptr(rstd), ptr(keep[0]), rows, cols, eps,
+                      keep[1], keep[2], dtype_code(x), stream_ptr())
         else:
             _lib.call("mmgl_layernorm_fwd", work, ptr(x2), ptr(g), ptr(b), ptr(y), ptr(mean), ptr(rstd), rows, cols, eps, dtype_code(x),
                       stream_ptr())
@@ -505,40 +516,54 @@
 class _NormPair(torch.autograd.Function):
 
     @staticmethod
-    def forward(ctx, x, res, gamma, beta, eps, rms, p, seed, tiles):
+    def forward(ctx, x, res, gamma, beta, eps, rms, p, seed, tiles, *extra):
+        presummed, keep_next = extra if extra else (False, None)
         yc = None if tiles is None else x.new_empty(tiles.m_live, x.shape[-1])
-        s, y, g, mean, rstd = _norm_fwd(rms, x, res, gamma, beta, eps, p, seed, compact=None if tiles is None else (tiles.rowmap, yc))
+        keep = None
+        if keep_next is not None:
+            keep = torch.empty(x.numel() // x.shape[-1], x.shape[-1] // 8, dtype=torch.uint8, device=x.device)
+        s, y, g, mean, rstd = _norm_fwd(rms, x, None if presummed else res, gamma, beta, eps, 0.0 if presummed else p, seed,
+                                        compact=None if tiles is None else (tiles.rowmap, yc),
+                                        keep=None if keep is None else (keep,) + tuple(keep_next))
         ctx.save_for_backward(s, g, mean, rstd)
         ctx.set_materialize_grads(False)
         _norm_ctx(ctx, rms, x.shape, gamma, beta, p, seed)
-        ctx.fanout = res is None
-        outs = (x if res is None else s.view(x.shape)), y.view(x.shape)
-        if tiles is None:
-            return outs
-        ctx.mark_non_differentiable(yc)
-        return outs + (yc,)
-
-    @staticmethod
-    def backward(ctx, ds, dy, _dyc=None):
+        ctx.fanout, ctx.n_extra = res is None, len(extra)
+        outs = (x if res is None or presummed else s.view(x.shape)), y.view(x.shape)
+        for t in (yc, keep):
+            if t is not None:
+                ctx.mark_non_differentiable(t)
+                outs += (t,)
+        return outs
+
+    @staticmethod
+    def backward(ctx, ds, dy, *_):
         s, g, mean, rstd = ctx.saved_tensors
         rms, shape, pgrad, pdtype, p, seed = ctx.cfg
+        tail = (None,) * (5 + ctx.n_extra)
         if dy is None:
             if ds is None or p == 0.0:
-                return ds, (None if ctx.fanout else ds), None, None, None, None, None, None, None
+                return (ds, (None if ctx.fanout else ds), None, None) + tail
             dy = torch.zeros_like(ds)
         dres, dx, dg, db = _norm_bwd(rms, True, dy, ds, s, g, mean, rstd, pgrad, pdtype, p, seed)
         dres = dres.view(shape)
         if ctx.fanout:
-            return dres, None, dg, db, None, None, None, None, None
-        return (dres if dx is None else dx.view(shape)), dres, dg, db, None, None, None, None, None
+            return (dres, None, dg, db) + tail
+        return ((dres if dx is None else dx.view(shape)), dres, dg, db) + tail
 
 
 def layer_norm(x, gamma, beta, eps=1e-5):
     return _Norm.apply(x, gamma, beta, float(eps), False)
 
 
-def layer_norm_fanout(x, gamma, beta, eps=1e-5):
+def layer_norm_fanout(x, gamma, beta, eps=1e-5, keep_next=None):
+    if keep_next is not None:
+        return _NormPair.apply(x, None, gamma, beta, float(eps), False, 0.0, 0, None, False, keep_next)
     return _NormPair.apply(x, None, gamma, beta, float(eps), False, 0.0, 0, None)
+
+
+def presummed_layer_norm(s, res, gamma, beta, eps, p, seed, tiles=None, keep_next=None):
+    return _NormPair.apply(s, res, gamma, beta, float(eps), False, float(p), int(seed), tiles, True, keep_next)
 
 
 def add_layer_norm_pair(x, res, gamma, beta, eps=1e-5, p_drop=0.0, training=False, seed=None):
@@ -1057,6 +1082,31 @@
     return out
 
 
+FUSED_ADD = True
+
+
+def gemm_nt_add_fast(M, N, K, ldx, ldw, ldy, dtype):
+    return dtype == torch.bfloat16 and lib().mmgl_gemm_nt_add_fast(M, N, K, ldx, ldw, ldy, _lib.BF16) == 1
+
+
+def gemm_nt_add(x2, w, bias, res, keep=None, p=0.0, out=None, K=None):
+    require_cuda(x2, w, res)
+    M, N = x2.shape[0], w.shape[0]
+    K = x2.shape[1] if K is None else K
+    y = torch.empty(M, N, dtype=x2.dtype, device=x2.device) if out is None else out
+    if x2.stride(1) != 1 or w.stride(1) != 1 or res.stride(1) != 1 or res.stride(0) != y.stride(0) or res.shape != y.shape or tuple(y.shape) != (M, N) or y.stride(1) != 1:
+        raise ValueError("gemm_nt_add: operands need unit column stride, the residual the output's shape and row stride")
+    if w.shape[1] < K or x2.dtype != w.dtype or res.dtype != x2.dtype or y.dtype != x2.dtype or (bias is not None and (bias.shape != (N,) or bias.dtype != x2.dtype)):
+        raise ValueError(f"gemm_nt_add: x{tuple(x2.shape)} w{tuple(w.shape)} K={K}: one dtype throughout, w with K columns, bias [N]")
+    if keep is not None and (keep.dtype != torch.uint8 or keep.shape != (M, N // 8) or not keep.is_contiguous()):
+        raise ValueError(f"gemm_nt_add: keep map must be contiguous uint8 [{M}, {N // 8}]")
+    _lib.call("mmgl_gemm_nt_add", dict(flops=2.0 * M * N * K, bytes=float(M * K + N * K + 2 * M * N) * x2.element_size(),
+                                       tag=f"{M}x{N}x{K}" + ("+b" if bias is not None else "") + "+add" + ("+keep" if keep is not None else "")),
+              ptr(x2), x2.stride(0), ptr(w), w.stride(0), ptr(bias), ptr(res), ptr(keep), ptr(y), y.stride(0), M, N, K, float(p), dtype_code(x2),
+              stream_ptr())
+    return y
+
+
 def _dgrad_pad_to(g, weight):
     N, K = weight.shape
     if N % 128 == 0 or not (g.dtype == weight.dtype == torch.bfloat16):
@@ -1137,6 +1187,61 @@
         return frozen_dgrad(g, weight).reshape(*dy.shape[:-1], K), None, None, None
 
 
+class _FrozenLinearAdd(torch.autograd.Function):
+
+    @staticmethod
+    def forward(ctx, x, weight, bias, res, keep, p):
+        N, K = weight.shape
+        x2 = _row_strided(x.reshape(-1, K), K, N)
+        out = torch.empty(*x.shape[:-1], N, dtype=x.dtype, device=x.device)
+        gemm_nt_add(x2, weight, bias, res.contiguous().view(-1, N), keep, p, out=out.view(-1, N))
+        ctx.save_for_backward(weight)
+        return out
+
+    @staticmethod
+    def backward(ctx, dy):
+        weight, = ctx.saved_tensors
+        N, K = weight.shape
+        return frozen_dgrad(_row_strided(dy.reshape(-1, N), N, K), weight).reshape(*dy.shape[:-1], K), None, None, None, None, None
+
+
+def frozen_linear_add_supported(x, weight, bias):
+    N, K = weight.shape
+    if not (FUSED_ADD and x.is_cuda and x.dtype == weight.dtype == torch.bfloat16 and weight.is_contiguous() and not weight.requires_grad):
+        return False
+    if bias is not None and (bias.dtype != x.dtype or bias.requires_grad):
+        return False
+    return x.shape[-1] == K and gemm_nt_add_fast(x.numel() // K, N, K, K, K, N, x.dtype)
+
+
+def frozen_linear_add_norm(x, weight, bias, res, gamma, beta, eps, p=0.0, seed=0, keep=None, keep_next=None):
+    s = _FrozenLinearAdd.apply(x, weight, bias, res, keep, float(p))
+    return _NormPair.apply(s, res, gamma, beta, float(eps), False, float(p), int(seed), None, True, keep_next)
+
+
+class _PresummedResidual(torch.autograd.Function):
+
+    @staticmethod
+    def forward(ctx, s, res, p, seed):
+        ctx.p, ctx.seed = p, seed
+        return s.view_as(s)
+
+    @staticmethod
+    def backward(ctx, dy):
+        dy = dy.contiguous()
+        if ctx.p == 0.0:
+            return dy, dy, None, None
+        dx = torch.empty_like(dy)
+        ws = _ws(lib().mmgl_gated_residual_bwd_workspace(dy.numel()), dy.device)
+        _lib.call("mmgl_gated_residual_bwd", dict(bytes=3.0 * dy.numel() * dy.element_size()), ptr(dy), ptr(dy), None, ptr(dx), None, ptr(ws),
+                  ws.numel(), dy.numel(), ctx.p, ctx.seed, dtype_code(dy), stream_ptr())
+        return dx, dy, None, None
+
+
+def presummed_residual(s, res, p, seed):
+    return _PresummedResidual.apply(s, res, float(p), int(seed))
+
+
 def frozen_linear(x, weight, bias, act="none"):
     if weight.requires_grad or (bias is not None and bias.requires_grad):
         raise ValueError("frozen_linear: weight and bias must be frozen (requires_grad=False)")
@@ -1148,7 +1253,9 @@
 class _FrozenReluFFN(torch.autograd.Function):
 
     @staticmethod
-    def forward(ctx, x, w1, b1, w2, b2):
+    def forward(ctx, x, w1, b1, w2, b2, *add):
+        res, keep, p = add if add else (None, None, 0.0)
+        ctx.n_add = len(add)
         (F_, K), N = w1.shape, w2.shape[0]
         x2 = x.contiguous().reshape(-1, K)
         M = x2.shape[0]
@@ -1169,7 +1276,10 @@
             _mfma_aligned(gemm_nt, x2, w, b, act=1, out=h)
         hx = _row_strided(h, F_, N)
         y = x.new_empty(*x.shape[:-1], N)
-        _mfma_aligned(gemm_nt, hx, w2.to(x.dtype).contiguous(), None if b2 is None else b2.to(x.dtype), out=y.view(-1, N))
+        if res is None:
+            _mfma_aligned(gemm_nt, hx, w2.to(x.dtype).contiguous(), None if b2 is None else b2.to(x.dtype), out=y.view(-1, N))
+        else:
+            gemm_nt_add(hx, w2, b2, res.contiguous().view(-1, N), keep, p, out=y.view(-1, N))
         mask, ctx.mask_bits = hx, None
         if nb and hx.stride(0) == pitch and N % 128 == 0 and relu_bits_bytes(rows, F_, N, N, N, pitch, x.dtype) == nb:
             mask, ctx.mask_bits = None, (bits, pitch, rows)
@@ -1194,18 +1304,33 @@
             frozen_dgrad(g[:rows], w2, out=dh[:rows], bits=bits)
             if rows < g.shape[0]:
                 frozen_dgrad(g[rows:], w2, zmask=mask, out=dh[rows:])
-        return frozen_dgrad(_row_strided(dh, F_, K), w1).reshape(*dy.shape[:-1], K), None, None, None, None
-
-
-def relu_ffn(x, w1, b1, w2, b2, frozen=None, return_hidden=False):
+        return (frozen_dgrad(_row_strided(dh, F_, K), w1).reshape(*dy.shape[:-1], K), None, None, None, None) + (None,) * ctx.n_add
+
+
+def relu_ffn_add_supported(x, w1, b1, w2, b2):
+    ps = (w1, b1, w2, b2)
+    if not FUSED_ADD or not x.is_cuda or x.dtype != torch.bfloat16:
+        return False
+    if any(t is not None and (t.requires_grad or t.dtype != torch.bfloat16) for t in ps):
+        return False
+    (F_, K), N = w1.shape, w2.shape[0]
+    M = x.numel() // K
+    return x.shape[-1] == K and w2.is_contiguous() and gemm_nt_add_fast(M, N, F_, _ffn_pitch(M, F_, K, x.dtype), F_, N, x.dtype)
+
+
+def relu_ffn(x, w1, b1, w2, b2, frozen=None, return_hidden=False, add=None):
     if x.shape[-1] != w1.shape[1] or w1.shape[0] != w2.shape[1]:
         raise ValueError(f"relu_ffn: x has {x.shape[-1]} features, fc1 maps {w1.shape[1]} to {w1.shape[0]}, fc2 expects {w2.shape[1]}")
     trainable = any(p is not None and p.requires_grad for p in (w1, b1, w2, b2))
     if frozen and trainable:
         raise ValueError("relu_ffn: weight and bias must be frozen (requires_grad=False)")
+    if add is not None and (trainable or frozen is False):
+        raise ValueError("relu_ffn: `add` is the frozen route's")
     if trainable or frozen is False:
         h = _linear(x, w1, b1, _lib.ACT_RELU, premasked=True)
         y = _linear(h, w2, b2, _lib.ACT_NONE, mask_dx=True)
+    elif add is not None:
+        y, h = _FrozenReluFFN.apply(x, w1, b1, w2, b2, *add)
     else:
         y, h = _FrozenReluFFN.apply(x, w1, b1, w2, b2)
     return (y, h) if return_hidden else y
```

New measurement: 281.1 samples/s. -3.1%, worse.
